# blairstar/NaturalDiffusion

Hardware: AMD Instinct MI355X
Metric: images/sec at 15-step Natural Inference (CIFAR10 32x32, NCSN++), 3-stream throughput (higher is better)
Workload: dtype bf16; 1 GPU; CIFAR10 NI 15-step step_15_weight_173.npz B=512/GPU NCSN++ 61.8M bf16, ni_step fp64 history; nfe=15, batch_per_gpu=512, streams=3

## Files before the change

### include/natinf_ncsnpp.h

```cpp
#ifndef NATINF_NCSNPP_H
#define NATINF_NCSNPP_H

#include <stdint.h>
#include "natinf.h"

#ifdef __cplusplus
extern "C" {
#endif

typedef struct natinf_ncsnpp* natinf_ncsnpp_t;

#define NATINF_NCSNPP_KEEP_ACTIVATIONS 1
#define NATINF_NCSNPP_DDPM 2

int64_t natinf_ncsnpp_param_count(void);
int64_t natinf_ncsnpp_packed_bytes(void);
int64_t natinf_ncsnpp_handle_param_count(natinf_ncsnpp_t h);
int64_t natinf_ncsnpp_handle_packed_bytes(natinf_ncsnpp_t h);
int64_t natinf_ncsnpp_workspace_bytes(natinf_ncsnpp_t h, int max_batch);

int natinf_ncsnpp_create(natinf_ncsnpp_t* out, int flags);
int natinf_ncsnpp_destroy(natinf_ncsnpp_t h);

int natinf_ncsnpp_describe(natinf_ncsnpp_t h, char* buf, int cap);

int natinf_ncsnpp_load(natinf_ncsnpp_t h, const float* params_f32, int64_t n_params,
                       void* packed, int64_t packed_bytes, natinf_stream_t stream);

int natinf_ncsnpp_share(natinf_ncsnpp_t h, natinf_ncsnpp_t loaded);

int natinf_ncsnpp_forward(natinf_ncsnpp_t h, const float* x, const float* labels, float* out, int B,
                          void* workspace, int64_t workspace_bytes, natinf_stream_t stream);

int natinf_ncsnpp_describe_gemms(natinf_ncsnpp_t h, int B, char* buf, int cap);

int natinf_debug_gemm(int variant, int M, int N, int K0, int K1, int taps, int logW, int batch,
                      const void* a0, const void* a1, const void* b, const float* bias_n, void* c, int c_f32, float scale,
                      int iters, natinf_stream_t stream);
int natinf_debug_quant_fp8_rows(const float* w, void* q, float* row_scale, int rows, int cols, natinf_stream_t stream);
int natinf_debug_gemm_fused(int variant, int M, int N, int K, const void* a, const void* b, const float* bias_n, const float* bias_m,
                            const float* rowvec, const float* gate, int log_rows_per_sample, const void* resid_bf16, const float* resid_f32,
                            float scale, int act, void* c, int c_f32, float* gn_part, int* bm_out, int fp32_slab, natinf_stream_t stream);
int natinf_debug_gemm_fp8(int M, int N, int K, const void* a8, const float* a_scale, const void* a_mx, const void* b8, const float* b_scale,
                          const float* bias_n, void* c, void* c_mx, int c_mode, int iters, natinf_stream_t stream);
int natinf_debug_conv_gn_up(int flags);
int natinf_debug_conv_gn(int res, int B, int N, int cin, int c1, const void* x, const float* scale, const float* shift, const void* w_packed, void* w_frag,
                         const void* a1, const float* bias_n, const void* resid, float out_scale, void* out, float* gn_part, int iters,
                         natinf_stream_t stream);
int natinf_set_gemm_variant(int variant);
int natinf_set_gemm_epilogue(int fp32_slab);
int natinf_set_gemm_pref512(int on);
int natinf_set_gemm_half_issue(int on);
int natinf_set_gemm_round_model(int on);
int natinf_set_gemm_w128(int on);
int natinf_set_gemm_raster(int rows);
int natinf_set_fuse_gn(int on);
int natinf_set_conv_gn_wide(int mask);
int natinf_set_conv_gn_w128(int mask);
int natinf_set_conv_gn_w128_min_k(int shape, int k);
int natinf_set_conv_gn_regw(int on);
int natinf_set_fuse_up(int on);
int natinf_set_fuse_head(int on);
int natinf_set_fuse_gn8(int on);
int natinf_set_fuse_gn4(int on);
int natinf_set_fuse_fin(int on);
int natinf_set_conv_gn_warm(int mask);
int natinf_set_attn256(int on);
int natinf_set_attn_proj(int on);
int natinf_set_attn_waves8(int on);
int natinf_set_attn_block(int on);
int natinf_set_attn_qkv(int on);
int natinf_set_conv_gn8_tile(int one_image);
int natinf_set_gemm_splitk(int on);
int natinf_debug_set_splitk_workspace(float* ws, int max_slices);
int natinf_debug_timestamps(void* dev_buf16);

int natinf_ncsnpp_profile(natinf_ncsnpp_t h, int enable);
int natinf_ncsnpp_profile_read(natinf_ncsnpp_t h, double* ms_by_class , int64_t* launches_by_class );

int natinf_gemm_profile(int enable);
int natinf_gemm_profile_read(char* buf, int cap);

int natinf_ncsnpp_debug_tap(natinf_ncsnpp_t h, int module_idx, float* out, int64_t capacity_elems,
                            natinf_stream_t stream);

#ifdef __cplusplus
}
#endif
#endif
```

### naturaldiffusion_amd/_lib.py

```python
from __future__ import annotations

import ctypes as C
import os
from pathlib import Path

os.environ.setdefault("GPU_MAX_HW_QUEUES", "8")

_HERE = Path(__file__).resolve().parent
LIB_PATH = Path(os.environ.get("NATINF_LIB", _HERE / "libnatinf.so"))

if not LIB_PATH.exists():
    raise ImportError(
        f"{LIB_PATH} not found: build it with `make -C {_HERE / 'csrc'}` "
        "(or `python -c 'import __graft_entry__ as g; g.build()'`). "
        "naturaldiffusion_amd has no CPU or eager-PyTorch fallback.")

lib = C.CDLL(str(LIB_PATH))

_p, _i32, _i64, _f32, _f64 = C.c_void_p, C.c_int, C.c_int64, C.c_float, C.c_double

SIGNATURES = {
    "natinf_abi_version": (C.c_int, []),
    "natinf_strerror": (C.c_char_p, [_i32]),
    "natinf_probe": (C.c_int, []),
    "natinf_step_f64hist": (C.c_int, [_p, _p, _p, _p, _p, _p, _p, _i32, _f64, _i32, _f64, _f64, _f32, _f32, _i64, _p]),
    "natinf_step_f32hist": (C.c_int, [_p, _p, _p, _p, _p, _p, _p, _i32, _f32, _i32, _f32, _f32, _f32, _f32, _i64, _p]),
    "natinf_weighted_sum_f64": (C.c_int, [_p, _p, _p, _p, _i32, _i64, _p]),
    "natinf_randn_philox_f32": (C.c_int, [_p, _i64, _i64, _p, _i64, _i64, C.c_uint64, _p]),
    "natinf_to_pixel_u8": (C.c_int, [_p, _p, _i32, _i32, _i32, _i32, _i32, _p]),
    "natinf_step_f32prod": (C.c_int, [_p, _p, _p, _f32, _i64, _i64, _p, _p, _p, _p, _p, _i32, _f32, _p, _p, _i32,
                                      _i32, _f32, _f32, _i64, _p]),
    "natinf_weighted_sum_f32prod": (C.c_int, [_p, _p, _p, _p, _i32, _i64, _p]),
    "natinf_step_f16chain": (C.c_int, [_p, _p, _p, _p, _p, _p, _p, _p, _p, _i32, _f32, _f32, _i32, _f32, _f32, _f32,
                                       _f32, _i32, _i64, _p]),
    "natinf_weighted_mean_f16": (C.c_int, [_p, _p, _p, _p, _i32, _f32, _i64, _p]),
    "natinf_flow_input_f16": (C.c_int, [_p, _p, _p, _f32, _f32, _i64, _p]),
    "natinf_ncsnpp_param_count": (C.c_int64, []),
    "natinf_ncsnpp_workspace_bytes": (C.c_int64, [_p, _i32]),
    "natinf_ncsnpp_packed_bytes": (C.c_int64, []),
    "natinf_ncsnpp_handle_param_count": (_i64, [_p]),
    "natinf_ncsnpp_handle_packed_bytes": (_i64, [_p]),
    "natinf_ncsnpp_create": (C.c_int, [C.POINTER(_p), _i32]),
    "natinf_ncsnpp_describe": (C.c_int, [_p, C.c_char_p, _i32]),
    "natinf_ncsnpp_destroy": (C.c_int, [_p]),
    "natinf_ncsnpp_load": (C.c_int, [_p, _p, _i64, _p, _i64, _p]),
    "natinf_ncsnpp_share": (C.c_int, [_p, _p]),
    "natinf_ncsnpp_forward": (C.c_int, [_p, _p, _p, _p, _i32, _p, _i64, _p]),
    "natinf_ncsnpp_debug_tap": (C.c_int, [_p, _i32, _p, _i64, _p]),
    "natinf_ncsnpp_describe_gemms": (C.c_int, [_p, _i32, C.c_char_p, _i32]),
    "natinf_debug_gemm": (C.c_int, [_i32, _i32, _i32, _i32, _i32, _i32, _i32, _i32, _p, _p, _p, _p, _p, _i32, _f32, _i32, _p]),
    "natinf_set_gemm_variant": (C.c_int, [_i32]),
    "natinf_debug_timestamps": (C.c_int, [_p]),
    "natinf_set_gemm_epilogue": (C.c_int, [_i32]),
    "natinf_debug_gemm_fused": (C.c_int, [_i32, _i32, _i32, _i32, _p, _p, _p, _p, _p, _p, _i32, _p, _p, _f32, _i32, _p, _i32, _p, _p, _i32, _p]),
    "natinf_set_gemm_pref512": (C.c_int, [_i32]),
    "natinf_set_gemm_half_issue": (C.c_int, [_i32]),
    "natinf_set_gemm_raster": (C.c_int, [_i32]),
    "natinf_set_gemm_round_model": (C.c_int, [_i32]),
    "natinf_set_gemm_w128": (C.c_int, [_i32]),
    "natinf_set_fuse_gn": (C.c_int, [_i32]),
    "natinf_set_conv_gn_wide": (C.c_int, [_i32]),
    "natinf_set_attn_block": (C.c_int, [_i32]),
    "natinf_set_conv_gn_w128": (C.c_int, [_i32]),
    "natinf_set_conv_gn_w128_min_k": (C.c_int, [_i32, _i32]),
    "natinf_set_conv_gn_regw": (C.c_int, [_i32]),
    "natinf_set_fuse_up": (C.c_int, [_i32]),
    "natinf_set_fuse_head": (C.c_int, [_i32]),
    "natinf_set_fuse_gn8": (C.c_int, [_i32]),
    "natinf_set_fuse_gn4": (C.c_int, [_i32]),
    "natinf_set_fuse_fin": (C.c_int, [_i32]),
    "natinf_set_attn_proj": (C.c_int, [_i32]),
    "natinf_set_attn_waves8": (C.c_int, [_i32]),
    "natinf_set_attn_qkv": (C.c_int, [_i32]),
    "natinf_set_conv_gn_warm": (C.c_int, [_i32]),
    "natinf_set_attn256": (C.c_int, [_i32]),
    "natinf_set_conv_gn8_tile": (C.c_int, [_i32]),
    "natinf_set_gemm_splitk": (C.c_int, [_i32]),
    "natinf_debug_set_splitk_workspace": (C.c_int, [_p, _i32]),
    "natinf_debug_conv_gn": (C.c_int, [_i32, _i32, _i32, _i32, _i32, _p, _p, _p, _p, _p, _p, _p, _p, _f32, _p, _p, _i32, _p]),
    "natinf_debug_conv_gn_up": (C.c_int, [_i32]),
    "natinf_ncsnpp_profile": (C.c_int, [_p, _i32]),
    "natinf_ncsnpp_profile_read": (C.c_int, [_p, C.POINTER(C.c_double), C.POINTER(C.c_int64)]),
    "natinf_debug_quant_fp8_rows": (C.c_int, [_p, _p, _p, _i32, _i32, _p]),
    "natinf_debug_gemm_fp8": (C.c_int, [_i32, _i32, _i32, _p, _p, _p, _p, _p, _p, _p, _p, _i32, _i32, _p]),
    "natinf_dit_create": (C.c_int, [C.POINTER(_p), _i32, _i32, _i32, _i32]),
    "natinf_dit_destroy": (C.c_int, [_p]),
    "natinf_dit_param_count": (C.c_int64, [_p]),
    "natinf_dit_packed_bytes": (C.c_int64, [_p]),
    "natinf_dit_workspace_bytes": (C.c_int64, [_p, _i32]),
    "natinf_dit_load": (C.c_int, [_p, _p, _i64, _p, _i64, _p]),
    "natinf_dit_forward": (C.c_int, [_p, _p, _p, _p, _p, _i32, _p, _i64, _p]),
    "natinf_mmdit_create": (C.c_int, [C.POINTER(_p), _i32, _i32, _i32, _i32, _i32, _i32, _i32, _i32]),
    "natinf_mmdit_destroy": (C.c_int, [_p]),
    "natinf_mmdit_param_count": (C.c_int64, [_p]),
    "natinf_mmdit_packed_bytes": (C.c_int64, [_p]),
    "natinf_mmdit_workspace_bytes": (C.c_int64, [_p, _i32]),
    "natinf_mmdit_load": (C.c_int, [_p, _p, _i64, _p, _i64, _p]),
    "natinf_mmdit_forward": (C.c_int, [_p, _p, _p, _p, _p, _p, _i32, _p, _i64, _p]),
    "natinf_attention_hd64_bf16": (C.c_int, [_p, _p, _i32, _i64, _p, _p, _i32, _i64, _i32, _i32, _i32, _i32, C.c_float, _p]),
    "natinf_inception_create": (C.c_int, [_p, _i32, _i32]),
    "natinf_inception_destroy": (C.c_int, [_p]),
    "natinf_set_inception_conv": (C.c_int, [_i32]),
    "natinf_debug_conv_ring": (C.c_int, [_i32] * 14 + [_p, _p, _p, _p, _p, _p, _i32, _p]),
    "natinf_inception_param_count": (_i64, [_p]),
    "natinf_inception_packed_bytes": (_i64, [_p]),
    "natinf_inception_workspace_bytes": (_i64, [_p, _i32]),
    "natinf_inception_load": (C.c_int, [_p, _p, _i64, _p, _i64, _p]),
    "natinf_inception_forward": (C.c_int, [_p, _p, _i32, _p, _i32, _p, _i64, _p]),
    "natinf_gemm_profile": (C.c_int, [_i32]),
    "natinf_gemm_profile_read": (C.c_int, [_p, _i32]),
    "natinf_set_mmdit_stream16": (C.c_int, [_i32]),
    "natinf_set_dit_stream16": (C.c_int, [_i32]),
    "natinf_set_mmdit_text_flat": (C.c_int, [_i32]),
    "natinf_attention_profile": (C.c_int, [_i32]),
    "natinf_set_mmdit_text_stream": (C.c_int, [_i32]),
    "natinf_set_flash_mode": (C.c_int, [_i32]),
    "natinf_attention_profile_read": (C.c_int, [_p, _p]),
    "natinf_vae_create": (C.c_int, [C.POINTER(_p), _i32, _i32]),
    "natinf_vae_destroy": (C.c_int, [_p]),
    "natinf_vae_param_count": (C.c_int64, [_p]),
    "natinf_vae_packed_bytes": (C.c_int64, [_p]),
    "natinf_vae_workspace_bytes": (C.c_int64, [_p, _i32]),
    "natinf_vae_load": (C.c_int, [_p, _p, _i64, _p, _i64, _p]),
    "natinf_vae_decode": (C.c_int, [_p, _p, _p, _i32, _p, _i64, _p]),
}

for _name, (_res, _args) in SIGNATURES.items():
    try:
        _fn = getattr(lib, _name)
    except AttributeError as e:
        raise ImportError(f"{LIB_PATH} does not export {_name}; rebuild it") from e
    _fn.restype, _fn.argtypes = _res, _args

SD3_CFG_ON_VELOCITY = 1


def check(rc: int, what: str) -> None:
    if rc != 0:
        raise RuntimeError(f"{what} failed: {lib.natinf_strerror(rc).decode()} ({rc})")


def stream_ptr(stream=None) -> int:
    import torch
    s = stream if stream is not None else torch.cuda.current_stream()
    return int(s.cuda_stream)


def ptr(t) -> int:
    return 0 if t is None else int(t.data_ptr())


def require_gpu() -> None:
    import torch
    if not torch.cuda.is_available():
        raise RuntimeError("naturaldiffusion_amd needs an MI355X (gfx950) GPU: torch.cuda.is_available() is False "
                           "and there is no CPU fallback")
    check(lib.natinf_probe(), "natinf_probe")
```

### naturaldiffusion_amd/csrc/conv_gn3.h

```cpp
#pragma once
#include "gemm_dma.h"

namespace ncsn {

template <int RES, int WM_, int WN_>
struct ConvGn3Cfg {
    static_assert(WM_ * WN_ == 4 && (RES == 32 || RES == 16), "four waves; 32x32 / 16x16 images");
    static constexpr int W = RES, WS = RES + 2, HW = RES * RES, NW = 4, THREADS = 256, KT = 32;
    static constexpr int WM = WM_, WN = WN_, TM = 8, TN = 8;
    static constexpr int BM_ = WM_ * 128, BN_ = WN_ * 128;
    static_assert(HW % BM_ == 0 && BM_ % W == 0, "a tile is whole image rows of one image");
    static constexpr int PR = BM_ / W + 2, PLAST = PR * WS;
    static constexpr int NPIECE = (PLAST + 15) / 16, NROUND = (NPIECE + NW - 1) / NW;
    static constexpr int PATCH_BYTES = NROUND * NW * 1024;
    static constexpr int TAB_BYTES = 256;
    static constexpr int PSW = BM_ / 16 / NW, SC_BYTES = BM_ * 64;
    static constexpr int OFF_TAB = 2 * PATCH_BYTES, OFF_SC = OFF_TAB + 2 * TAB_BYTES, LOOP_BYTES = OFF_SC + 2 * SC_BYTES;
    using Epi = EpiCfg<WM_, WN_, 8, 8, 163840>;
    static constexpr int LDS_BYTES = LOOP_BYTES > Epi::PACK_BYTES ? LOOP_BYTES : Epi::PACK_BYTES;
    static_assert(Epi::PACK_OK && LDS_BYTES <= 163840, "one block per CU");
    static constexpr int swz_key(int xx) { return (xx >> 1) & 2; }
    static constexpr int aoff(int i) { return (RES == 32 ? (i >> 1) * WS + (i & 1) * 16 : i * WS) * 64; }
    static constexpr int BAR = 40;
    static constexpr int rd_a(int i) { return 10 + 2 * i; }
    static constexpr int rd_a_late(int i) { return BAR + 2 + 2 * i; }
    static constexpr int dma_sc(int n) { return BAR + 1 + 2 * n; }
    static_assert(rd_a_late(7) < 64 && dma_sc(PSW - 1) < 64, "inside the step");
    static constexpr int RLEN = 34;
    static constexpr int G_END = 6 * 64 + BAR - 2;
    static constexpr int STRIDE = (G_END - 1 - RLEN - 2 - 12) / (NROUND - 1) > RLEN + 1 ? (G_END - 1 - RLEN - 2 - 12) / (NROUND - 1) : RLEN + 1;
    static constexpr int gp(int r) { return 12 + r * STRIDE; }
    static constexpr int gl(int r) { return r == 0 ? 2 : gp(r - 1) + 5; }
    static_assert(gp(NROUND - 1) + RLEN + 2 < G_END, "the rounds end in front of the barrier of tap 8");
    static constexpr int td(int r) { return gl(r) / 64; }
    static constexpr int nd(int t) { int n = t == 0 ? 2 : 0; for (int r = 0; r < NROUND; ++r) n += td(r) == t; return n; }
    static constexpr int DMA_TAB = 9;
    static constexpr int dma_piece(int r) { int k = td(r) == 0 ? 1 : 0; for (int q = 0; q < r; ++q) k += td(q) == td(r); return 9 + 2 * k; }
    static_assert(td(NROUND - 1) < 8 && dma_piece(NROUND - 1) < 40, "requests behind the weight loads, in front of the barrier");
};

__device__ __forceinline__ void cg3_mfma(f32x4& acc, const u32x4& b, const u32x4& a) {
    asm volatile("v_mfma_f32_16x16x32_bf16 %0, %1, %2, %0" : "+a"(acc) : "v"(b), "v"(a));
}
__device__ __forceinline__ u32x4 cg3_gload16(unsigned voff, const void* sbase) {
    u32x4 v;
    asm volatile("global_load_dwordx4 %0, %1, %2" : "=v"(v) : "v"(voff), "s"(sbase) : "memory");
    return v;
}
__device__ __forceinline__ void cg3_glds16(unsigned voff, const void* sbase, unsigned lds_dst) {
    NATINF_M0_ASM_BEGIN
    asm volatile("s_mov_b32 m0, %2\n\ts_nop 0\n\tglobal_load_lds_dwordx4 %0, %1" :: "v"(voff), "s"(sbase), "s"(lds_dst) : "memory", "m0");
    NATINF_M0_ASM_END
}
__device__ __forceinline__ void cg3_gtab(unsigned toff, const float* sc, const float* sh, unsigned lds_dst) {
    unsigned long long save;
    NATINF_M0_ASM_BEGIN
    asm volatile("s_mov_b32 m0, %4\n\t"
                 "s_mov_b64 %0, exec\n\t"
                 "s_mov_b32 exec_lo, -1\n\t"
                 "s_mov_b32 exec_hi, 0\n\t"
                 "global_load_lds_dword %1, %2\n\t"
                 "s_not_b64 exec, exec\n\t"
                 "global_load_lds_dword %1, %3\n\t"
                 "s_mov_b64 exec, %0"
                 : "=&s"(save) : "v"(toff), "s"(sc), "s"(sh), "s"(lds_dst) : "memory", "m0", "scc");
    NATINF_M0_ASM_END
}
template <int OFF> __device__ __forceinline__ void cg3_lds_write16(unsigned addr, const u32x4& v) {
    asm volatile("ds_write_b128 %0, %1 offset:%2" :: "v"(addr), "v"(v), "n"(OFF) : "memory");
}
template <int VM, int LGKM> __device__ __forceinline__ void cg3_wait() {
    if constexpr (LGKM >= 0) asm volatile("s_waitcnt vmcnt(%0) lgkmcnt(%1)" :: "n"(VM), "n"(LGKM) : "memory");
    else asm volatile("s_waitcnt vmcnt(%0)" :: "n"(VM) : "memory");
}
__device__ __forceinline__ void cg3_wait_lgkm0() { asm volatile("s_waitcnt lgkmcnt(0)" ::: "memory"); }
__device__ __forceinline__ void cg3_barrier() { asm volatile("s_barrier" ::: "memory"); }

#ifdef NATINF_CG3_TIMELINE
#define NATINF_CG3_STAMP(i) do { if (g.dbg_ts && (blockIdx.x == 0 || blockIdx.x == 300) && threadIdx.x == 0) { unsigned long long t_; \
    asm volatile("s_memtime %0\n\ts_waitcnt lgkmcnt(0)" : "=s"(t_) :: "memory"); g.dbg_ts[(blockIdx.x ? 64 : 0) + (i)] = t_; } } while (0)
#else
#define NATINF_CG3_STAMP(i) do { } while (0)
#endif

template <class Cfg>
struct CG3Ctx {
    u32x4 fa[2][8], fb[2][8];
    unsigned boff[8];
    unsigned vo[Cfg::NROUND];
    unsigned scv[Cfg::PSW];
    unsigned a_dx[3];
    unsigned a_sc;
    unsigned nadr[Cfg::NROUND];
    unsigned ninf[Cfg::NROUND];
    unsigned n_tab;
    unsigned tvo;
    u32x4 nv, ns0, ns1, nh0, nh1, npk;
    unsigned nx[8], ne[8];
    const unsigned char* wnext;
    const bf16* pnext;
    const float* tsc; const float* tsh;
    const bf16* scnext;
    unsigned lds_patch, lds_tab, lds_sc, wave;
};

template <int GG, int R, class Cfg>
__device__ __forceinline__ void cg3_norm_gap(CG3Ctx<Cfg>& c) {
    if constexpr (GG < 4) {
        asm volatile("v_lshlrev_b32 %0, 16, %1" : "=v"(c.nx[2 * GG]) : "v"(c.nv[GG]));
        asm volatile("v_and_b32 %0, 0xffff0000, %1" : "=v"(c.nx[2 * GG + 1]) : "v"(c.nv[GG]));
    } else if constexpr (GG < 8) {
        constexpr int P = GG - 4;
        if constexpr (P < 2) {
            asm volatile("v_fma_f32 %0, %0, %1, %2" : "+v"(c.nx[2 * P]) : "v"(c.ns0[2 * P]), "v"(c.nh0[2 * P]));
            asm volatile("v_fma_f32 %0, %0, %1, %2" : "+v"(c.nx[2 * P + 1]) : "v"(c.ns0[2 * P + 1]), "v"(c.nh0[2 * P + 1]));
        } else {
            asm volatile("v_fma_f32 %0, %0, %1, %2" : "+v"(c.nx[2 * P]) : "v"(c.ns1[2 * P - 4]), "v"(c.nh1[2 * P - 4]));
            asm volatile("v_fma_f32 %0, %0, %1, %2" : "+v"(c.nx[2 * P + 1]) : "v"(c.ns1[2 * P - 3]), "v"(c.nh1[2 * P - 3]));
        }
    } else if constexpr (GG < 16) asm volatile("v_exp_f32 %0, %1" : "=v"(c.ne[GG - 8]) : "v"(c.nx[GG - 8]));
    else if constexpr (GG < 20) {
        asm volatile("v_add_f32 %0, %1, %0" : "+v"(c.ne[2 * (GG - 16)]) : "v"(c.ninf[R]));
        asm volatile("v_add_f32 %0, %1, %0" : "+v"(c.ne[2 * (GG - 16) + 1]) : "v"(c.ninf[R]));
    } else if constexpr (GG < 28) asm volatile("v_rcp_f32 %0, %0" : "+v"(c.ne[GG - 20]));
    else if constexpr (GG < 32) {
        asm volatile("v_mul_f32 %0, %0, %1" : "+v"(c.nx[2 * (GG - 28)]) : "v"(c.ne[2 * (GG - 28)]));
        asm volatile("v_mul_f32 %0, %0, %1" : "+v"(c.nx[2 * (GG - 28) + 1]) : "v"(c.ne[2 * (GG - 28) + 1]));
    } else {
        constexpr int P = 2 * (GG - 32);
        asm volatile("v_cvt_pk_bf16_f32 %0, %1, %2" : "=v"(c.npk[P]) : "v"(c.nx[2 * P]), "v"(c.nx[2 * P + 1]));
        asm volatile("v_cvt_pk_bf16_f32 %0, %1, %2" : "=v"(c.npk[P + 1]) : "v"(c.nx[2 * P + 2]), "v"(c.nx[2 * P + 3]));
    }
}

template <class Cfg, int NB, int G, int R = 0>
__device__ __forceinline__ void cg3_norm_slot(CG3Ctx<Cfg>& c) {
    if constexpr (R == 0) {
        if constexpr (G == 0) { c.ns0 = lds_read16<NB * Cfg::TAB_BYTES>(c.n_tab); c.ns1 = lds_read16<NB * Cfg::TAB_BYTES + 16>(c.n_tab); }
        if constexpr (G == 1) { c.nh0 = lds_read16<NB * Cfg::TAB_BYTES + 128>(c.n_tab); c.nh1 = lds_read16<NB * Cfg::TAB_BYTES + 144>(c.n_tab); }
    }
    if constexpr (R < Cfg::NROUND) {
        constexpr int GP = Cfg::gp(R);
        if constexpr (G == Cfg::gl(R)) c.nv = lds_read16<NB * Cfg::PATCH_BYTES>(c.nadr[R]);
        if constexpr (G == GP) cg3_wait_lgkm0();
        if constexpr (G >= GP && G < GP + Cfg::RLEN) cg3_norm_gap<G - GP, R>(c);
        if constexpr (G == GP + Cfg::RLEN) cg3_lds_write16<NB * Cfg::PATCH_BYTES>(c.nadr[R], c.npk);
        cg3_norm_slot<Cfg, NB, G, R + 1>(c);
    }
}

template <class Cfg, int T, int HP, bool NEXT, int S>
struct CG3Tap {
    template <int I>
    static __device__ __forceinline__ void reads(CG3Ctx<Cfg>& c) {
        if constexpr (I < 8) {
            constexpr int P = (T + HP) & 1;
            if constexpr (T < 8) {
                if constexpr (S == Cfg::rd_a(I))
                    c.fa[P ^ 1][I] = lds_read16<HP * Cfg::PATCH_BYTES + Cfg::aoff(I) + ((T + 1) / 3) * Cfg::WS * 64>(c.a_dx[(T + 1) % 3]);
            } else if constexpr (S == Cfg::rd_a_late(I)) {
                if constexpr (NEXT) c.fa[P ^ 1][I] = lds_read16<(HP ^ 1) * Cfg::PATCH_BYTES + Cfg::aoff(I)>(c.a_dx[0]);
                else c.fa[P ^ 1][I] = lds_read16<I * 1024>(c.a_sc);
            }
            reads<I + 1>(c);
        }
    }
    template <int R>
    static __device__ __forceinline__ void requests(CG3Ctx<Cfg>& c) {
        if constexpr (R < Cfg::NROUND) {
            if constexpr (T == Cfg::td(R) && S == Cfg::dma_piece(R))
                cg3_glds16(c.vo[R], c.pnext, c.lds_patch + (HP ^ 1) * Cfg::PATCH_BYTES + (R * Cfg::NW) * 1024 + c.wave * 1024);
            requests<R + 1>(c);
        }
    }
    static __device__ __forceinline__ void run(f32x4 (&acc)[8][8], CG3Ctx<Cfg>& c) {
        constexpr int P = (T + HP) & 1;
        if constexpr (S == 0) {
            if constexpr (T >= 1 && NEXT) cg3_wait<Cfg::nd(T - 1), 0>(); else cg3_wait<0, 0>();
        }
        if constexpr (S >= 1 && S <= 8) c.fb[P ^ 1][S - 1] = cg3_gload16(c.boff[S - 1], c.wnext);
        reads<0>(c);
        if constexpr (NEXT) {
            if constexpr (T == 0 && S == Cfg::DMA_TAB) cg3_gtab(c.tvo, c.tsc, c.tsh, c.lds_tab + (HP ^ 1) * Cfg::TAB_BYTES);
            requests<0>(c);
        } else if constexpr (T == 8 && S > Cfg::BAR && (S - Cfg::BAR - 1) % 2 == 0 && (S - Cfg::BAR - 1) / 2 < Cfg::PSW) {
            constexpr int n = (S - Cfg::BAR - 1) / 2;
            cg3_glds16(c.scv[n], c.scnext, c.lds_sc + Cfg::SC_BYTES + n * 1024 + c.wave * (Cfg::PSW * 1024));
        }
        if constexpr (T >= 2 && NEXT) cg3_norm_slot<Cfg, HP ^ 1, (T - 2) * 64 + S>(c);
        if constexpr (T == 8) {
            if constexpr (S == Cfg::BAR - 1) cg3_wait_lgkm0();
            if constexpr (S == Cfg::BAR) cg3_barrier();
        }
        constexpr int i = S >> 3, j = S & 7;
        cg3_mfma(acc[i][j], c.fb[P][j], c.fa[P][i]);
        if constexpr (S + 1 < 64) CG3Tap<Cfg, T, HP, NEXT, S + 1>::run(acc, c);
    }
};

template <class Cfg, int P, int S>
struct CG3Sc {
    static __device__ __forceinline__ void run(f32x4 (&acc)[8][8], CG3Ctx<Cfg>& c) {
        if constexpr (S == 0) cg3_wait<Cfg::PSW, 0>();
        if constexpr (S == 1) cg3_barrier();
        if constexpr (S >= 1 && S <= 8) c.fb[P ^ 1][S - 1] = cg3_gload16(c.boff[S - 1], c.wnext);
        if constexpr (S >= 9 && (S - 9) % 2 == 0 && (S - 9) / 2 < Cfg::PSW) {
            constexpr int n = (S - 9) / 2;
            cg3_glds16(c.scv[n], c.scnext, c.lds_sc + P * Cfg::SC_BYTES + n * 1024 + c.wave * (Cfg::PSW * 1024));
        }
        if constexpr (S == Cfg::BAR - 1) cg3_wait<8 + Cfg::PSW, -1>();
        if constexpr (S == Cfg::BAR) cg3_barrier();
        if constexpr (S > Cfg::BAR + 1 && (S - Cfg::BAR - 2) % 2 == 0 && (S - Cfg::BAR - 2) / 2 < 8) {
            constexpr int i = (S - Cfg::BAR - 2) / 2;
            c.fa[P ^ 1][i] = lds_read16<(P ^ 1) * Cfg::SC_BYTES + i * 1024>(c.a_sc);
        }
        constexpr int i = S >> 3, j = S & 7;
        cg3_mfma(acc[i][j], c.fb[P][j], c.fa[P][i]);
        if constexpr (S + 1 < 64) CG3Sc<Cfg, P, S + 1>::run(acc, c);
    }
};

template <int RES, int WM, int WN, int EPI>
__global__ __launch_bounds__(256) __attribute__((amdgpu_waves_per_eu(1, 1))) void k_conv_gn3(const GemmArgs g)
{
    using Cfg = ConvGn3Cfg<RES, WM, WN>;
    constexpr int W = Cfg::W, WS = Cfg::WS, HW = Cfg::HW, BM_ = Cfg::BM_, BN_ = Cfg::BN_, NROUND = Cfg::NROUND, PSW = Cfg::PSW, KT = Cfg::KT;
    extern __shared__ __attribute__((aligned(16))) unsigned char smem[];
    lds_poison();
    const int tid = threadIdx.x, lane = tid & 63;
    const int wave = __builtin_amdgcn_readfirstlane(tid >> 6);
    NATINF_CG3_STAMP(0);
    const int wm = wave / WN, wn = wave % WN;
    const int nN = g.N / BN_, nM = g.M / BM_;
    const int tile = xcd_remap(blockIdx.x, nM * nN);
    const int mt = tile / nN, nt = tile - mt * nN;
    const int m0 = mt * BM_, n0 = nt * BN_;
    const int b = m0 / HW, y0 = (m0 % HW) / W;
    const int ush = g.a0_up;
    const bf16* const img = g.a0 + (int64_t)b * (HW >> (2 * ush)) * g.a0_ld;
    const float* const gsc = g.gn_scale + (int64_t)b * g.gn_ld;
    const float* const gsh = g.gn_shift + (int64_t)b * g.gn_ld;
    const int n_half = g.a0_C / KT, n_sc = g.a1 ? g.a1_C / KT : 0;
    const int nk = 9 * n_half, NT = nk + n_sc;
    const unsigned char* const wfrag = reinterpret_cast<const unsigned char*>(g.b_frag);
    const int sup = g.a1_up;
    const bf16* const a1base = g.a1 ? g.a1 + (int64_t)(sup ? b * (HW >> 2) : m0) * g.a1_ld : nullptr;

    typedef __attribute__((address_space(3))) unsigned char lds_u8;
    CG3Ctx<Cfg> c;
    c.wave = (unsigned)wave;
    c.lds_patch = (unsigned)(uintptr_t)((lds_u8*)smem);
    c.lds_tab = c.lds_patch + Cfg::OFF_TAB;
    c.lds_sc = c.lds_patch + Cfg::OFF_SC;
    const int prow = lane >> 2, pslot = lane & 3;
#pragma unroll
    for (int j = 0; j < 8; ++j) c.boff[j] = (unsigned)(((n0 >> 4) + wn * 8 + j) * NT) * 1024u + (unsigned)lane * 16u;
#pragma unroll
    for (int r = 0; r < NROUND; ++r) {
        const int pp = (r * 4 + wave) * 16 + prow;
        const int yy = pp / WS, xx = pp - yy * WS;
        const int y = min(max(y0 - 1 + yy, 0), RES - 1), x = min(max(xx - 1, 0), RES - 1);
        c.vo[r] = (unsigned)(((y >> ush) * (W >> ush) + (x >> ush)) * g.a0_ld + ((pslot ^ Cfg::swz_key(xx)) << 3)) * 2u;
        const bool inside = (unsigned)(y0 - 1 + yy) < (unsigned)RES && (unsigned)(xx - 1) < (unsigned)RES;
        c.ninf[r] = inside ? 0x3f800000u : 0x7f800000u;
        c.nadr[r] = c.lds_patch + (unsigned)((r * 4 + wave) * 1024 + prow * 64 + ((pslot ^ Cfg::swz_key(xx)) << 4));
    }
#pragma unroll
    for (int n = 0; n < PSW; ++n) {
        const int pp = (wave * PSW + n) * 16 + prow;
        const int src = sup ? ((y0 + pp / W) >> 1) * (W >> 1) + ((pp % W) >> 1) : pp;
        c.scv[n] = (unsigned)(src * g.a1_ld + ((pslot ^ ((pp >> 1) & 2)) << 3)) * 2u;
    }
    c.tvo = (unsigned)(lane & 31) * 4u;
    c.n_tab = c.lds_tab + ((unsigned)pslot << 5);
    {
        const int frow = lane & 15, fq = lane >> 4;
        const int ml = wm * 128 + frow;
        const int pc = ((ml / W) + 1) * WS + (ml % W) + 1, xc = ml % W;
#pragma unroll
        for (int d = 0; d < 3; ++d) c.a_dx[d] = c.lds_patch + (unsigned)((pc - WS + d - 1) * 64 + ((fq ^ Cfg::swz_key(xc + d)) << 4));
        c.a_sc = c.lds_sc + (unsigned)(ml * 64 + ((fq ^ ((ml >> 1) & 2)) << 4));
    }

    if (n_sc > 0) {
#pragma unroll
        for (int n = 0; n < PSW; ++n) cg3_glds16(c.scv[n], a1base, c.lds_sc + n * 1024 + c.wave * (PSW * 1024));
    }
    cg3_gtab(c.tvo, gsc, gsh, c.lds_tab);
#pragma unroll
    for (int r = 0; r < NROUND; ++r) cg3_glds16(c.vo[r], img, c.lds_patch + (r * 4) * 1024 + c.wave * 1024);
#pragma unroll
    for (int j = 0; j < 8; ++j) c.fb[0][j] = cg3_gload16(c.boff[j], wfrag);
    c.scnext = n_sc > 0 ? a1base + KT : reinterpret_cast<const bf16*>(wfrag);
    f32x4 acc[8][8];
#pragma unroll
    for (int i = 0; i < 8; ++i)
#pragma unroll
        for (int j = 0; j < 8; ++j) acc[i][j] = f32x4{0.f, 0.f, 0.f, 0.f};
    NATINF_CG3_STAMP(1);
    auto norm0 = [&](auto r_tag, const f32x4& s0, const f32x4& s1, const f32x4& h0, const f32x4& h1) __attribute__((always_inline)) {
        constexpr int R = decltype(r_tag)::value;
        cg3_wait<NROUND - 1 - R + 8, -1>();
        unsigned char* const pa = smem + (c.nadr[R] - c.lds_patch);
        const u32x4 nv = *reinterpret_cast<const u32x4*>(pa);
        const float ni = __uint_as_float(c.ninf[R]);
        u32x4 ou;
#pragma unroll
        for (int p = 0; p < 4; ++p) {
            const unsigned w_ = nv[p];
            const float x0 = __uint_as_float(w_ << 16), x1 = __uint_as_float(w_ & 0xffff0000u);
            const float sa = p < 2 ? s0[2 * p] : s1[2 * p - 4], sb = p < 2 ? s0[2 * p + 1] : s1[2 * p - 3];
            const float ha = p < 2 ? h0[2 * p] : h1[2 * p - 4], hb = p < 2 ? h0[2 * p + 1] : h1[2 * p - 3];
            const float t0 = __builtin_fmaf(x0, sa, ha), t1 = __builtin_fmaf(x1, sb, hb);
            const float y0_ = t0 * __builtin_amdgcn_rcpf(ni + __builtin_amdgcn_exp2f(t0)), y1_ = t1 * __builtin_amdgcn_rcpf(ni + __builtin_amdgcn_exp2f(t1));
            typedef __bf16 bf16x2_t __attribute__((ext_vector_type(2)));
            const bf16x2_t pr_ = {(bf16)y0_, (bf16)y1_};
            ou[p] = __builtin_bit_cast(unsigned, pr_);
        }
        *reinterpret_cast<u32x4*>(pa) = ou;
    };
    {
        cg3_wait<NROUND + 8, -1>();
        NATINF_CG3_STAMP(2);
        const unsigned char* const tp = smem + (c.n_tab - c.lds_patch);
        const f32x4 s0 = *reinterpret_cast<const f32x4*>(tp), s1 = *reinterpret_cast<const f32x4*>(tp + 16);
        const f32x4 h0 = *reinterpret_cast<const f32x4*>(tp + 128), h1 = *reinterpret_cast<const f32x4*>(tp + 144);
        using std::integral_constant;
        norm0(integral_constant<int, 0>{}, s0, s1, h0, h1); norm0(integral_constant<int, 1>{}, s0, s1, h0, h1); norm0(integral_constant<int, 2>{}, s0, s1, h0, h1);
        norm0(integral_constant<int, 3>{}, s0, s1, h0, h1); norm0(integral_constant<int, 4>{}, s0, s1, h0, h1); norm0(integral_constant<int, 5>{}, s0, s1, h0, h1);
        if constexpr (NROUND > 6) { norm0(integral_constant<int, 6>{}, s0, s1, h0, h1); norm0(integral_constant<int, 7>{}, s0, s1, h0, h1); }
        if constexpr (NROUND > 8) { norm0(integral_constant<int, 8>{}, s0, s1, h0, h1); norm0(integral_constant<int, 9>{}, s0, s1, h0, h1); }
        static_assert(NROUND == 6 || NROUND == 8 || NROUND == 10, "rounds of the prologue");
    }
    cg3_wait<0, -1>();
    __syncthreads();
#pragma unroll
    for (int i = 0; i < 8; ++i) c.fa[0][i] = *reinterpret_cast<const u32x4*>(smem + (c.a_dx[0] - c.lds_patch) + Cfg::aoff(i));
    asm volatile("s_waitcnt lgkmcnt(0)" ::: "memory");
    __builtin_amdgcn_sched_barrier(0);

    NATINF_CG3_STAMP(3);
    using std::integral_constant;
    auto half_chunk = [&](auto hp_tag, auto next_tag, int h) __attribute__((always_inline)) {
        constexpr int HP = decltype(hp_tag)::value;
        constexpr bool NEXT = decltype(next_tag)::value;
        c.pnext = img + (h + 1) * KT; c.tsc = gsc + (h + 1) * KT; c.tsh = gsh + (h + 1) * KT;
        const int kt = h * 9;
        NATINF_CG3_STAMP(4 + (h < 36 ? h : 35));
#define NATINF_CG3_TAP(T)                                                                                             \
        c.wnext = wfrag + (int64_t)((T < 8 || NEXT) ? kt + T + 1 : min(nk, NT - 1)) * 1024;                              \
        CG3Tap<Cfg, T, HP, NEXT, 0>::run(acc, c);
        NATINF_CG3_TAP(0) NATINF_CG3_TAP(1) NATINF_CG3_TAP(2) NATINF_CG3_TAP(3) NATINF_CG3_TAP(4)
        NATINF_CG3_TAP(5) NATINF_CG3_TAP(6) NATINF_CG3_TAP(7) NATINF_CG3_TAP(8)
#undef NATINF_CG3_TAP
    };
    for (int h = 0; h + 2 < n_half; h += 2) {
        half_chunk(integral_constant<int, 0>{}, std::true_type{}, h);
        half_chunk(integral_constant<int, 1>{}, std::true_type{}, h + 1);
    }
    half_chunk(integral_constant<int, 0>{}, std::true_type{}, n_half - 2);
    half_chunk(integral_constant<int, 1>{}, std::false_type{}, n_half - 1);
    NATINF_CG3_STAMP(40);
    for (int s = 0; s < n_sc; s += 2) {
        c.wnext = wfrag + (int64_t)min(nk + s + 1, NT - 1) * 1024; c.scnext = a1base + min(s + 2, n_sc - 1) * KT;
        CG3Sc<Cfg, 0, 0>::run(acc, c);
        c.wnext = wfrag + (int64_t)min(nk + s + 2, NT - 1) * 1024; c.scnext = a1base + min(s + 3, n_sc - 1) * KT;
        CG3Sc<Cfg, 1, 0>::run(acc, c);
    }
    cg3_wait<0, 0>();
#define NATINF_CG3_PIN8(a) asm volatile("" :: "v"(a[0]), "v"(a[1]), "v"(a[2]), "v"(a[3]), "v"(a[4]), "v"(a[5]), "v"(a[6]), "v"(a[7]));
    NATINF_CG3_PIN8(c.fb[0]) NATINF_CG3_PIN8(c.fb[1]) NATINF_CG3_PIN8(c.fa[0]) NATINF_CG3_PIN8(c.fa[1])
#undef NATINF_CG3_PIN8
    NATINF_CG3_STAMP(41);
#if defined(__HIP_DEVICE_COMPILE__)
    typedef const unsigned __attribute__((address_space(4))) *kernarg_u32_t;
    kernarg_u32_t gp = (kernarg_u32_t)__builtin_amdgcn_kernarg_segment_ptr();
    asm volatile("" : "+s"(gp));
    GemmArgs ge;
    {
        unsigned* d = reinterpret_cast<unsigned*>(&ge);
#pragma unroll
        for (unsigned i = 0; i < sizeof(GemmArgs) / 4; ++i) d[i] = gp[i];
    }
    asm volatile("" :: "s"(ge.c), "s"(ge.bias_n), "s"(ge.rowvec), "s"(ge.resid), "s"(ge.gn_part), "s"(ge.c_ld), "s"(ge.rowvec_ld), "s"(ge.resid_ld), "s"(ge.gn_quads),
                 "s"(ge.log_rows_per_sample), "s"(ge.scale), "s"(ge.M), "s"(ge.N));
#else
    const GemmArgs ge = g;
#endif
    asm volatile("s_waitcnt vmcnt(0) lgkmcnt(0)\n\ts_nop 15\n\ts_nop 15\n\ts_barrier" ::: "memory");
    __builtin_amdgcn_sched_barrier(0);
    int lane_e;
    asm volatile("v_mbcnt_lo_u32_b32 %0, -1, 0\n\tv_mbcnt_hi_u32_b32 %0, -1, %0" : "=v"(lane_e));
    const int tid_e = wave * 64 + lane_e;
    NATINF_CG3_STAMP(42);
    static_assert(EPI == 1 || EPI == 2 || EPI == 5 || EPI == 6, "packed epilogues: plain / + GroupNorm partials / + bf16 residual / both");
    constexpr bool FIN16 = RES == 16 && WM == 2 && WN == 2 && (EPI == 2 || EPI == 6);
    packed_tile_epilogue<WM, WN, 8, 8, typename Cfg::Epi, ACT_NONE, EPI == 2 || EPI == 6, EPI == 5 || EPI == 6, false, false, 1, FIN16, true, true>(ge, smem, acc, m0, n0, 0, tid_e, lane_e, wm, wn);
    NATINF_CG3_STAMP(43);
}

}
```

### naturaldiffusion_amd/csrc/ncsnpp.hip

```cpp
#include <hip/hip_runtime.h>
#include <stdint.h>
#include <stdio.h>
#include <string.h>
#include <stdlib.h>
#include <functional>
#include <map>
#include <memory>
#include <string>
#include <vector>

#include "natinf_ncsnpp.h"
#include "ncsnpp_kernels.h"
#include "gemm_dma.h"
#include "gemm_w128.h"
#include "conv_ring.h"
#include "conv_gn.h"
#include "conv_gn2.h"
#include "head_conv.h"
#ifdef NATINF_DEV
#include "conv_patch.h"
#include "gemm_8phase.h"
#endif
#include "gemm_fp8.h"
#include "attn_fused.h"
#include "attn256.h"
#include "attn_qkv.h"
#include "attn_blk256.h"
#include "flash_attn.h"

using namespace ncsn;

namespace {

constexpr int NF = 128, IMG = 32, TEMB = 512, NLEVEL = 4;
constexpr int CH_MULT[NLEVEL] = {1, 2, 2, 2};
constexpr float GN_EPS = 1e-6f;
constexpr float INV_SQRT2 = 0.70710678118654752440f;
inline bool attn_at(int res) { return res == 16; }
inline int ilog2(int v) { int l = 0; while ((1 << l) < v) ++l; return l; }
inline int64_t align_up(int64_t v, int64_t a) { return (v + a - 1) / a * a; }

enum Kind { K_LIN, K_CONV, K_RES, K_ATTN, K_GN, K_DOWN, K_UP };
const char* kind_name(int k) { static const char* n[] = {"lin", "conv", "res", "attn", "gn", "down", "up"}; return n[k]; }

struct Mod { int idx, kind, cin, cout, up, down, res; int64_t poff; };

struct TRef { int64_t off = -1; int C = 0, ld = 0, res = 0, coff = 0, pad = 0; };

struct Ctx {
    int B; unsigned char* ws; const unsigned char* wp; hipStream_t stream;
    const float* x; const float* labels; float* out;
    int* part_bm;
    hipStream_t stream2 = nullptr; hipEvent_t* ev = nullptr;
    unsigned char* fin_done = nullptr;
    bf16* act(const TRef& t) const { return reinterpret_cast<bf16*>(ws + t.off * B) + t.coff; }
    template <class T> T* at(int64_t off) const { return reinterpret_cast<T*>(ws + off * B); }
    template <class T> const T* w(int64_t off) const { return reinterpret_cast<const T*>(wp + off); }
};
using OpFn = std::function<void(const Ctx&)>;
enum { CLS_GEMM = 0, CLS_OTHER = 1, CLS_CONV_GN = 2, CLS_CONV_GN8 = 3, N_CLS = 4 };

struct PackCtx { const float* params; unsigned char* packed; hipStream_t stream; };
using PackFn = std::function<void(const PackCtx&)>;

struct Arena {
    bool keep = false; int64_t top = 0, peak = 0;
    std::map<int64_t, int64_t> free_;
    std::map<int64_t, int64_t> live_;
    int64_t alloc(int64_t bytes) {
        bytes = align_up(bytes, 256);
        if (!keep)
            for (auto it = free_.begin(); it != free_.end(); ++it)
                if (it->second >= bytes) {
                    const int64_t off = it->first, rest = it->second - bytes;
                    free_.erase(it);
                    if (rest) free_[off + bytes] = rest;
                    live_[off] = bytes;
                    return off;
                }
        const int64_t off = top; top += bytes; if (top > peak) peak = top;
        live_[off] = bytes;
        return off;
    }
    void release(int64_t off) {
        if (keep || off < 0) return;
        auto it = live_.find(off);
        if (it == live_.end()) return;
        int64_t o = off, s = it->second;
        live_.erase(it);
        auto nx = free_.lower_bound(o);
        if (nx != free_.end() && o + s == nx->first) { s += nx->second; nx = free_.erase(nx); }
        if (nx != free_.begin()) { auto pv = std::prev(nx); if (pv->first + pv->second == o) { o = pv->first; s += pv->second; free_.erase(pv); } }
        if (o + s == top) top = o; else free_[o] = s;
    }
};

}

struct natinf_ncsnpp {
    int flags = 0;
    std::vector<Mod> mods;
    int64_t n_params = 0;
    std::vector<OpFn> ops;
    std::vector<int> op_cls;
    std::vector<PackFn> packs;
    bool prof = false;
    struct Rec { hipEvent_t a, b; int cls; };
    std::vector<Rec> recs;
    std::vector<hipEvent_t> pool;
    std::map<int, TRef> taps;
    int64_t ws_per_image = 0, packed_bytes = 0;
    uint64_t plan_sig = 0;
    const unsigned char* packed = nullptr;
    bool attr_set = false;
    int last_B = 0; unsigned char* last_ws = nullptr;
    std::vector<int> part_bm;
    std::vector<unsigned char> fin_done;
};

bool configure_conv_ring();
namespace { bool configure_dit_attention(); }
namespace ncsn_cg3 { bool configure(); int tile_rows(int shape); int tile_cols(int shape); void launch(const void* gemm_args, int shape, int epi, void* stream); }

namespace {

int g_epi_fp32_slab = 0;
GemmArgs gemm_defaults() {
    GemmArgs g;
    memset(&g, 0, sizeof(g));
    g.epi_fp32_slab = g_epi_fp32_slab;
    g.taps = 1; g.batch = 1; g.scale = 1.0f; g.act = ACT_NONE; g.c_mode = OUT_BF16;
    return g;
}
constexpr int NUM_CU = 256;
enum GemmVariant {
    V_AUTO = 0, V_GENERIC = 1,
    V_DMA_256x256 = 2, V_DMA_256x128 = 3, V_DMA_128x128 = 4,
    V_RING_256x256 = 5, V_RING_256x128 = 6, V_RING_128x128 = 7, V_RING_64x128 = 8,
    V_RING_256x128_W4 = 9, V_DMA_256x128_W4 = 10,
    V_DMA_256x256_S = 11, V_DMA_128x128_S = 12,
    V_DMA_512x128 = 13,
    V_PATCH_256x256 = 14, V_PATCH_256x128 = 15,
    V_DMA_256x256_P = 16, V_DMA_128x128_P = 17, V_DMA_256x128W4_P = 18,
    V_8PH_256x256 = 19, V_8PH_NOPRIO = 20, V_8PH_READFIRST = 21, V_8PH_BOTH = 22,
    V_FP8_256x256 = 23,
    V_ABL_NODMA = 24, V_ABL_NOMFMA = 25,
    V_DMA_256x256_H = 26, V_DMA_512x128_H = 27,
    V_CONV_GN = 28,
    V_W128 = 29,
    V_W128_A = 30, V_W128_D = 31, V_W128_X = 32,
    V_COUNT
};
const char* variant_name(int v) {
    static const char* n[] = {"auto", "generic128", "dma256x256", "dma256x128", "dma128x128", "ring256x256", "ring256x128",
                              "ring128x128", "ring64x128", "ring256x128w4", "dma256x128w4", "dma256x256s", "dma128x128s", "dma512x128", "patch256x256", "patch256x128", "dma256x256p", "dma128x128p", "dma256x128w4p", "gemm8ph", "gemm8ph_np", "gemm8ph_rf", "gemm8ph_nprf", "fp8_256x256", "abl_nodma", "abl_nomfma", "dma256x256h", "dma512x128h", "conv_gn", "w128_256x256", "w128_a", "w128_d", "w128_x"};
    return v >= 0 && v < V_COUNT ? n[v] : "?";
}
inline bool variant_shipped(int v) {
#ifdef NATINF_DEV
    return v >= 0 && v < V_COUNT;
#else
    switch (v) {
        case V_AUTO: case V_GENERIC: case V_RING_64x128: case V_RING_256x128_W4: case V_DMA_128x128_P: case V_FP8_256x256:
        case V_DMA_256x256_H: case V_DMA_512x128_H: case V_CONV_GN: case V_W128: return true;
        default: return false;
    }
#endif
}
unsigned long long* g_dbg_ts = nullptr;
int g_force_variant = V_AUTO;
int g_half_issue = 1;
int g_round_model = 1;
int g_round_model_w128 = 13;
int g_pref_512 = 1;
std::string* g_record = nullptr;

int g_raster_g = 8;
template <class Cfg, class K>
inline void launch_tiles(K kernel, const GemmArgs& g0, hipStream_t s) {
    const int nM = (g0.M + Cfg::BM_ - 1) / Cfg::BM_, nN = (g0.N + Cfg::BN_ - 1) / Cfg::BN_;
    GemmArgs g = g0;
    g.raster_g = (g_raster_g > 1 && nN >= 8 && nM >= g_raster_g) ? g_raster_g : 0;
    int lds = Cfg::LDS_BYTES;
#ifdef NATINF_DEV
    static const int one_per_cu = getenv("NATINF_ONE_BLOCK_PER_CU") ? 1 : 0;
    if (one_per_cu && lds < 84000) {
        lds = 84000;
        (void)hipFuncSetAttribute(reinterpret_cast<const void*>(kernel), hipFuncAttributeMaxDynamicSharedMemorySize, lds);
    }
#endif
    hipLaunchKernelGGL(kernel, dim3(nM * nN, 1, g.batch), dim3(Cfg::THREADS), lds, s, g);
}
template <class Cfg, class K>
inline bool set_lds(K kernel) {
    return hipFuncSetAttribute(reinterpret_cast<const void*>(kernel), hipFuncAttributeMaxDynamicSharedMemorySize, Cfg::LDS_BYTES) == hipSuccess;
}
using CfgD256x256 = DmaCfg<2, 4, 8, 4>;  using CfgD256x128 = DmaCfg<4, 2, 4, 4>;  using CfgD128x128 = DmaCfg<2, 2, 4, 4>;
using CfgR256x256 = RingCfg<2, 4, 8, 4, 4>; using CfgR256x128 = RingCfg<4, 2, 4, 4, 6>;
using CfgR128x128 = RingCfg<2, 2, 4, 4, 4>; using CfgR64x128 = RingCfg<2, 2, 2, 4, 4>;
using CfgR256x128W4 = RingCfg<2, 2, 8, 4, 3>; using CfgD256x128W4 = DmaCfg<2, 2, 8, 4>;
using CfgD512x128 = DmaCfg<4, 2, 8, 4>;
using CfgH32 = ConvGn2Cfg<32>; using CfgH16 = ConvGn2Cfg<16>; using CfgH16W = ConvGn2Cfg<16, true>; using CfgH32W = ConvGn2Cfg<32, true>; using CfgH8T = ConvGn2Cfg<8, true, 4>; using CfgH4T = ConvGn2Cfg<4, true, 4, 2, 2>;
#ifdef NATINF_DEV
using CfgH8W = ConvGn2Cfg<8, true>;
using CfgP256x256 = PatchCfg<2, 4, 8, 4, 344>; using CfgP256x128 = PatchCfg<4, 2, 4, 4, 400>;
using CfgG32 = ConvGnCfg<32>; using CfgG16 = ConvGnCfg<16>; using CfgG16W = ConvGnCfg<16, true>;
#endif
int g_fuse_head = 1;
int g_cg8_tm4 = 1;
constexpr int ATTN_BLK_DEFAULT = 2;
int g_attn_blk = ATTN_BLK_DEFAULT;
int g_attn_qkv = 1;
int g_attn_w8 = 1;
int g_attn_proj = 1;
int g_attn256 = 1;
int g_fuse_gn8 = 1;
int g_cg_warm = 15;
int g_fuse_fin = 3;
int g_fuse_gn4 = 1;
int g_fuse_gn = 1;

constexpr unsigned EPI_ALL = 0x1FF;
constexpr unsigned EPI_R64 = EPI_ALL, EPI_D128 = EPI_ALL, EPI_RW4 = EPI_ALL & ~(1u << 3), EPI_D256H = EPI_ALL & ~(1u << 3),
                   EPI_D512H = EPI_ALL & ~((1u << 3) | (1u << 4) | (1u << 7) | (1u << 8)),
                   EPI_W128 = EPI_ALL & ~((1u << 2) | (1u << 3) | (1u << 6));
template <unsigned MASK, int E, class F> inline void epi_case(F&& f) { if constexpr ((MASK >> E) & 1u) f(std::integral_constant<int, E>{}); }
template <unsigned MASK, class F> inline bool for_each_epi(F&& f) {
    bool ok = true;
    auto one = [&](auto tag) { ok = ok && f(tag); };
    epi_case<MASK, 0>(one); epi_case<MASK, 1>(one); epi_case<MASK, 2>(one); epi_case<MASK, 3>(one); epi_case<MASK, 4>(one);
    epi_case<MASK, 5>(one); epi_case<MASK, 6>(one); epi_case<MASK, 7>(one); epi_case<MASK, 8>(one);
    return ok;
}
#define NATINF_EPI_OF(tag) decltype(tag)::value
bool set_lds_epi_all() {
    return for_each_epi<EPI_D128>([](auto t) { return set_lds<CfgD128x128>(&k_gemm_dma<2, 2, 4, 4, 2, NATINF_EPI_OF(t)>); }) &&
           for_each_epi<EPI_RW4>([](auto t) { return set_lds<CfgR256x128W4>(&k_gemm_ring<2, 2, 8, 4, 3, NATINF_EPI_OF(t)>); }) &&
           for_each_epi<EPI_R64>([](auto t) { return set_lds<CfgR64x128>(&k_gemm_ring<2, 2, 2, 4, 4, NATINF_EPI_OF(t)>); }) &&
           for_each_epi<EPI_D256H>([](auto t) { return set_lds<CfgD256x256>(&k_gemm_dma<2, 4, 8, 4, 6, NATINF_EPI_OF(t)>); }) &&
           for_each_epi<EPI_D512H>([](auto t) { return set_lds<CfgD512x128>(&k_gemm_dma<4, 2, 8, 4, 6, NATINF_EPI_OF(t)>); }) &&
           for_each_epi<EPI_W128>([](auto t) { return set_lds<W128Cfg>(&k_gemm_w128<NATINF_EPI_OF(t)>); }) && set_lds<W128Cfg>(&k_gemm_w128<9>)
#ifdef NATINF_DEV
           && set_lds<W128Cfg>(&k_gemm_w128<1, W128SchA>) && set_lds<W128Cfg>(&k_gemm_w128<1, W128SchP>) && set_lds<W128Cfg>(&k_gemm_w128<1, W128SchX>)
           && for_each_epi<EPI_ALL>([](auto t) { return set_lds<CfgD256x256>(&k_gemm_dma<2, 4, 8, 4, 2, NATINF_EPI_OF(t)>); })
           && for_each_epi<EPI_ALL>([](auto t) { return set_lds<CfgD512x128>(&k_gemm_dma<4, 2, 8, 4, 2, NATINF_EPI_OF(t)>); })
#endif
        ;
}
template <int EPI>
bool set_lds_conv_gn() {
    return set_lds<CfgH32>(&k_conv_gn2<32, false, EPI>) && set_lds<CfgH32W>(&k_conv_gn2<32, true, EPI>) && set_lds<CfgH16>(&k_conv_gn2<16, false, EPI>) && set_lds<CfgH16W>(&k_conv_gn2<16, true, EPI>) &&
           set_lds<CfgH8T>(&k_conv_gn2<8, true, EPI, 4>) && set_lds<CfgH4T>(&k_conv_gn2<4, true, EPI, 4, 2, 2>)
#ifdef NATINF_DEV
           && set_lds<CfgH8W>(&k_conv_gn2<8, true, EPI>)
           && set_lds<CfgG32>(&k_conv_gn<32, false, EPI>) && set_lds<CfgG16>(&k_conv_gn<16, false, EPI>) && set_lds<CfgG16W>(&k_conv_gn<16, true, EPI>)
#endif
        ;
}

bool configure_gemm_kernels() {
    bool ok = hipFuncSetAttribute(reinterpret_cast<const void*>(&k_gemm_bf16), hipFuncAttributeMaxDynamicSharedMemorySize,
                                  GEMM_LDS_BYTES) == hipSuccess;
    ok = ok && hipFuncSetAttribute(reinterpret_cast<const void*>(&k_head_conv), hipFuncAttributeMaxDynamicSharedMemorySize, HeadConvCfg::LDS_BYTES) == hipSuccess &&
         set_lds<CfgR128x128>(&k_gemm_ring<2, 2, 4, 4, 4, 9>) &&
         set_lds_epi_all() && ncsn_cg3::configure() && ::configure_conv_ring() && configure_dit_attention() && set_lds_conv_gn<1>() && set_lds_conv_gn<2>() && set_lds_conv_gn<5>() && set_lds_conv_gn<6>() &&
#ifdef NATINF_DEV
         set_lds<CfgD256x256>(&k_gemm_dma<2, 4, 8, 4>) && set_lds<CfgD256x128>(&k_gemm_dma<4, 2, 4, 4>) &&
         set_lds<CfgD128x128>(&k_gemm_dma<2, 2, 4, 4>) && set_lds<CfgR256x256>(&k_gemm_ring<2, 4, 8, 4, 4>) &&
         set_lds<CfgR256x128>(&k_gemm_ring<4, 2, 4, 4, 6>) && set_lds<CfgR128x128>(&k_gemm_ring<2, 2, 4, 4, 4>) &&
         set_lds<CfgD256x128W4>(&k_gemm_dma<2, 2, 8, 4>) && set_lds<CfgD256x256>(&k_gemm_dma<2, 4, 8, 4, 1>) &&
         set_lds<CfgD128x128>(&k_gemm_dma<2, 2, 4, 4, 1>) && set_lds<CfgD512x128>(&k_gemm_dma<4, 2, 8, 4>) &&
         set_lds<CfgP256x256>(&k_conv_patch<2, 4, 8, 4, 344>) && set_lds<CfgP256x128>(&k_conv_patch<4, 2, 4, 4, 400>) &&
         set_lds<CfgD256x128W4>(&k_gemm_dma<2, 2, 8, 4, 2>) &&
         set_lds<CfgD256x256>(&k_gemm_dma<2, 4, 8, 4, 3, 1>) && set_lds<CfgD256x256>(&k_gemm_dma<2, 4, 8, 4, 4, 1>) &&
         set_lds<Cfg8ph>(&k_gemm_8ph<0>) && set_lds<Cfg8ph>(&k_gemm_8ph<1>) && set_lds<Cfg8ph>(&k_gemm_8ph<2>) && set_lds<Cfg8ph>(&k_gemm_8ph<3>) &&
#endif
         set_lds<CfgD256x256>(&k_gemm_fp8<false, 0>) && set_lds<CfgD256x256>(&k_gemm_fp8<true, 0>) &&
         set_lds<CfgD256x256>(&k_gemm_fp8<false, 1>) && set_lds<CfgD256x256>(&k_gemm_fp8<true, 1>) &&
         set_lds<CfgD256x256>(&k_gemm_fp8<false, 2>) && set_lds<CfgD256x256>(&k_gemm_fp8<true, 2>) &&
         set_lds<CfgD256x256>(&k_gemm_fp8<false, 3>) && set_lds<CfgD256x256>(&k_gemm_fp8<true, 3>) &&
         set_lds<W128F8Cfg>(&k_gemm_w128_fp8<false, 0>) && set_lds<W128F8Cfg>(&k_gemm_w128_fp8<true, 0>) && set_lds<W128F8Cfg>(&k_gemm_w128_fp8<false, 1>) && set_lds<W128F8Cfg>(&k_gemm_w128_fp8<true, 1>) &&
         set_lds<W128F8Cfg>(&k_gemm_w128_fp8<false, 2>) && set_lds<W128F8Cfg>(&k_gemm_w128_fp8<true, 2>) && set_lds<W128F8Cfg>(&k_gemm_w128_fp8<false, 3>) && set_lds<W128F8Cfg>(&k_gemm_w128_fp8<true, 3>) &&
#ifdef NATINF_DEV
         set_lds<AttnCfg<8, 16, true>>(&k_attn_fused<8, 16, true>) &&
#endif
         hipFuncSetAttribute(reinterpret_cast<const void*>(&k_qkv256), hipFuncAttributeMaxDynamicSharedMemorySize, QKV_LDS_BYTES) == hipSuccess &&
         hipFuncSetAttribute(reinterpret_cast<const void*>(&k_attn256<false>), hipFuncAttributeMaxDynamicSharedMemorySize, A256_LDS_BYTES) == hipSuccess &&
         hipFuncSetAttribute(reinterpret_cast<const void*>(&k_attn256<true>), hipFuncAttributeMaxDynamicSharedMemorySize, A256_LDS_BYTES) == hipSuccess &&
         hipFuncSetAttribute(reinterpret_cast<const void*>(&k_attn256<true, 8>), hipFuncAttributeMaxDynamicSharedMemorySize, A256_LDS_BYTES) == hipSuccess &&
         hipFuncSetAttribute(reinterpret_cast<const void*>(&k_attn_blk256), hipFuncAttributeMaxDynamicSharedMemorySize, ABLK_LDS_BYTES) == hipSuccess &&
         hipFuncSetAttribute(reinterpret_cast<const void*>(&k_attn_blk256_v2), hipFuncAttributeMaxDynamicSharedMemorySize, ABLK2_LDS_BYTES) == hipSuccess &&
         hipFuncSetAttribute(reinterpret_cast<const void*>(&k_flash_attn64), hipFuncAttributeMaxDynamicSharedMemorySize, FA_LDS_BYTES) == hipSuccess &&
#ifdef NATINF_DEV
         hipFuncSetAttribute(reinterpret_cast<const void*>(&k_flash_attn64_v2<0>), hipFuncAttributeMaxDynamicSharedMemorySize, FA_LDS_BYTES) == hipSuccess &&
         hipFuncSetAttribute(reinterpret_cast<const void*>(&k_flash_attn64_v2<1>), hipFuncAttributeMaxDynamicSharedMemorySize, FA_LDS_BYTES) == hipSuccess &&
#endif
         hipFuncSetAttribute(reinterpret_cast<const void*>(&k_flash_attn64_v2<1, 64>), hipFuncAttributeMaxDynamicSharedMemorySize, FA_LDS_BYTES / 2) == hipSuccess;
    if (!ok) (void)hipGetLastError();
    return ok;
}

#ifdef NATINF_DEV
inline bool eligible_8ph(const GemmArgs& g) { return g.M % 256 == 0 && g.N % 256 == 0; }
#endif

int variant_bm(int v);
int packed_epi(const GemmArgs& g, int bm);
int g_cg3 = 7;
int g_cg_wide = 3;
int g_fuse_up = 1;
int g_cg_regw = 1;
int g_cg3_min_k[3] = {2304, 0, 2304};
inline int conv_gn3_shape(const GemmArgs& g) {
    const int res = 1 << g.logW;
    if (!g_cg3 || !g_cg_regw || !g.b_frag || g.N % 128) return -1;
    int sh = -1;
    if (res == 32) sh = g.N % 256 ? ((g_cg3 & 1) ? 0 : -1) : ((g_cg3 & 2) ? 1 : -1);
    else if (res == 16) sh = (g.N % 256 == 0 && (g_cg3 & 4)) ? 2 : -1;
    if (sh >= 0 && 9 * g.a0_C + (g.a1 ? g.a1_C : 0) < g_cg3_min_k[sh]) sh = -1;
    return sh;
}
inline int conv_gn_bm(const GemmArgs& g) {
    const int res = 1 << g.logW;
    if (const int sh3 = conv_gn3_shape(g); sh3 >= 0) return ncsn_cg3::tile_rows(sh3);
    if (res == 8) return g_cg8_tm4 ? 64 : 128;
    if (res == 4) return 64;
    if (res == 32) return ((g_cg_wide & 2) && g.N % 256 == 0 && g_cg_regw && g.b_frag) ? 128 : 256;
    return ((g_cg_wide & 1) && res == 16 && g.N % 256 == 0) ? 128 : 256;
}
inline int conv_gn_part_rows(const GemmArgs& g) { const int res = 1 << g.logW; return res <= 8 ? res * res : conv_gn_bm(g); }
inline bool conv_gn_regw(const GemmArgs& g) { return g_cg_regw && g.b_frag && (conv_gn3_shape(g) >= 0 || g.N % ((conv_gn_bm(g) <= 128 && (1 << g.logW) != 4) ? 256 : 128) == 0); }
#ifdef NATINF_DEV
constexpr bool HAVE_CONV_GN_V1 = true;
#else
constexpr bool HAVE_CONV_GN_V1 = false;
#endif
inline int conv_gn_epi(const GemmArgs& g) { GemmArgs t = g; t.epi_fp32_slab = 0; return packed_epi(t, conv_gn_part_rows(g)); }
inline bool conv_gn_ok(const GemmArgs& g) {
    if (!g.gn_scale || !g.gn_shift || !g.gn_folded || g.taps != 9 || g.batch != 1 || g.a0_C % BK || (g.a1 && g.a1_C % BK)) return false;
    const int res = 1 << g.logW;
    if (g.logHW != 2 * g.logW || (res != 32 && res != 16 && res != 8 && res != 4) || g.N % 8) return false;
    if (res == 4 && (g.a0_C % (64 * CfgH4T::NG) || (g.a1 && g.a1_C % (64 * CfgH4T::NG)))) return false;
    if (res <= 8 ? (g.M % (res * res) || g.N % (res == 4 ? 128 : 256) || g.a0_up || g.a1_up || !conv_gn_regw(g) || (g.resid && g.rowvec)) : g.M % std::max(256, conv_gn_bm(g)) != 0) return false;
    if ((g.a0_up || g.a1_up || !HAVE_CONV_GN_V1) && !conv_gn_regw(g)) return false;
    const int e = conv_gn_epi(g);
    return e == 1 || e == 2 || e == 5 || e == 6;
}
int g_w128 = 1;
bool w128_ok(const GemmArgs& g) {
    if (g.taps != 1 || g.a1 || g.gn_scale || g.deq_m || g.deq_n || g.splitk > 1) return false;
    if (g.a0_C % BK || g.a0_C < 2 * BK || g.N % 8 || g.M % 8) return false;
    return (int64_t)g.M * g.a0_ld * 2 < (int64_t)1 << 32 && (int64_t)g.N * g.b_ld * 2 < (int64_t)1 << 32;
}
int choose_variant(const GemmArgs& g) {
    if (g.gn_scale) return V_CONV_GN;
    const int K0 = g.taps * g.a0_C, K1 = g.a1 ? g.a1_C : 0;
    const bool dma = K0 % BK == 0 && K1 % BK == 0 && (g.taps == 1 || (g.a0_padded && g.a0_C % BK == 0));
    if (!dma) return V_GENERIC;
    if (!variant_shipped(g_force_variant)) {  }
#ifdef NATINF_DEV
    else if (g_force_variant == V_PATCH_256x256 || g_force_variant == V_PATCH_256x128) {
        const bool patch_ok = g.taps == 9 && g.batch == 1 && g.logW >= 3;
        if (patch_ok && (g_force_variant == V_PATCH_256x128 || g.logW >= 4)) return g_force_variant;
    } else if (g_force_variant >= V_8PH_256x256 && g_force_variant <= V_8PH_BOTH) {
        if (eligible_8ph(g)) return g_force_variant;
    }
#endif
    else if (g_force_variant == V_W128) {
        if (w128_ok(g) && (!g.gn_part || (1 << g.logHW) % 256 == 0)) return V_W128;
    }
#ifdef NATINF_DEV
    else if (g_force_variant >= V_W128_A && g_force_variant <= V_W128_X) {
        if (w128_ok(g) && packed_epi(g, 256) == 1) return g_force_variant;
    }
#endif
    else if (g_force_variant > V_GENERIC && g_force_variant != V_CONV_GN && g_force_variant != V_FP8_256x256) {
        if (!g.gn_part || (g.taps == 9 && (1 << g.logHW) % variant_bm(g_force_variant) == 0)) return g_force_variant;
    }
    const int64_t mt256 = (g.M + 255) / 256, mt128 = (g.M + 127) / 128;
    const int64_t nt128 = (g.N + 127) / 128;
#ifdef NATINF_DEV
    const bool half = g_half_issue != 0;
#else
    constexpr bool half = true;
#endif
    const bool w128 = g_w128 && w128_ok(g) && (!g.gn_part || (1 << g.logHW) % 256 == 0);
    const int64_t nt256 = (g.N + 255) / 256;
    const bool n_ok256 = g.N % 256 == 0 || (w128 && g.N % 128 == 0);
    if (g_round_model && g.taps == 1 && !g.gn_part && g.batch == 1 && n_ok256 && K0 + K1 >= 1024 && mt256 * nt256 < 2 * NUM_CU) {
        const int64_t r256 = (mt256 * nt256 + NUM_CU - 1) / NUM_CU, r128 = (mt128 * nt128 + 2 * NUM_CU - 1) / (2 * NUM_CU);
        const int64_t c256 = w128 ? g_round_model_w128 : 15;
        if (mt128 * nt128 >= NUM_CU / 2) return c256 * r256 < 10 * r128 ? (w128 ? V_W128 : half ? V_DMA_256x256_H : V_DMA_256x256_P) : V_DMA_128x128_P;
    }
    if (n_ok256 && K0 + K1 >= 1024 && mt256 * nt256 * g.batch >= NUM_CU) return w128 ? V_W128 : half ? V_DMA_256x256_H : V_DMA_256x256_P;
    if (g_pref_512 && g.N <= 128 && K0 + K1 >= 1024 && ((g.M + 511) / 512) * g.batch >= 2 * NUM_CU &&
        (!g.gn_part || (g.taps == 9 && (1 << g.logHW) % 512 == 0)))
        return half ? V_DMA_512x128_H : V_DMA_512x128;
    if (mt256 * nt128 * g.batch >= 2 * NUM_CU) return V_RING_256x128_W4;
    if (mt128 * nt128 * g.batch >= NUM_CU) return V_DMA_128x128_P;
    return V_RING_64x128;
}

int variant_bm(int v) {
    switch (v) {
        case V_CONV_GN: case V_DMA_256x256: case V_DMA_256x128: case V_RING_256x256: case V_RING_256x128: case V_RING_256x128_W4: case V_DMA_256x128_W4:
        case V_ABL_NODMA: case V_ABL_NOMFMA: case V_DMA_256x256_H: case V_DMA_256x256_S: case V_PATCH_256x256: case V_PATCH_256x128: case V_DMA_256x256_P: case V_DMA_256x128W4_P: case V_8PH_256x256: case V_8PH_NOPRIO: case V_8PH_READFIRST: case V_8PH_BOTH: case V_FP8_256x256: case V_W128: case V_W128_A: case V_W128_D: case V_W128_X: return 256;
        case V_DMA_512x128: case V_DMA_512x128_H: return 512;
        case V_RING_64x128: return 64;
        default: return 128;
    }
}

int fp8_epi(const GemmArgs& g) {
    if (g.epi_fp32_slab || g.resid || g.gn_part) return 0;
    if ((g.rowvec || g.gate) && g.log_rows_per_sample < 30 && ((1 << g.log_rows_per_sample) % 256 != 0)) return 0;
    if (g.c_mode == OUT_F32 && g.resid_f32 && !g.bias_m && g.act == ACT_NONE && g.resid_f32_ld % 4 == 0 && g.c_ld % 4 == 0) return 3;
    if (g.resid_f32 || g.gate) return 0;
    if (g.c_mode == OUT_BF16 && g.act == ACT_NONE) return 1;
    if (g.c_mode == OUT_FP8_MX && g.act == ACT_GELU_TANH && g.c_mx && g.N % 32 == 0 && !g.bias_m && g.scale == 1.0f) return 2;
    return 0;
}
extern int g_w128;
bool w128_fp8_ok(const GemmArgs& g) {
    return g.taps == 1 && !g.a1 && g.a0_C % 256 == 0 && g.N % 8 == 0 && g.M % 8 == 0 && (!g.a_mx || g.M % 256 == 0) &&
           (int64_t)g.M * g.a0_ld < (int64_t)1 << 32 && (int64_t)g.N * g.b_ld < (int64_t)1 << 32;
}
bool fp8_on_w128(const GemmArgs& g) { return g_w128 && w128_fp8_ok(g) && (fp8_epi(g) != 2 || g_w128 != 2); }
template <bool MXA>
void launch_gemm_fp8_t(const GemmArgs& g, hipStream_t s) {
    if (fp8_on_w128(g)) {
        switch (fp8_epi(g)) {
            case 1: launch_tiles<W128F8Cfg>(&k_gemm_w128_fp8<MXA, 1>, g, s); break;
            case 2: launch_tiles<W128F8Cfg>(&k_gemm_w128_fp8<MXA, 2>, g, s); break;
            case 3: launch_tiles<W128F8Cfg>(&k_gemm_w128_fp8<MXA, 3>, g, s); break;
            default: launch_tiles<W128F8Cfg>(&k_gemm_w128_fp8<MXA, 0>, g, s); break;
        }
        return;
    }
    switch (fp8_epi(g)) {
        case 1: launch_tiles<CfgD256x256>(&k_gemm_fp8<MXA, 1>, g, s); break;
        case 2: launch_tiles<CfgD256x256>(&k_gemm_fp8<MXA, 2>, g, s); break;
        case 3: launch_tiles<CfgD256x256>(&k_gemm_fp8<MXA, 3>, g, s); break;
        default: launch_tiles<CfgD256x256>(&k_gemm_fp8<MXA, 0>, g, s); break;
    }
}
struct GemmProf {
    struct Rec { hipEvent_t a, b; std::string tag; };
    bool on = false; std::vector<Rec> ev; std::vector<std::pair<hipEvent_t, hipEvent_t>> pool;
    bool begin(Rec& r, hipStream_t s) {
        r.a = r.b = nullptr;
        if (!pool.empty()) { r.a = pool.back().first; r.b = pool.back().second; pool.pop_back(); }
        else if (hipEventCreate(&r.a) != hipSuccess || hipEventCreate(&r.b) != hipSuccess) { r.a = r.b = nullptr; (void)hipGetLastError(); return false; }
        (void)hipEventRecord(r.a, s);
        return true;
    }
    void end(Rec& r, hipStream_t s) { (void)hipEventRecord(r.b, s); ev.push_back(std::move(r)); }
} g_gemm_prof;
void launch_gemm_fp8(const GemmArgs& g, hipStream_t s) {
    GemmProf::Rec r;
    const bool prof = g_gemm_prof.on && !g_record && g_gemm_prof.begin(r, s);
    if (prof) {
        char line[160];
        snprintf(line, sizeof(line), "%d %d %d %d %d %d %s%s/e%d", g.M, g.N, g.taps * g.a0_C, 0, g.taps, g.batch, fp8_on_w128(g) ? "w128_fp8" : "fp8_256x256", g.a_mx ? "_mxa" : "", fp8_epi(g));
        r.tag = line;
    }
    if (g.a_mx) launch_gemm_fp8_t<true>(g, s); else launch_gemm_fp8_t<false>(g, s);
    if (prof) g_gemm_prof.end(r, s);
}

int packed_epi(const GemmArgs& g, int bm) {
    if (g.epi_fp32_slab || g.deq_m || g.deq_n || g.act == ACT_RELU) return 0;
    if (g.bias_m) return (g.c_mode == OUT_BF16 && !g.resid && !g.resid_f32 && !g.gate && !g.rowvec && !g.gn_part && g.act == ACT_NONE) ? 8 : 0;
    if ((g.rowvec || g.gate) && g.log_rows_per_sample < 30 && ((1 << g.log_rows_per_sample) % bm != 0)) return 0;
    if (g.c_mode == OUT_F32 && g.resid_f32 && !g.resid && !g.gn_part && g.act == ACT_NONE && g.resid_f32_ld % 4 == 0 && g.c_ld % 4 == 0) return 7;
    if (g.c_mode != OUT_BF16 || g.resid_f32 || g.gate) return 0;
    if (g.resid && (g.act != ACT_NONE || g.resid_ld % 4 != 0)) return 0;
    if (g.gn_part) return (g.act == ACT_NONE && g.M % bm == 0) ? (g.resid ? 6 : 2) : 0;
    if (g.resid) return 5;
    return g.act == ACT_NONE ? 1 : (g.act == ACT_SILU ? 3 : 4);
}
inline unsigned epi_mask(int v) {
    switch (v) {
        case V_RING_64x128: return EPI_R64;  case V_DMA_128x128_P: return EPI_D128;  case V_RING_256x128_W4: return EPI_RW4;
        case V_DMA_256x256_H: return EPI_D256H;  case V_DMA_512x128_H: return EPI_D512H;
        case V_DMA_256x256_P: case V_DMA_512x128: return EPI_ALL;
        case V_W128: return EPI_W128;
        default: return 1u;
    }
}
inline int effective_epi(int v, const GemmArgs& g) { const int e = packed_epi(g, variant_bm(v)); return ((epi_mask(v) >> e) & 1u) ? e : 0; }
#define NATINF_LAUNCH_EPI(MASK, CFG, KERN, ...)                                                                      \
    {                                                                                                                \
        auto run_ = [&](auto t_) { launch_tiles<CFG>(&KERN<__VA_ARGS__, NATINF_EPI_OF(t_)>, g, s); };                \
        switch (effective_epi(v, g)) {                                                                               \
            case 1: epi_case<MASK, 1>(run_); break;  case 2: epi_case<MASK, 2>(run_); break;                         \
            case 3: epi_case<MASK, 3>(run_); break;  case 4: epi_case<MASK, 4>(run_); break;                         \
            case 5: epi_case<MASK, 5>(run_); break;  case 6: epi_case<MASK, 6>(run_); break;                         \
            case 7: epi_case<MASK, 7>(run_); break;  case 8: epi_case<MASK, 8>(run_); break;                         \
            default: run_(std::integral_constant<int, 0>{}); break;                                                  \
        }                                                                                                            \
    }

thread_local int g_launch_error = 0;
thread_local bool g_fin_written = false;
int g_splitk = 1;
float* g_dbg_splitk_ws = nullptr; int g_dbg_splitk_max = 0;
int splitk_slices(const GemmArgs& g) {
    if (!g_splitk || !g.splitk_ws || g.splitk_max < 2 || g.batch != 1 || g.gn_scale || g.c_mode != OUT_BF16 || g.N % 8 || 256 % (g.N / 8)) return 1;
    if (g.gn_part && (g.M % SPLITK_ROWS || g.act != ACT_NONE || (g.taps == 9 && (1 << g.logHW) % SPLITK_ROWS))) return 1;
    if (g.bias_m || g.gate || g.resid_f32 || g.deq_m || g.deq_n) return 1;
    const int K0 = g.taps * g.a0_C, K1 = g.a1 ? g.a1_C : 0;
    if (K0 % 64 || K1 % 64 || (g.taps == 9 && !g.a0_padded) || K0 + K1 < 2048) return 1;
    const int64_t tiles = ((g.M + 127) / 128) * ((g.N + 127) / 128);
    if (tiles >= 2 * NUM_CU) return 1;
    int S = (int)((2 * NUM_CU + tiles - 1) / tiles);
    if (S > g.splitk_max) S = g.splitk_max;
    while (S > 1 && (K0 + K1) / 32 / S < 16) --S;
    return S;
}
int w128_splitk_slices(const GemmArgs& g) {
    if (!g_splitk || !g_w128 || !g.splitk_ws || g.splitk_max < 2 || g.batch != 1 || !w128_ok(g) || g.a0_C < 3072) return 1;
    if (g.c_mode != OUT_F32 || !g.resid_f32 || g.resid || g.rowvec || g.bias_m || g.gn_part || g.act != ACT_NONE || g.epi_fp32_slab || g.N % 4 || g.c_ld % 4 || g.resid_f32_ld % 4) return 1;
    const int64_t tiles = (int64_t)((g.M + 255) / 256) * ((g.N + 255) / 256) * g.batch;
    if (tiles * 2 > NUM_CU) return 1;
    int S = (int)(NUM_CU / tiles);
    if (S > g.splitk_max) S = g.splitk_max;
    while (S > 1 && g.a0_C / BK / S < 16) --S;
    return S;
}
int launch_gemm_run(const GemmArgs& g0, hipStream_t s);
int launch_gemm(const GemmArgs& g0, hipStream_t s) {
    if (!g_gemm_prof.on || g_record) return launch_gemm_run(g0, s);
    GemmProf::Rec r;
    std::string tag;
    g_record = &tag; (void)launch_gemm_run(g0, s); g_record = nullptr;
    while (!tag.empty() && tag.back() == '\n') tag.pop_back();
    if (!g_gemm_prof.begin(r, s)) return launch_gemm_run(g0, s);
    r.tag = std::move(tag);
    const int bm = launch_gemm_run(g0, s);
    g_gemm_prof.end(r, s);
    return bm;
}
int launch_gemm_run(const GemmArgs& g0, hipStream_t s) {
    if (g_force_variant == V_AUTO) {
        const int S8 = w128_splitk_slices(g0);
        if (S8 > 1) {
            if (g_record) {
                char line[160];
                snprintf(line, sizeof(line), "%d %d %d %d %d %d splitk%d_w128_256x256/e7\n", g0.M, g0.N, g0.taps * g0.a0_C, 0, g0.taps, g0.batch, S8);
                *g_record += line;
                return 256;
            }
            GemmArgs p = g0;
            p.splitk = S8; p.c = g0.splitk_ws; p.c_mode = OUT_F32;
            const int nM = (p.M + 255) / 256, nN = (p.N + 255) / 256;
            p.raster_g = 0;
            hipLaunchKernelGGL((k_gemm_w128<9>), dim3(nM * nN, S8, p.batch), dim3(256), W128Cfg::LDS_BYTES, s, p);
            const int64_t per = (int64_t)g0.M * (g0.N / 4);
            hipLaunchKernelGGL(k_splitk_reduce_f32, dim3((unsigned)((per + 255) / 256), (unsigned)g0.batch), dim3(256), 0, s, g0.splitk_ws, S8, (int64_t)g0.batch * g0.M * g0.N, g0.M, g0.N,
                               g0.bias_n, g0.gate, g0.gate_ld, g0.log_rows_per_sample, g0.z_samples, g0.resid_f32, g0.resid_f32_ld, g0.c_bs, g0.scale,
                               reinterpret_cast<float*>(g0.c), g0.c_ld, g0.stream_f16);
            return 256;
        }
    }
    const int S = g_force_variant == V_AUTO ? splitk_slices(g0) : 1;
    if (S > 1) {
        if (g_record) {
            char line[160];
            snprintf(line, sizeof(line), "%d %d %d %d %d %d splitk%d_ring128x128/e9\n", g0.M, g0.N, g0.taps * g0.a0_C, g0.a1 ? g0.a1_C : 0, g0.taps, g0.batch, S);
            *g_record += line;
            return SPLITK_ROWS;
        }
        GemmArgs p = g0;
        p.splitk = S; p.c = g0.splitk_ws; p.c_mode = OUT_F32; p.batch = S;
        p.bias_n = nullptr; p.rowvec = nullptr; p.resid = nullptr; p.scale = 1.0f; p.act = ACT_NONE; p.gn_part = nullptr;
        launch_tiles<CfgR128x128>(&k_gemm_ring<2, 2, 4, 4, 4, 9>, p, s);
        hipLaunchKernelGGL(k_splitk_reduce, dim3((unsigned)((g0.M + SPLITK_ROWS - 1) / SPLITK_ROWS)), dim3(256), 0, s, g0.splitk_ws, S, g0.M, g0.N,
                           g0.bias_n, g0.rowvec, g0.rowvec_ld, g0.log_rows_per_sample, reinterpret_cast<const bf16*>(g0.resid), g0.resid_ld, g0.scale,
                           g0.act, reinterpret_cast<bf16*>(g0.c), g0.c_ld, reinterpret_cast<float2*>(g0.gn_part), g0.gn_quads);
        return SPLITK_ROWS;
    }
    const GemmArgs& g = g0;
    const int v = choose_variant(g);
    if (v == V_CONV_GN && !conv_gn_ok(g)) {
        if (g_record) {
            char line[160];
            snprintf(line, sizeof(line), "%d %d %d %d %d %d invalid_conv_gn/e0\n", g.M, g.N, g.taps * g.a0_C, g.a1 ? g.a1_C : 0, g.taps, g.batch);
            *g_record += line;
        } else g_launch_error = 1;
        return 256;
    }
    if (g_record) {
        char line[160];
        snprintf(line, sizeof(line), "%d %d %d %d %d %d %s/e%d\n", g.M, g.N, g.taps * g.a0_C, g.a1 ? g.a1_C : 0, g.taps, g.batch,
                 v == V_CONV_GN && conv_gn3_shape(g) >= 0 ? "conv_gn3" : variant_name(v), v == V_CONV_GN ? conv_gn_epi(g) : effective_epi(v, g));
        *g_record += line;
        return v == V_CONV_GN ? conv_gn_part_rows(g) : variant_bm(v);
    }
    switch (v) {
        case V_GENERIC: {
            const int nM = (g.M + BM - 1) / BM, nN = (g.N + BN - 1) / BN;
            hipLaunchKernelGGL(k_gemm_bf16, dim3(nM * nN, 1, g.batch), dim3(256), GEMM_LDS_BYTES, s, g);
            break;
        }
        case V_RING_64x128: NATINF_LAUNCH_EPI(EPI_R64, CfgR64x128, k_gemm_ring, 2, 2, 2, 4, 4) break;
        case V_RING_256x128_W4: NATINF_LAUNCH_EPI(EPI_RW4, CfgR256x128W4, k_gemm_ring, 2, 2, 8, 4, 3) break;
        case V_DMA_128x128_P: NATINF_LAUNCH_EPI(EPI_D128, CfgD128x128, k_gemm_dma, 2, 2, 4, 4, 2) break;
        case V_FP8_256x256: launch_tiles<CfgD256x256>(&k_gemm_fp8<false, 0>, g, s); break;
        case V_DMA_256x256_H: NATINF_LAUNCH_EPI(EPI_D256H, CfgD256x256, k_gemm_dma, 2, 4, 8, 4, 6) break;
        case V_DMA_512x128_H: NATINF_LAUNCH_EPI(EPI_D512H, CfgD512x128, k_gemm_dma, 4, 2, 8, 4, 6) break;
#ifdef NATINF_DEV
        case V_W128_A: launch_tiles<W128Cfg>(&k_gemm_w128<1, W128SchA>, g, s); break;
        case V_W128_D: launch_tiles<W128Cfg>(&k_gemm_w128<1, W128SchP>, g, s); break;
        case V_W128_X: launch_tiles<W128Cfg>(&k_gemm_w128<1, W128SchX>, g, s); break;
#endif
        case V_W128: {
            auto run_ = [&](auto t_) { launch_tiles<W128Cfg>(&k_gemm_w128<NATINF_EPI_OF(t_)>, g, s); };
            switch (effective_epi(v, g)) {
                case 1: epi_case<EPI_W128, 1>(run_); break;  case 4: epi_case<EPI_W128, 4>(run_); break;
                case 5: epi_case<EPI_W128, 5>(run_); break;  case 7: epi_case<EPI_W128, 7>(run_); break;
                case 8: epi_case<EPI_W128, 8>(run_); break;
                default: run_(std::integral_constant<int, 0>{}); break;
            }
            break;
        }
#ifdef NATINF_DEV
        case V_DMA_256x256: launch_tiles<CfgD256x256>(&k_gemm_dma<2, 4, 8, 4>, g, s); break;
        case V_DMA_256x128: launch_tiles<CfgD256x128>(&k_gemm_dma<4, 2, 4, 4>, g, s); break;
        case V_DMA_128x128: launch_tiles<CfgD128x128>(&k_gemm_dma<2, 2, 4, 4>, g, s); break;
        case V_RING_256x256: launch_tiles<CfgR256x256>(&k_gemm_ring<2, 4, 8, 4, 4>, g, s); break;
        case V_RING_256x128: launch_tiles<CfgR256x128>(&k_gemm_ring<4, 2, 4, 4, 6>, g, s); break;
        case V_RING_128x128: launch_tiles<CfgR128x128>(&k_gemm_ring<2, 2, 4, 4, 4>, g, s); break;
        case V_DMA_256x128_W4: launch_tiles<CfgD256x128W4>(&k_gemm_dma<2, 2, 8, 4>, g, s); break;
        case V_DMA_256x256_S: launch_tiles<CfgD256x256>(&k_gemm_dma<2, 4, 8, 4, 1>, g, s); break;
        case V_DMA_128x128_S: launch_tiles<CfgD128x128>(&k_gemm_dma<2, 2, 4, 4, 1>, g, s); break;
        case V_DMA_512x128: NATINF_LAUNCH_EPI(EPI_ALL, CfgD512x128, k_gemm_dma, 4, 2, 8, 4, 2) break;
        case V_PATCH_256x256: launch_tiles<CfgP256x256>(&k_conv_patch<2, 4, 8, 4, 344>, g, s); break;
        case V_PATCH_256x128: launch_tiles<CfgP256x128>(&k_conv_patch<4, 2, 4, 4, 400>, g, s); break;
        case V_DMA_256x256_P: NATINF_LAUNCH_EPI(EPI_ALL, CfgD256x256, k_gemm_dma, 2, 4, 8, 4, 2) break;
        case V_DMA_256x128W4_P: launch_tiles<CfgD256x128W4>(&k_gemm_dma<2, 2, 8, 4, 2>, g, s); break;
        case V_8PH_256x256: launch_tiles<Cfg8ph>(&k_gemm_8ph<0>, g, s); break;
        case V_8PH_NOPRIO: launch_tiles<Cfg8ph>(&k_gemm_8ph<1>, g, s); break;
        case V_8PH_READFIRST: launch_tiles<Cfg8ph>(&k_gemm_8ph<2>, g, s); break;
        case V_8PH_BOTH: launch_tiles<Cfg8ph>(&k_gemm_8ph<3>, g, s); break;
        case V_ABL_NODMA: launch_tiles<CfgD256x256>(&k_gemm_dma<2, 4, 8, 4, 3, 1>, g, s); break;
        case V_ABL_NOMFMA: launch_tiles<CfgD256x256>(&k_gemm_dma<2, 4, 8, 4, 4, 1>, g, s); break;
#endif
        case V_CONV_GN: {
            GemmArgs gw = g0;
            gw.w_warm = (g_cg_warm >> (g0.logW - 2)) & 1;
            const GemmArgs& g = gw;
            const int e = conv_gn_epi(g);
            const int e4 = e == 1 ? 0 : (e == 2 ? 1 : (e == 5 ? 2 : 3));
#define NATINF_CG2_LAUNCH(CFG, RES, WIDE)                                                                   \
            switch (e4) {                                                                                       \
                case 0: launch_tiles<CFG>(&k_conv_gn2<RES, WIDE, 1>, g, s); break;                              \
                case 1: launch_tiles<CFG>(&k_conv_gn2<RES, WIDE, 2>, g, s); break;                              \
                case 2: launch_tiles<CFG>(&k_conv_gn2<RES, WIDE, 5>, g, s); break;                              \
                default: launch_tiles<CFG>(&k_conv_gn2<RES, WIDE, 6>, g, s); break;                             \
            }
            if (const int sh3 = conv_gn3_shape(g); sh3 >= 0) {
                ncsn_cg3::launch(&g, sh3, e, (void*)s);
                g_fin_written = sh3 == 2 && g.fin_scale && (e == 2 || e == 6) && g.N == 256;
                return conv_gn_part_rows(g);
            }
            if (conv_gn_regw(g)) {
                if ((1 << g.logW) == 8 && g_cg8_tm4) {
                    switch (e4) {
                        case 0: launch_tiles<CfgH8T>(&k_conv_gn2<8, true, 1, 4>, g, s); break;
                        case 1: launch_tiles<CfgH8T>(&k_conv_gn2<8, true, 2, 4>, g, s); break;
                        case 2: launch_tiles<CfgH8T>(&k_conv_gn2<8, true, 5, 4>, g, s); break;
                        default: launch_tiles<CfgH8T>(&k_conv_gn2<8, true, 6, 4>, g, s); break;
                    }
                }
#ifdef NATINF_DEV
                else if ((1 << g.logW) == 8) { NATINF_CG2_LAUNCH(CfgH8W, 8, true) }
#endif
                else if ((1 << g.logW) == 4) {
                    switch (e4) {
                        case 0: launch_tiles<CfgH4T>(&k_conv_gn2<4, true, 1, 4, 2, 2>, g, s); break;
                        case 1: launch_tiles<CfgH4T>(&k_conv_gn2<4, true, 2, 4, 2, 2>, g, s); break;
                        case 2: launch_tiles<CfgH4T>(&k_conv_gn2<4, true, 5, 4, 2, 2>, g, s); break;
                        default: launch_tiles<CfgH4T>(&k_conv_gn2<4, true, 6, 4, 2, 2>, g, s); break;
                    }
                }
                else if ((1 << g.logW) == 32 && conv_gn_bm(g) == 128) { NATINF_CG2_LAUNCH(CfgH32W, 32, true) }
                else if ((1 << g.logW) == 32) { NATINF_CG2_LAUNCH(CfgH32, 32, false) }
                else if (conv_gn_bm(g) == 128) { NATINF_CG2_LAUNCH(CfgH16W, 16, true) }
                else { NATINF_CG2_LAUNCH(CfgH16, 16, false) }
            }
#undef NATINF_CG2_LAUNCH
#ifdef NATINF_DEV
#define NATINF_CG_LAUNCH(CFG, RES, WIDE)                                                                    \
            switch (e4) {                                                                                       \
                case 0: launch_tiles<CFG>(&k_conv_gn<RES, WIDE, 1>, g, s); break;                               \
                case 1: launch_tiles<CFG>(&k_conv_gn<RES, WIDE, 2>, g, s); break;                               \
                case 2: launch_tiles<CFG>(&k_conv_gn<RES, WIDE, 5>, g, s); break;                               \
                default: launch_tiles<CFG>(&k_conv_gn<RES, WIDE, 6>, g, s); break;                              \
            }
            else if ((1 << g.logW) == 32) { NATINF_CG_LAUNCH(CfgG32, 32, false) }
            else if (conv_gn_bm(g) == 128) { NATINF_CG_LAUNCH(CfgG16W, 16, true) }
            else { NATINF_CG_LAUNCH(CfgG16, 16, false) }
#undef NATINF_CG_LAUNCH
#endif
            return conv_gn_part_rows(g);
        }
        default: break;
    }
    return variant_bm(v);
}
inline int grid1d(int64_t n, int block = 256, int cap = 4096) {
    int64_t g = (n + block - 1) / block; return (int)(g < 1 ? 1 : (g > cap ? cap : g));
}

struct Builder {
    natinf_ncsnpp& E;
    Arena arena;
    int64_t wtop = 0;
    int64_t poff = 0;
    int dense_total = 0; int64_t dense_w = 0, dense_b = 0, dense_out = 0;

    const bool ddpm;
    const int NUM_RES;
    const float res_scale;
    explicit Builder(natinf_ncsnpp& e) : E(e), ddpm((e.flags & NATINF_NCSNPP_DDPM) != 0), NUM_RES(ddpm ? 2 : 4), res_scale(ddpm ? 1.0f : INV_SQRT2) {
        arena.keep = (e.flags & NATINF_NCSNPP_KEEP_ACTIVATIONS) != 0;
    }

    void op(int cls, OpFn f) { E.ops.push_back(std::move(f)); E.op_cls.push_back(cls); }
    int64_t wres(int64_t bytes) { const int64_t o = wtop; wtop += align_up(bytes, 256); return o; }
    int64_t take(int64_t n) { const int64_t o = poff; poff += n; return o; }

    void pack_conv(int64_t src, int64_t dst, int N, int Cin, int taps, int dst_ld, int koff, int tapstride, float wmul = 1.0f) {
        const int chunked = taps == 9 && Cin % BK == 0;
        E.packs.push_back([=](const PackCtx& p) {
            const int64_t n = (int64_t)N * Cin * taps;
            hipLaunchKernelGGL(k_pack_conv, dim3(grid1d(n, 256, 1 << 30)), dim3(256), 0, p.stream, p.params + src,
                               reinterpret_cast<bf16*>(p.packed + dst), N, Cin, taps, dst_ld, koff, tapstride, chunked, wmul);
        });
    }
    void pack_frag(int64_t src_packed, int64_t dst, int N, int ld, int cin, int c1) {
        E.packs.push_back([=](const PackCtx& p) {
            const int64_t n = (int64_t)(N / 16) * (9 * (cin / 32) + c1 / 32) * 64;
            hipLaunchKernelGGL(k_pack_frag, dim3(grid1d(n, 256, 1 << 30)), dim3(256), 0, p.stream, reinterpret_cast<const bf16*>(p.packed + src_packed),
                               reinterpret_cast<bf16*>(p.packed + dst), N, ld, cin, c1);
        });
    }
    void pack_transpose(int64_t src, int64_t dst, int K, int N, int dst_ld) {
        E.packs.push_back([=](const PackCtx& p) {
            hipLaunchKernelGGL(k_pack_transpose, dim3(grid1d((int64_t)K * N, 256, 1 << 30)), dim3(256), 0, p.stream,
                               p.params + src, reinterpret_cast<bf16*>(p.packed + dst), K, N, dst_ld);
        });
    }
    void pack_transpose_at(int64_t src, int64_t dst_bytes, int K, int N, int dst_ld) { pack_transpose(src, dst_bytes, K, N, dst_ld); }
    void pack_zero(int64_t dst, int64_t n) {
        E.packs.push_back([=](const PackCtx& p) {
            hipLaunchKernelGGL(k_fill_bf16_zero, dim3(grid1d(n, 256, 1 << 30)), dim3(256), 0, p.stream,
                               reinterpret_cast<bf16*>(p.packed + dst), n);
        });
    }
    int64_t pack_f32(int64_t src, int n, int64_t src2 = -1) {
        const int64_t dst = wres((int64_t)n * 4);
        pack_f32_at(src, n, dst, src2);
        return dst;
    }
    void pack_f32_at(int64_t src, int n, int64_t dst, int64_t src2 = -1) {
        E.packs.push_back([=](const PackCtx& p) {
            hipLaunchKernelGGL(k_copy_add_f32, dim3(grid1d(n)), dim3(256), 0, p.stream, p.params + src,
                               src2 >= 0 ? p.params + src2 : nullptr, reinterpret_cast<float*>(p.packed + dst), n);
        });
    }

    struct GN { int64_t gamma, beta; };
    GN take_gn(int C) { GN g; g.gamma = pack_f32(take(C), C); g.beta = pack_f32(take(C), C); return g; }

    void emit_gn_stats(const TRef& x, GN gn, int64_t& sc, int64_t& sh, float out_mul = 1.0f) {
        if (emit_gn_from_parts(x, gn, sc, sh, out_mul)) return;
        const int HW = x.res * x.res;
        op(CLS_OTHER, [=](const Ctx& c) {
            hipLaunchKernelGGL(k_gn_stats, dim3(c.B), dim3(256), 0, c.stream, c.act(x), x.ld, x.C, HW,
                               c.w<float>(gn.gamma), c.w<float>(gn.beta), c.at<float>(sc), c.at<float>(sh), GN_EPS, out_mul);
        });
    }
    void emit_gn_apply(const TRef& x, int64_t sc, int64_t sh, const TRef& y, const TRef* xr, int act, int mode) {
        const int logW = ilog2(x.res), logHW = 2 * logW;
        const int rd = mode == RS_UP ? 2 * x.res : (mode == RS_DOWN ? x.res / 2 : x.res);
        const int rows_per_img = rd + 2 * y.pad;
        const TRef xrr = xr ? *xr : TRef();
        op(CLS_OTHER, [=](const Ctx& c) {
            hipLaunchKernelGGL(k_gn_apply, dim3((unsigned)((rows_per_img + GN_ROWS - 1) / GN_ROWS), (unsigned)c.B), dim3(256), 0, c.stream, c.act(x), x.ld, x.C,
                               logW, logHW, c.at<float>(sc), c.at<float>(sh), c.act(y),
                               xrr.off >= 0 ? c.act(xrr) : (bf16*)nullptr, act, mode, y.pad);
        });
    }
    TRef new_act(int res, int C, int pad = 0) {
        TRef t; t.off = arena.alloc((int64_t)(res + 2 * pad) * (res + 2 * pad) * C * 2); t.C = C; t.ld = C; t.res = res; t.pad = pad;
        return t;
    }

    void emit_res(const Mod& m, const TRef& x, const TRef& out) {
        const int cin = m.cin, cout = m.cout;
        const int ro = m.up ? m.res * 2 : (m.down ? m.res / 2 : m.res);
        const bool shortcut = cin != cout || m.up || m.down;
        const GN gn0 = take_gn(cin);
        const int64_t p_c0w = take((int64_t)cout * cin * 9), p_c0b = take(cout);
        const int64_t p_dw = take((int64_t)cout * TEMB), p_db = take(cout);
        const GN gn1 = take_gn(cout);
        const int64_t p_c1w = take((int64_t)cout * cout * 9), p_c1b = take(cout);
        const int64_t p_c2w = shortcut ? take((int64_t)cout * cin) : -1, p_c2b = shortcut ? take(cout) : -1;

        const int K0a = 9 * cin, K1tot = 9 * cout + (shortcut ? cin : 0);
        const bool fusable_res = g_fuse_gn && (ro == 32 || ro == 16 || (ro == 8 && g_fuse_gn8 && cout % 256 == 0) || (ro == 4 && g_fuse_gn4 && cout % 256 == 0));
        const bool fuse1 = fusable_res && cout % BK == 0;
        const bool fuse_up = fuse1 && ro > 8 && g_fuse_up && m.up && cin % BK == 0 && cout % 128 == 0;
        const bool fuse = (fusable_res && !m.up && !m.down && cin % BK == 0) || fuse_up;
        const float LOG2E = 1.4426950408889634f, LN2 = 0.6931471805599453f;
        const float gn_mul = fuse ? -LOG2E : 1.0f, w_mul = fuse ? -LN2 : 1.0f, gn_mul1 = fuse1 ? -LOG2E : 1.0f, w_mul1 = fuse1 ? -LN2 : 1.0f;
        const int64_t w0 = wres((int64_t)cout * K0a * 2), w1 = wres((int64_t)cout * K1tot * 2);
        pack_conv(p_c0w, w0, cout, cin, 9, K0a, 0, cin, w_mul);
        pack_conv(p_c1w, w1, cout, cout, 9, K1tot, 0, cout, w_mul1);
        if (shortcut && !ddpm) pack_conv(p_c2w, w1, cout, cin, 1, K1tot, 9 * cout, cin);
        if (shortcut && ddpm) pack_transpose_at(p_c2w, w1 + (int64_t)9 * cout * 2, cin, cout, K1tot);
        const int64_t w0f = (fuse && cout % 16 == 0) ? wres((int64_t)cout * K0a * 2) : -1, w1f = (fuse1 && cout % 16 == 0) ? wres((int64_t)cout * K1tot * 2) : -1;
        if (w0f >= 0) pack_frag(w0, w0f, cout, K0a, cin, 0);
        if (w1f >= 0) pack_frag(w1, w1f, cout, K1tot, cout, shortcut ? cin : 0);
        const int64_t b0 = pack_f32(p_c0b, cout), b1 = pack_f32(p_c1b, cout, shortcut ? p_c2b : -1);
        const int drow = dense_rows_next;
        pack_conv(p_dw, dense_w + (int64_t)drow * TEMB * 2, cout, TEMB, 1, TEMB, 0, TEMB);
        pack_f32_at(p_db, cout, dense_b + (int64_t)drow * 4);
        dense_rows_next += cout;

        const int64_t own_sc = arena.alloc((int64_t)std::max(cin, cout) * 4), own_sh = arena.alloc((int64_t)std::max(cin, cout) * 4);
        int64_t sc = own_sc, sh = own_sh;
        emit_gn_stats(x, gn0, sc, sh, gn_mul);
        TRef h, xr;
        if (!fuse) {
            h = new_act(ro, cin, 1);
            if (m.up || m.down) xr = new_act(ro, cin);
            emit_gn_apply(x, sc, sh, h, (m.up || m.down) ? &xr : nullptr, ACT_SILU, m.up ? RS_UP : (m.down ? RS_DOWN : RS_NONE));
        }

        const int SK_MAX = 4;
        const int64_t skws = (ro <= 8) ? arena.alloc((int64_t)SK_MAX * ro * ro * cout * 4) : -1;
        TRef t = new_act(ro, cout);
        const Part pt = register_output(t, fuse);
        const int logW = ilog2(ro), logHW = 2 * logW, HWo = ro * ro;
        const int dtotal = dense_total; const int64_t dout = dense_out;
        op(fuse ? (ro <= 8 ? CLS_CONV_GN8 : CLS_CONV_GN) : CLS_GEMM, [=](const Ctx& c) {
            GemmArgs g = gemm_defaults();
            if (fuse) { g.a0 = c.act(x); g.a0_ld = x.ld; g.gn_scale = c.at<float>(sc); g.gn_shift = c.at<float>(sh); g.gn_ld = cin; g.gn_folded = 1; g.a0_up = fuse_up; }
            else { g.a0 = c.act(h); g.a0_ld = h.ld; g.a0_padded = 1; }
            g.a0_C = cin; g.taps = 9; g.logW = logW; g.logHW = logHW;
            g.M = c.B * HWo; g.N = cout; g.b = c.w<bf16>(w0); g.b_ld = K0a;
            if (w0f >= 0) g.b_frag = c.w<bf16>(w0f);
            g.bias_n = c.w<float>(b0);
            g.rowvec = c.at<float>(dout) + drow; g.rowvec_ld = dtotal; g.log_rows_per_sample = logHW;
            if (skws >= 0) { g.splitk_ws = c.at<float>(skws); g.splitk_max = SK_MAX; }
            g.c = c.act(t); g.c_ld = t.ld;
            if (pt.valid) { g.gn_part = c.at<float>(pt.off); g.gn_quads = pt.quads; set_fin(g, pt, c); }
            g_fin_written = false;
            const int bm = launch_gemm(g, c.stream);
            if (pt.valid) c.part_bm[pt.id] = bm;
            if (pt.fin && pt.fin->check) c.fin_done[pt.id] = g_fin_written;
        });
        if (!fuse) arena.release(h.off);
        int64_t sc1 = own_sc, sh1 = own_sh;
        emit_gn_stats(t, gn1, sc1, sh1, gn_mul1);
        TRef u;
        if (!fuse1) {
            u = new_act(ro, cout, 1);
            emit_gn_apply(t, sc1, sh1, u, nullptr, ACT_SILU, RS_NONE);
            arena.release(t.off);
        }
        if (pt.valid) arena.release(pt.off);
        const TRef xs = ((m.up || m.down) && !fuse_up) ? xr : x;
        const float rs = res_scale;
        const Part po = register_output(out, fuse1);
        op(fuse1 ? (ro <= 8 ? CLS_CONV_GN8 : CLS_CONV_GN) : CLS_GEMM, [=](const Ctx& c) {
            GemmArgs g = gemm_defaults();
            if (fuse1) { g.a0 = c.act(t); g.a0_ld = t.ld; g.gn_scale = c.at<float>(sc1); g.gn_shift = c.at<float>(sh1); g.gn_ld = cout; g.gn_folded = 1; }
            else { g.a0 = c.act(u); g.a0_ld = u.ld; g.a0_padded = 1; }
            g.a0_C = cout; g.taps = 9; g.logW = logW; g.logHW = logHW;
            if (shortcut) { g.a1 = c.act(xs); g.a1_ld = xs.ld; g.a1_C = cin; g.a1_up = fuse_up; }
            else { g.resid = c.act(xs); g.resid_ld = xs.ld; }
            g.M = c.B * HWo; g.N = cout; g.b = c.w<bf16>(w1); g.b_ld = K1tot;
            if (w1f >= 0) g.b_frag = c.w<bf16>(w1f);
            g.bias_n = c.w<float>(b1); g.scale = rs;
            if (skws >= 0) { g.splitk_ws = c.at<float>(skws); g.splitk_max = SK_MAX; }
            g.c = c.act(out); g.c_ld = out.ld;
            if (po.valid) { g.gn_part = c.at<float>(po.off); g.gn_quads = po.quads; set_fin(g, po, c); }
            g_fin_written = false;
            const int bm = launch_gemm(g, c.stream);
            if (po.valid) c.part_bm[po.id] = bm;
            if (po.fin && po.fin->check) c.fin_done[po.id] = g_fin_written;
        });
        if (skws >= 0) arena.release(skws);
        if (fuse1) arena.release(t.off); else arena.release(u.off);
        if ((m.up || m.down) && !fuse_up) arena.release(xr.off);
        arena.release(own_sc); arena.release(own_sh);
        if (sc != own_sc) { arena.release(sc); arena.release(sh); }
        if (sc1 != own_sc) { arena.release(sc1); arena.release(sh1); }
        E.taps[m.idx] = out;
    }

    void emit_attn(const Mod& m, const TRef& x, const TRef& out) {
        const int C = m.cin, T = m.res * m.res;
        const GN gn = take_gn(C);
        int64_t pw[4], pb[4];
        for (int i = 0; i < 4; ++i) { pw[i] = take((int64_t)C * C); pb[i] = take(C); }
        const int64_t wqk = wres((int64_t)2 * C * C * 2), wv = wres((int64_t)C * C * 2), w3 = wres((int64_t)C * C * 2);
        pack_transpose(pw[0], wqk, C, C, C);
        pack_transpose(pw[1], wqk + (int64_t)C * C * 2, C, C, C);
        pack_transpose(pw[2], wv, C, C, C);
        pack_transpose(pw[3], w3, C, C, C);
        const int64_t bqk = wres((int64_t)2 * C * 4);
        pack_f32_at(pb[0], C, bqk); pack_f32_at(pb[1], C, bqk + (int64_t)C * 4);
        const int64_t bv = pack_f32(pb[2], C), b3 = pack_f32(pb[3], C);

        const int64_t own_sc = arena.alloc((int64_t)C * 4), own_sh = arena.alloc((int64_t)C * 4);
        int64_t sc = own_sc, sh = own_sh;
        emit_gn_stats(x, gn, sc, sh);
        const bool fuse_qkv = T == 256 && C == 256 && g_attn_qkv;
        TRef h = new_act(m.res, C);
        if (!fuse_qkv) emit_gn_apply(x, sc, sh, h, nullptr, ACT_NONE, RS_NONE);
        const int64_t qk = arena.alloc((int64_t)T * 2 * C * 2), vT = arena.alloc((int64_t)C * T * 2);
        const bool blk = fuse_qkv && g_attn256 && g_attn_proj && g_attn_w8 && g_attn_blk;
        int64_t wqkvf = -1;
        const int64_t sc_q = sc, sh_q = sh;
        if (fuse_qkv) {
            wqkvf = wres((int64_t)3 * C * C * 2);
            const int64_t s0 = pw[0], s1 = pw[1], s2 = pw[2];
            E.packs.push_back([=](const PackCtx& p) {
                hipLaunchKernelGGL(k_pack_qkv_w, dim3(3 * 256), dim3(256), 0, p.stream, p.params + s0, p.params + s1, p.params + s2, reinterpret_cast<bf16*>(p.packed + wqkvf));
            });
            const int64_t sc_ = sc, sh_ = sh;
            if (!blk)
            op(CLS_GEMM, [=](const Ctx& c) {
                if (g_record) return;
                hipLaunchKernelGGL(k_qkv256, dim3((unsigned)c.B), dim3(512), QKV_LDS_BYTES, c.stream, (const bf16*)c.act(x), x.ld, c.at<float>(sc_), c.at<float>(sh_),
                                   c.w<bf16>(wqkvf), c.w<float>(bqk), c.w<float>(bv), c.at<bf16>(qk), c.at<bf16>(vT));
            });
        }
        if (!fuse_qkv)
        op(CLS_GEMM, [=](const Ctx& c) {
            GemmArgs g = gemm_defaults();
            g.a0 = c.act(h); g.a0_ld = C; g.a0_C = C; g.M = c.B * T; g.N = 2 * C;
            g.b = c.w<bf16>(wqk); g.b_ld = C; g.bias_n = c.w<float>(bqk);
            g.c = c.at<bf16>(qk); g.c_ld = 2 * C;
            launch_gemm(g, c.stream);
        });
        if (!fuse_qkv)
        op(CLS_GEMM, [=](const Ctx& c) {
            GemmArgs g = gemm_defaults();
            g.a0 = c.w<bf16>(wv); g.a0_ld = C; g.a0_C = C; g.a_bs = 0; g.M = C; g.N = T;
            g.b = c.act(h); g.b_ld = C; g.b_bs = (int64_t)T * C; g.bias_m = c.w<float>(bv);
            g.c = c.at<bf16>(vT); g.c_ld = T; g.c_bs = (int64_t)C * T; g.batch = c.B;
            launch_gemm(g, c.stream);
        });
        arena.release(h.off);
        const bool proj = T == 256 && C == 256 && g_attn256 && g_attn_proj;
        int64_t w3f = -1;
        if (proj) {
            w3f = wres((int64_t)C * C * 2);
            const int64_t src = pw[3];
            E.packs.push_back([=](const PackCtx& p) {
                hipLaunchKernelGGL(k_pack_attn_w3, dim3(256), dim3(256), 0, p.stream, p.params + src, reinterpret_cast<bf16*>(p.packed + w3f));
            });
        }
        const bool blk2 = blk && g_attn_blk == 2;
        int64_t wqf2 = -1, wvof2 = -1, cq2 = -1, bo2 = -1;
        if (blk2) {
            const int64_t fq = wres((int64_t)C * C * 4), fv = wres((int64_t)C * C * 4);
            cq2 = wres((int64_t)C * 4); bo2 = wres((int64_t)C * 4);
            wqf2 = wres((int64_t)C * C * 2); wvof2 = wres((int64_t)C * C * 2);
            const int64_t w0_ = pw[0], w1_ = pw[1], w2_ = pw[2], w3_ = pw[3], b0_ = pb[0], b2_ = pb[2], b3_ = pb[3], cq_ = cq2, bo_ = bo2, wq_ = wqf2, wv_ = wvof2;
            E.packs.push_back([=](const PackCtx& p) {
                float* fqp = reinterpret_cast<float*>(p.packed + fq); float* fvp = reinterpret_cast<float*>(p.packed + fv);
                hipLaunchKernelGGL(k_attn_fold_w, dim3(257), dim3(256), 0, p.stream, p.params + w0_, p.params + w1_, p.params + w2_, p.params + w3_, p.params + b0_, p.params + b2_,
                                   p.params + b3_, fqp, reinterpret_cast<float*>(p.packed + cq_), fvp, reinterpret_cast<float*>(p.packed + bo_));
                hipLaunchKernelGGL(k_pack_qkv_w, dim3(256), dim3(256), 0, p.stream, (const float*)fqp, (const float*)fqp, (const float*)fqp, reinterpret_cast<bf16*>(p.packed + wq_), 1);
                hipLaunchKernelGGL(k_pack_attn_w3, dim3(256), dim3(256), 0, p.stream, (const float*)fvp, reinterpret_cast<bf16*>(p.packed + wv_));
            });
        }
        const Part po_attn = proj ? register_output(out) : Part();
        const float rs_attn = res_scale;
        TRef O = new_act(m.res, C);
        if (T == 256 && C == 256) {
            op(CLS_GEMM, [=](const Ctx& c) {
                if (g_record) return;
                if (blk2) {
                    hipLaunchKernelGGL(k_attn_blk256_v2, dim3((unsigned)c.B), dim3(512), ABLK2_LDS_BYTES, c.stream, (const bf16*)c.act(x), x.ld, c.at<float>(sc_q), c.at<float>(sh_q),
                                       c.w<bf16>(wqf2), c.w<float>(cq2), 1.0f / sqrtf((float)C), c.w<bf16>(wvof2), c.w<float>(bo2),
                                       c.act(out), out.ld, rs_attn, po_attn.valid ? c.at<float2>(po_attn.off) : (float2*)nullptr, po_attn.quads);
                    if (po_attn.valid) c.part_bm[po_attn.id] = 256;
                } else if (blk) {
                    hipLaunchKernelGGL(k_attn_blk256, dim3((unsigned)c.B), dim3(512), ABLK_LDS_BYTES, c.stream, (const bf16*)c.act(x), x.ld, c.at<float>(sc_q), c.at<float>(sh_q),
                                       c.w<bf16>(wqkvf), c.w<float>(bqk), c.w<float>(bv), c.at<bf16>(qk), c.at<bf16>(vT), 1.0f / sqrtf((float)C), c.w<bf16>(w3f), c.w<float>(b3),
                                       c.act(out), out.ld, rs_attn, po_attn.valid ? c.at<float2>(po_attn.off) : (float2*)nullptr, po_attn.quads);
                    if (po_attn.valid) c.part_bm[po_attn.id] = 256;
                } else if (proj) {
                    if (g_attn_w8) {
                        hipLaunchKernelGGL((k_attn256<true, 8>), dim3((unsigned)c.B), dim3(512), A256_LDS_BYTES, c.stream, c.at<bf16>(qk), 2 * C, C, c.at<bf16>(vT), c.act(out), out.ld,
                                           1.0f / sqrtf((float)C), c.w<bf16>(w3f), c.w<float>(b3), (const bf16*)c.act(x), x.ld, rs_attn,
                                           po_attn.valid ? c.at<float2>(po_attn.off) : (float2*)nullptr, po_attn.quads);
                        if (po_attn.valid) c.part_bm[po_attn.id] = 256;
                    } else {
                    hipLaunchKernelGGL(k_attn256<true>, dim3((unsigned)(2 * c.B)), dim3(256), A256_LDS_BYTES, c.stream, c.at<bf16>(qk), 2 * C, C, c.at<bf16>(vT), c.act(out), out.ld,
                                       1.0f / sqrtf((float)C), c.w<bf16>(w3f), c.w<float>(b3), (const bf16*)c.act(x), x.ld, rs_attn,
                                       po_attn.valid ? c.at<float2>(po_attn.off) : (float2*)nullptr, po_attn.quads);
                    if (po_attn.valid) c.part_bm[po_attn.id] = 128;
                    }
                }
                else if (g_attn256)
                    hipLaunchKernelGGL(k_attn256<false>, dim3((unsigned)(2 * c.B)), dim3(256), A256_LDS_BYTES, c.stream, c.at<bf16>(qk), 2 * C, C, c.at<bf16>(vT), c.act(O), C,
                                       1.0f / sqrtf((float)C), (const bf16*)nullptr, (const float*)nullptr, (const bf16*)nullptr, 0, 1.0f, (float2*)nullptr, 0);
#ifdef NATINF_DEV
                else {
                    using Cfg = AttnCfg<8, 16, true>;
                    hipLaunchKernelGGL((&k_attn_fused<8, 16, true>), dim3((unsigned)c.B), dim3(Cfg::THREADS), Cfg::LDS_BYTES, c.stream, c.at<bf16>(qk), 2 * C, C,
                                       c.at<bf16>(vT), c.act(O), C, 1, C, 1.0f / sqrtf((float)C));
                }
#endif
            });
            arena.release(vT); arena.release(qk);
        } else {
        const int64_t S = arena.alloc((int64_t)T * T * 4);
            op(CLS_GEMM, [=](const Ctx& c) {
                GemmArgs g = gemm_defaults();
                g.a0 = c.at<bf16>(qk); g.a0_ld = 2 * C; g.a0_C = C; g.a_bs = (int64_t)T * 2 * C; g.M = T; g.N = T;
                g.b = c.at<bf16>(qk) + C; g.b_ld = 2 * C; g.b_bs = (int64_t)T * 2 * C;
                g.scale = 1.0f / sqrtf((float)C);
                g.c = c.at<float>(S); g.c_ld = T; g.c_bs = (int64_t)T * T; g.c_mode = OUT_F32; g.batch = c.B;
                launch_gemm(g, c.stream);
            });
            const int64_t P = arena.alloc((int64_t)T * T * 2);
            op(CLS_OTHER, [=](const Ctx& c) {
                const int64_t rows = (int64_t)c.B * T;
                hipLaunchKernelGGL(k_softmax_rows, dim3((unsigned)((rows + 3) / 4)), dim3(256), 0, c.stream,
                                   c.at<float>(S), c.at<bf16>(P), T, rows);
            });
            arena.release(S);
            op(CLS_GEMM, [=](const Ctx& c) {
                GemmArgs g = gemm_defaults();
                g.a0 = c.at<bf16>(P); g.a0_ld = T; g.a0_C = T; g.a_bs = (int64_t)T * T; g.M = T; g.N = C;
                g.b = c.at<bf16>(vT); g.b_ld = T; g.b_bs = (int64_t)C * T;
                g.c = c.act(O); g.c_ld = C; g.c_bs = (int64_t)T * C; g.batch = c.B;
                launch_gemm(g, c.stream);
            });
            arena.release(P); arena.release(vT); arena.release(qk);
        }
        if (proj) {
            arena.release(O.off); arena.release(own_sc); arena.release(own_sh);
            if (sc != own_sc) { arena.release(sc); arena.release(sh); }
            E.taps[m.idx] = out;
            return;
        }
        const Part po = register_output(out);
        const float rs = res_scale;
        op(CLS_GEMM, [=](const Ctx& c) {
            GemmArgs g = gemm_defaults();
            g.a0 = c.act(O); g.a0_ld = C; g.a0_C = C; g.M = c.B * T; g.N = C;
            g.b = c.w<bf16>(w3); g.b_ld = C; g.bias_n = c.w<float>(b3);
            g.resid = c.act(x); g.resid_ld = x.ld; g.scale = rs;
            g.c = c.act(out); g.c_ld = out.ld;
            if (po.valid) { g.gn_part = c.at<float>(po.off); g.gn_quads = po.quads; }
            const int bm = launch_gemm(g, c.stream);
            if (po.valid) c.part_bm[po.id] = bm;
        });
        arena.release(O.off); arena.release(own_sc); arena.release(own_sh);
        if (sc != own_sc) { arena.release(sc); arena.release(sh); }
        E.taps[m.idx] = out;
    }

    void emit_downconv(const Mod& m, const TRef& x, const TRef& out) {
        const int C = m.cin, ro = m.res / 2, Kd = 9 * C;
        const int64_t pw = take((int64_t)C * C * 9), pb = take(C);
        const int64_t w = wres((int64_t)C * Kd * 2);
        E.packs.push_back([=](const PackCtx& p) {
            const int64_t n = (int64_t)C * C * 9;
            hipLaunchKernelGGL(k_pack_conv, dim3(grid1d(n, 256, 1 << 30)), dim3(256), 0, p.stream, p.params + pw, reinterpret_cast<bf16*>(p.packed + w), C, C, 9, Kd, 0, C, 0, 1.0f);
        });
        const int64_t b = pack_f32(pb, C);
        const int64_t col = arena.alloc((int64_t)ro * ro * Kd * 2);
        const Part po = register_output(out);
        const int rin = m.res;
        op(CLS_GEMM, [=](const Ctx& c) {
            const int64_t M = (int64_t)c.B * ro * ro;
            if (!g_record) {
                const int64_t total = M * (Kd / 8);
                hipLaunchKernelGGL(k_inc_im2col, dim3(grid1d(total, 256, 1 << 30)), dim3(256), 0, c.stream, c.act(x), rin, rin, x.ld, C, 3, 3, 2, 0, 0, ro, ro, Kd,
                                   c.at<bf16>(col), total);
            }
            GemmArgs g = gemm_defaults();
            g.a0 = c.at<bf16>(col); g.a0_ld = Kd; g.a0_C = Kd; g.M = (int)M; g.N = C; g.b = c.w<bf16>(w); g.b_ld = Kd; g.bias_n = c.w<float>(b);
            g.log_rows_per_sample = 2 * ilog2(ro); g.logHW = 2 * ilog2(ro); g.logW = ilog2(ro);
            g.c = c.act(out); g.c_ld = out.ld;
            if (po.valid) { g.gn_part = c.at<float>(po.off); g.gn_quads = po.quads; }
            const int bm = launch_gemm(g, c.stream);
            if (po.valid) c.part_bm[po.id] = bm;
        });
        arena.release(col);
        E.taps[m.idx] = out;
    }
    int64_t ident_sc = -1, ident_sh = -1;
    void emit_upconv(const Mod& m, const TRef& x, const TRef& out) {
        const int C = m.cin, ro = m.res * 2, Ku = 9 * C;
        const int64_t pw = take((int64_t)C * C * 9), pb = take(C);
        const int64_t w = wres((int64_t)C * Ku * 2);
        pack_conv(pw, w, C, C, 9, Ku, 0, C);
        const int64_t b = pack_f32(pb, C);
        if (ident_sc < 0) {
            ident_sc = arena.alloc((int64_t)2 * NF * 4); ident_sh = arena.alloc((int64_t)2 * NF * 4);
            const int64_t isc = ident_sc, ish = ident_sh;
            op(CLS_OTHER, [=](const Ctx& c) {
                const int64_t n = (int64_t)c.B * 2 * NF;
                hipLaunchKernelGGL(k_fill_f32, dim3(grid1d(n, 256, 1 << 30)), dim3(256), 0, c.stream, c.at<float>(isc), 1.0f, n);
                hipLaunchKernelGGL(k_fill_f32, dim3(grid1d(n, 256, 1 << 30)), dim3(256), 0, c.stream, c.at<float>(ish), 0.0f, n);
            });
        }
        TRef u = new_act(ro, C, 1);
        emit_gn_apply(x, ident_sc, ident_sh, u, nullptr, ACT_NONE, RS_UP);
        const Part po = register_output(out);
        const int logW = ilog2(ro);
        op(CLS_GEMM, [=](const Ctx& c) {
            GemmArgs g = gemm_defaults();
            g.a0 = c.act(u); g.a0_ld = u.ld; g.a0_C = C; g.taps = 9; g.logW = logW; g.logHW = 2 * logW; g.a0_padded = 1;
            g.M = c.B * ro * ro; g.N = C; g.b = c.w<bf16>(w); g.b_ld = Ku; g.bias_n = c.w<float>(b); g.log_rows_per_sample = 2 * logW;
            g.c = c.act(out); g.c_ld = out.ld;
            if (po.valid) { g.gn_part = c.at<float>(po.off); g.gn_quads = po.quads; }
            const int bm = launch_gemm(g, c.stream);
            if (po.valid) c.part_bm[po.id] = bm;
        });
        arena.release(u.off);
        E.taps[m.idx] = out;
    }

    int dense_rows_next = 0;

    struct Fin { int64_t sc = -1, sh = -1, gamma = -1, beta = -1; int C = 0; float out_mul = 1.0f; bool claimed = false, check = false; };
    struct Part { int64_t off = -1; int quads = 0, id = -1, res = 0; bool valid = false; std::shared_ptr<Fin> fin; };
    static void set_fin(GemmArgs& g, const Part& p, const Ctx& c) {
        if (!p.fin || !p.fin->claimed) return;
        const Fin& f = *p.fin;
        g.fin_scale = c.at<float>(f.sc); g.fin_shift = c.at<float>(f.sh); g.fin_gamma = c.w<float>(f.gamma); g.fin_beta = c.w<float>(f.beta);
        g.fin_ld = f.C; g.fin_cg = f.C / 32; g.fin_mul = f.out_mul; g.fin_eps = GN_EPS;
    }
    std::map<std::pair<int64_t, int>, Part> parts;
    int n_parts = 0;
    static bool fusable(int res) { return res >= 16; }
    Part new_part(int res, int C) {
        Part p; p.quads = C / 4; p.res = res; p.id = n_parts++; p.valid = true;
        p.off = arena.alloc((int64_t)std::max(res * res / 64, 1) * p.quads * 8);
        return p;
    }
    Part register_output(const TRef& out, bool fused8 = false) {
        Part p;
        if (fusable(out.res) || (out.res <= 8 && fused8)) p = new_part(out.res, out.C);
        if (p.valid && out.res <= 8 && fused8 && (g_fuse_fin & 1) && out.C == 256) {
            p.fin = std::make_shared<Fin>();
            p.fin->sc = arena.alloc((int64_t)out.C * 4); p.fin->sh = arena.alloc((int64_t)out.C * 4); p.fin->C = out.C;
        }
        if (p.valid && out.res == 16 && fused8 && (g_fuse_fin & 2) && out.C == 256 && !ddpm) {
            p.fin = std::make_shared<Fin>();
            p.fin->sc = arena.alloc((int64_t)out.C * 4); p.fin->sh = arena.alloc((int64_t)out.C * 4); p.fin->C = out.C; p.fin->check = true;
        }
        parts[{out.off, out.coff}] = p;
        return p;
    }
    bool emit_gn_from_parts(const TRef& x, GN gn, int64_t& sc, int64_t& sh, float out_mul) {
        std::vector<Part> src;
        int ch = 0;
        while (ch < x.C) {
            auto it = parts.find({x.off, x.coff + ch});
            if (it == parts.end() || !it->second.valid || it->second.res != x.res) return false;
            src.push_back(it->second);
            ch += it->second.quads * 4;
        }
        if (ch != x.C || src.empty() || src.size() > 2) return false;
        const Part p0 = src[0], p1 = src.size() > 1 ? src[1] : Part();
        const int HW = x.res * x.res, C = x.C;
        if (src.size() == 1 && p0.fin && !p0.fin->claimed && p0.fin->C == C) {
            Fin& f = *p0.fin;
            f.gamma = gn.gamma; f.beta = gn.beta; f.out_mul = out_mul; f.claimed = true;
            sc = f.sc; sh = f.sh;
            if (f.check) {
                const std::shared_ptr<Fin> fp = p0.fin;
                const int64_t fsc = f.sc, fsh = f.sh;
                op(CLS_OTHER, [=](const Ctx& c) {
                    if (c.fin_done[p0.id]) return;
                    hipLaunchKernelGGL(k_gn_finalize, dim3(c.B), dim3(256), 0, c.stream, c.at<float2>(p0.off), HW / c.part_bm[p0.id], p0.quads, (const float2*)nullptr, 0, 0, C, HW,
                                       c.w<float>(gn.gamma), c.w<float>(gn.beta), c.at<float>(fsc), c.at<float>(fsh), GN_EPS, out_mul);
                });
            }
            return true;
        }
        const int64_t sc_ = sc, sh_ = sh;
        op(CLS_OTHER, [=](const Ctx& c) {
            const int tps0 = HW / c.part_bm[p0.id], tps1 = p1.valid ? HW / c.part_bm[p1.id] : 0;
            hipLaunchKernelGGL(k_gn_finalize, dim3(c.B), dim3(256), 0, c.stream, c.at<float2>(p0.off), tps0, p0.quads,
                               p1.valid ? c.at<float2>(p1.off) : (const float2*)nullptr, tps1, p1.valid ? p1.quads : 0, C, HW,
                               c.w<float>(gn.gamma), c.w<float>(gn.beta), c.at<float>(sc_), c.at<float>(sh_), GN_EPS, out_mul);
        });
        return true;
    }

    void list_modules() {
        auto add = [&](int kind, int cin, int cout, int up, int down, int res) {
            Mod m; m.idx = (int)E.mods.size(); m.kind = kind; m.cin = cin; m.cout = cout; m.up = up; m.down = down; m.res = res; m.poff = 0;
            E.mods.push_back(m);
        };
        add(K_LIN, NF, TEMB, 0, 0, 0); add(K_LIN, TEMB, TEMB, 0, 0, 0); add(K_CONV, 3, NF, 0, 0, IMG);
        std::vector<int> skip = {NF};
        int ch = NF, res = IMG;
        for (int l = 0; l < NLEVEL; ++l) {
            for (int b = 0; b < NUM_RES; ++b) {
                add(K_RES, ch, NF * CH_MULT[l], 0, 0, res); ch = NF * CH_MULT[l];
                if (attn_at(res)) add(K_ATTN, ch, ch, 0, 0, res);
                skip.push_back(ch);
            }
            if (l != NLEVEL - 1) { if (ddpm) add(K_DOWN, ch, ch, 0, 0, res); else add(K_RES, ch, ch, 0, 1, res); res /= 2; skip.push_back(ch); }
        }
        add(K_RES, ch, ch, 0, 0, res); add(K_ATTN, ch, ch, 0, 0, res); add(K_RES, ch, ch, 0, 0, res);
        for (int l = NLEVEL - 1; l >= 0; --l) {
            for (int b = 0; b < NUM_RES + 1; ++b) { add(K_RES, ch + skip.back(), NF * CH_MULT[l], 0, 0, res); skip.pop_back(); ch = NF * CH_MULT[l]; }
            if (attn_at(res)) add(K_ATTN, ch, ch, 0, 0, res);
            if (l != 0) { if (ddpm) add(K_UP, ch, ch, 0, 0, res); else add(K_RES, ch, ch, 1, 0, res); res *= 2; }
        }
        add(K_GN, ch, ch, 0, 0, res); add(K_CONV, ch, 3, 0, 0, res);
    }

    void build() {
        list_modules();
        auto& M = E.mods;
        struct Cat { TRef buf; int ch_h, ch_s; };
        std::vector<Cat> cats;
        std::vector<int> skip_ch, skip_res;
        {
            int ch = NF, res = IMG; skip_ch.push_back(NF); skip_res.push_back(IMG);
            for (int l = 0; l < NLEVEL; ++l) {
                for (int b = 0; b < NUM_RES; ++b) { ch = NF * CH_MULT[l]; skip_ch.push_back(ch); skip_res.push_back(res); }
                if (l != NLEVEL - 1) { res /= 2; skip_ch.push_back(ch); skip_res.push_back(res); }
            }
            int sp = (int)skip_ch.size();
            for (int l = NLEVEL - 1; l >= 0; --l) {
                for (int b = 0; b < NUM_RES + 1; ++b) {
                    --sp;
                    Cat c; c.ch_h = ch; c.ch_s = skip_ch[sp];
                    c.buf = new_act(res, c.ch_h + c.ch_s);
                    cats.push_back(c);
                    ch = NF * CH_MULT[l];
                }
                if (l != 0) res *= 2;
            }
        }
        const int P = (int)skip_ch.size();
        auto skip_slot = [&](int i) { const Cat& c = cats[P - 1 - i]; TRef t = c.buf; t.C = c.ch_s; t.coff = c.ch_h; return t; };
        auto h_slot = [&](int j) { const Cat& c = cats[j]; TRef t = c.buf; t.C = c.ch_h; t.coff = 0; return t; };

        for (auto& m : M) if (m.kind == K_RES) dense_total += m.cout;
        dense_w = wres((int64_t)dense_total * TEMB * 2); dense_b = wres((int64_t)dense_total * 4);
        dense_out = arena.alloc((int64_t)dense_total * 4);
        const int64_t emb = arena.alloc(128 * 2), t1 = arena.alloc(TEMB * 2), t2 = arena.alloc(TEMB * 2);

        size_t mi = 0;
        {
            const Mod& m0 = M[mi++]; const Mod& m1 = M[mi++]; (void)m0; (void)m1;
            const int64_t pw0 = take((int64_t)TEMB * NF), pb0 = take(TEMB), pw1 = take((int64_t)TEMB * TEMB), pb1 = take(TEMB);
            const int64_t w0 = wres((int64_t)TEMB * NF * 2), w1 = wres((int64_t)TEMB * TEMB * 2);
            pack_conv(pw0, w0, TEMB, NF, 1, NF, 0, NF); pack_conv(pw1, w1, TEMB, TEMB, 1, TEMB, 0, TEMB);
            const int64_t b0 = pack_f32(pb0, TEMB), b1 = pack_f32(pb1, TEMB);
            const int64_t dw = dense_w, db = dense_b, dout = dense_out; const int dtot = dense_total;
            op(CLS_OTHER, [=](const Ctx& c) {
                hipLaunchKernelGGL(k_time_embed, dim3(grid1d((int64_t)c.B * 128)), dim3(256), 0, c.stream, c.labels, c.at<bf16>(emb), c.B);
            });
            op(CLS_GEMM, [=](const Ctx& c) {
                GemmArgs g = gemm_defaults();
                g.a0 = c.at<bf16>(emb); g.a0_ld = NF; g.a0_C = NF; g.M = c.B; g.N = TEMB;
                g.b = c.w<bf16>(w0); g.b_ld = NF; g.bias_n = c.w<float>(b0); g.act = ACT_SILU;
                g.c = c.at<bf16>(t1); g.c_ld = TEMB;
                launch_gemm(g, c.stream);
                g = gemm_defaults();
                g.a0 = c.at<bf16>(t1); g.a0_ld = TEMB; g.a0_C = TEMB; g.M = c.B; g.N = TEMB;
                g.b = c.w<bf16>(w1); g.b_ld = TEMB; g.bias_n = c.w<float>(b1); g.act = ACT_SILU;
                g.c = c.at<bf16>(t2); g.c_ld = TEMB;
                launch_gemm(g, c.stream);
                g = gemm_defaults();
                g.a0 = c.at<bf16>(t2); g.a0_ld = TEMB; g.a0_C = TEMB; g.M = c.B; g.N = dtot;
                g.b = c.w<bf16>(dw); g.b_ld = TEMB; g.bias_n = c.w<float>(db);
                g.c = c.at<float>(dout); g.c_ld = dtot; g.c_mode = OUT_F32;
                launch_gemm(g, c.stream);
            });
        }
        int si = 0;
        TRef cur = skip_slot(si++);
        {
            const Mod& m = M[mi++];
            const int64_t pw = take((int64_t)NF * 27), pb = take(NF);
            const int64_t w = wres((int64_t)NF * 64 * 2);
            pack_zero(w, (int64_t)NF * 64);
            pack_conv(pw, w, NF, 3, 9, 64, 0, 3);
            const int64_t b = pack_f32(pb, NF);
            const int64_t a0 = arena.alloc((int64_t)IMG * IMG * 64 * 2);
            const TRef dst = cur;
            const Part po = register_output(dst);
            op(CLS_OTHER, [=](const Ctx& c) {
                const int64_t rows = (int64_t)c.B * IMG * IMG;
                hipLaunchKernelGGL(k_stem_im2col, dim3((unsigned)((rows * 8 + 255) / 256)), dim3(256), 0, c.stream, c.x, c.at<bf16>(a0), rows);
            });
            op(CLS_GEMM, [=](const Ctx& c) {
                const int64_t rows = (int64_t)c.B * IMG * IMG;
                GemmArgs g = gemm_defaults();
                g.a0 = c.at<bf16>(a0); g.a0_ld = 64; g.a0_C = 64; g.M = (int)rows; g.N = NF;
                g.b = c.w<bf16>(w); g.b_ld = 64; g.bias_n = c.w<float>(b);
                g.c = c.act(dst); g.c_ld = dst.ld;
                if (po.valid) { g.gn_part = c.at<float>(po.off); g.gn_quads = po.quads; }
                const int bm = launch_gemm(g, c.stream);
                if (po.valid) c.part_bm[po.id] = bm;
            });
            arena.release(a0);
            E.taps[m.idx] = dst;
        }
        int res = IMG;
        for (int l = 0; l < NLEVEL; ++l) {
            for (int b = 0; b < NUM_RES; ++b) {
                const Mod& m = M[mi++];
                const TRef dst = skip_slot(si++);
                if (attn_at(res)) {
                    TRef tmp = new_act(res, m.cout);
                    emit_res(m, cur, tmp);
                    emit_attn(M[mi++], tmp, dst);
                    arena.release(tmp.off);
                } else {
                    emit_res(m, cur, dst);
                }
                cur = dst;
            }
            if (l != NLEVEL - 1) {
                const Mod& m = M[mi++];
                const TRef dst = skip_slot(si++);
                if (ddpm) emit_downconv(m, cur, dst); else emit_res(m, cur, dst);
                cur = dst; res /= 2;
            }
        }
        {
            TRef a = new_act(res, cur.C), b = new_act(res, cur.C);
            emit_res(M[mi++], cur, a);
            emit_attn(M[mi++], a, b);
            arena.release(a.off);
            emit_res(M[mi++], b, h_slot(0));
            arena.release(b.off);
        }
        int j = 0;
        TRef last;
        for (int l = NLEVEL - 1; l >= 0; --l) {
            for (int b = 0; b < NUM_RES + 1; ++b) {
                const Mod& m = M[mi++];
                const bool level_end = b == NUM_RES;
                TRef in = cats[j].buf;
                TRef dst = level_end ? new_act(res, m.cout) : h_slot(j + 1);
                emit_res(m, in, dst);
                arena.release(cats[j].buf.off);
                last = dst; ++j;
            }
            if (attn_at(res)) {
                TRef dst = new_act(res, last.C);
                emit_attn(M[mi++], last, dst);
                arena.release(last.off);
                last = dst;
            }
            if (l != 0) {
                const Mod& m = M[mi++];
                if (ddpm) emit_upconv(m, last, h_slot(j)); else emit_res(m, last, h_slot(j));
                arena.release(last.off);
                res *= 2;
            }
        }
        {
            const Mod& mg = M[mi++]; const Mod& mc = M[mi++];
            const GN gn = take_gn(mg.cin);
            const int64_t pw = take((int64_t)3 * mc.cin * 9), pb = take(3);
            const int Kf = 9 * mc.cin;
            const int64_t w = wres((int64_t)3 * Kf * 2);
            pack_conv(pw, w, 3, mc.cin, 9, Kf, 0, mc.cin);
            const int64_t b = pack_f32(pb, 3);
            int64_t sc = arena.alloc((int64_t)mg.cin * 4), sh = arena.alloc((int64_t)mg.cin * 4);
            const int logW = ilog2(res), cinf = mc.cin;
            if (g_fuse_head && res == HeadConvCfg::RES && mc.cin == HeadConvCfg::C) {
                const int64_t w16 = wres((int64_t)16 * Kf * 2);
                pack_zero(w16, (int64_t)16 * Kf);
                pack_conv(pw, w16, 3, mc.cin, 9, Kf, 0, mc.cin, -0.6931471805599453f);
                emit_gn_stats(last, gn, sc, sh, -1.4426950408889634f);
                const TRef src = last;
                op(CLS_GEMM, [=](const Ctx& c) {
                    if (g_record) {
                        char line[160];
                        snprintf(line, sizeof(line), "%d %d %d %d %d %d head_conv/e0\n", c.B * res * res, 3, Kf, 0, 9, 1);
                        *g_record += line;
                        return;
                    }
                    hipLaunchKernelGGL(k_head_conv, dim3((unsigned)(c.B * (HeadConvCfg::RES / HeadConvCfg::ROWS))), dim3(256), HeadConvCfg::LDS_BYTES, c.stream,
                                       c.act(src), src.ld, c.at<float>(sc), c.at<float>(sh), c.w<bf16>(w16), c.w<float>(b), c.out);
                });
            } else {
            emit_gn_stats(last, gn, sc, sh);
            TRef u = new_act(res, mg.cin, 1);
            emit_gn_apply(last, sc, sh, u, nullptr, ACT_SILU, RS_NONE);
            op(CLS_GEMM, [=](const Ctx& c) {
                GemmArgs g = gemm_defaults();
                g.a0 = c.act(u); g.a0_ld = u.ld; g.a0_C = cinf; g.taps = 9; g.logW = logW; g.logHW = 2 * logW; g.a0_padded = 1;
                g.M = c.B * res * res; g.N = 3; g.b = c.w<bf16>(w); g.b_ld = Kf; g.bias_n = c.w<float>(b);
                g.c = c.out; g.c_mode = OUT_F32_NCHW;
                launch_gemm(g, c.stream);
            });
            }
            E.taps[mg.idx] = last;
        }
        E.n_params = poff;
        E.part_bm.assign(n_parts > 0 ? n_parts : 1, 128);
        E.fin_done.assign(n_parts > 0 ? n_parts : 1, 0);
        E.ws_per_image = arena.peak;
        E.packed_bytes = wtop;
    }
};

int64_t module_param_count(const Mod& m) {
    switch (m.kind) {
        case K_LIN: return (int64_t)m.cout * m.cin + m.cout;
        case K_CONV: return (int64_t)m.cout * m.cin * 9 + m.cout;
        case K_GN: return 2 * (int64_t)m.cin;
        case K_DOWN: case K_UP: return (int64_t)m.cout * m.cin * 9 + m.cout;
        case K_ATTN: return 2 * (int64_t)m.cin + 4 * ((int64_t)m.cin * m.cin + m.cin);
        case K_RES: {
            int64_t n = 2 * (int64_t)m.cin + (int64_t)m.cout * m.cin * 9 + m.cout + (int64_t)m.cout * TEMB + m.cout +
                        2 * (int64_t)m.cout + (int64_t)m.cout * m.cout * 9 + m.cout;
            if (m.cin != m.cout || m.up || m.down) n += (int64_t)m.cout * m.cin + m.cout;
            return n;
        }
    }
    return 0;
}

natinf_ncsnpp* make_engine(int flags) {
    natinf_ncsnpp* e = new natinf_ncsnpp();
    e->flags = flags;
    Builder b(*e);
    b.build();
    int64_t off = 0;
    for (auto& m : e->mods) { m.poff = off; off += module_param_count(m); }
    if (off != e->n_params) { delete e; return nullptr; }
    return e;
}

const natinf_ncsnpp& reference_engine() {
    static natinf_ncsnpp* e = [] {
        int* knobs[] = {&g_fuse_gn, &g_fuse_up, &g_fuse_head, &g_fuse_gn8, &g_fuse_gn4, &g_fuse_fin, &g_attn_qkv, &g_attn_proj, &g_attn256};
        int saved[sizeof(knobs) / sizeof(knobs[0])];
        for (size_t i = 0; i < sizeof(knobs) / sizeof(knobs[0]); ++i) { saved[i] = *knobs[i]; *knobs[i] = 1; }
        g_fuse_fin = 3;
        natinf_ncsnpp* r = make_engine(0);
        for (size_t i = 0; i < sizeof(knobs) / sizeof(knobs[0]); ++i) *knobs[i] = saved[i];
        return r;
    }();
    return *e;
}

}

extern "C" {

int64_t natinf_ncsnpp_param_count(void) { return reference_engine().n_params; }
int64_t natinf_ncsnpp_packed_bytes(void) { return reference_engine().packed_bytes; }

int64_t natinf_ncsnpp_handle_param_count(natinf_ncsnpp_t h) { return h ? h->n_params : NATINF_EINVAL; }
int64_t natinf_ncsnpp_handle_packed_bytes(natinf_ncsnpp_t h) { return h ? h->packed_bytes : NATINF_EINVAL; }

int64_t natinf_ncsnpp_workspace_bytes(natinf_ncsnpp_t h, int max_batch) {
    if (!h || max_batch <= 0) return NATINF_EINVAL;
    return h->ws_per_image * (int64_t)max_batch;
}

static uint64_t plan_signature() {
    const int k[] = {g_fuse_head, g_cg8_tm4, g_attn_qkv, g_attn_w8, g_attn_proj, g_attn256, g_fuse_gn8, g_fuse_fin, g_fuse_gn4, g_fuse_gn, g_cg_wide, g_fuse_up, g_cg_regw,
                     g_attn_blk , g_cg3 };
    uint64_t h = 1469598103934665603ull;
    for (int v : k) h = (h ^ (uint64_t)(v & 0xff)) * 1099511628211ull;
    return h;
}

int natinf_ncsnpp_create(natinf_ncsnpp_t* out, int flags) {
    if (!out || (flags & ~(NATINF_NCSNPP_KEEP_ACTIVATIONS | NATINF_NCSNPP_DDPM))) return NATINF_EINVAL;
    natinf_ncsnpp* e = make_engine(flags);
    if (!e) return NATINF_ESTATE;
    e->plan_sig = plan_signature();
    *out = e;
    return NATINF_OK;
}

int natinf_ncsnpp_destroy(natinf_ncsnpp_t h) {
    if (!h) return NATINF_EINVAL;
    for (auto& r : h->recs) { (void)hipEventDestroy(r.a); (void)hipEventDestroy(r.b); }
    for (auto e : h->pool) (void)hipEventDestroy(e);
    delete h;
    return NATINF_OK;
}

int natinf_ncsnpp_describe(natinf_ncsnpp_t h, char* buf, int cap) {
    if (!h || !buf || cap <= 0) return NATINF_EINVAL;
    std::string s;
    char line[160];
    for (const auto& m : h->mods) {
        snprintf(line, sizeof(line), "%d %s %d %d %d %d %d %lld\n", m.idx, kind_name(m.kind), m.cin, m.cout, m.up, m.down, m.res,
                 (long long)m.poff);
        s += line;
    }
    if ((int)s.size() + 1 > cap) return NATINF_EINVAL;
    memcpy(buf, s.c_str(), s.size() + 1);
    return (int)s.size();
}

int natinf_ncsnpp_load(natinf_ncsnpp_t h, const float* params_f32, int64_t n_params, void* packed, int64_t packed_bytes,
                       natinf_stream_t stream) {
    if (!h || !params_f32 || !packed || n_params != h->n_params || packed_bytes < h->packed_bytes) return NATINF_EINVAL;
    PackCtx p{params_f32, reinterpret_cast<unsigned char*>(packed), (hipStream_t)stream};
    for (const auto& f : h->packs) f(p);
    h->packed = reinterpret_cast<const unsigned char*>(packed);
    return hipGetLastError() == hipSuccess ? NATINF_OK : NATINF_ELAUNCH;
}

int natinf_ncsnpp_share(natinf_ncsnpp_t h, natinf_ncsnpp_t loaded) {
    if (!h || !loaded || h == loaded) return NATINF_EINVAL;
    if (!loaded->packed) return NATINF_ESTATE;
    if ((h->flags & NATINF_NCSNPP_DDPM) != (loaded->flags & NATINF_NCSNPP_DDPM) || h->n_params != loaded->n_params || h->packed_bytes != loaded->packed_bytes ||
        h->packs.size() != loaded->packs.size() || h->plan_sig != loaded->plan_sig)
        return NATINF_EINVAL;
    h->packed = loaded->packed;
    return NATINF_OK;
}

int natinf_ncsnpp_forward(natinf_ncsnpp_t h, const float* x, const float* labels, float* out, int B, void* workspace,
                          int64_t workspace_bytes, natinf_stream_t stream) {
    if (!h || !x || !labels || !out || !workspace || B <= 0) return NATINF_EINVAL;
    if (!h->packed) return NATINF_ESTATE;
    if (workspace_bytes < h->ws_per_image * (int64_t)B || (int64_t)B * IMG * IMG >= (1LL << 31)) return NATINF_EINVAL;
    if (!h->attr_set) {
        if (!configure_gemm_kernels()) return NATINF_ENODEV;
        h->attr_set = true;
    }
    Ctx c{B, reinterpret_cast<unsigned char*>(workspace), h->packed, (hipStream_t)stream, x, labels, out, h->part_bm.data()};
    c.fin_done = h->fin_done.data();
    g_launch_error = 0;
    if (!h->prof) {
        for (const auto& f : h->ops) f(c);
    } else {
        for (size_t i = 0; i < h->ops.size(); ++i) {
            natinf_ncsnpp::Rec r; r.cls = h->op_cls[i];
            for (hipEvent_t* e : {&r.a, &r.b}) {
                if (!h->pool.empty()) { *e = h->pool.back(); h->pool.pop_back(); }
                else if (hipEventCreate(e) != hipSuccess) return NATINF_ELAUNCH;
            }
            (void)hipEventRecord(r.a, c.stream);
            h->ops[i](c);
            (void)hipEventRecord(r.b, c.stream);
            h->recs.push_back(r);
        }
    }
    h->last_B = B; h->last_ws = c.ws;
    if (g_launch_error) { g_launch_error = 0; return NATINF_ESTATE; }
    return hipGetLastError() == hipSuccess ? NATINF_OK : NATINF_ELAUNCH;
}

int natinf_ncsnpp_describe_gemms(natinf_ncsnpp_t h, int B, char* buf, int cap) {
    if (!h || !buf || cap <= 0 || B <= 0) return NATINF_EINVAL;
    std::string out;
    g_record = &out;
    std::vector<int> scratch_bm(h->part_bm.size(), 128);
    std::vector<unsigned char> scratch_done(h->part_bm.size(), 0);
    Ctx c{B, reinterpret_cast<unsigned char*>(4096), reinterpret_cast<const unsigned char*>(4096), nullptr, nullptr, nullptr, nullptr, scratch_bm.data()};
    c.fin_done = scratch_done.data();
    for (size_t i = 0; i < h->ops.size(); ++i)
        if (h->op_cls[i] == CLS_GEMM || h->op_cls[i] == CLS_CONV_GN || h->op_cls[i] == CLS_CONV_GN8) h->ops[i](c);
    g_record = nullptr;
    if ((int)out.size() + 1 > cap) return NATINF_EINVAL;
    memcpy(buf, out.c_str(), out.size() + 1);
    return (int)out.size();
}

int natinf_debug_gemm(int variant, int M, int N, int K0, int K1, int taps, int logW, int batch,
                      const void* a0, const void* a1, const void* b, const float* bias_n, void* c, int c_f32, float scale,
                      int iters, natinf_stream_t stream) {
    if (variant < 0 || variant >= V_COUNT || !a0 || !b || !c || M <= 0 || N <= 0 || iters <= 0 || (taps != 1 && taps != 9)) return NATINF_EINVAL;
    if (!variant_shipped(variant) || variant == V_CONV_GN || variant == V_FP8_256x256) return NATINF_ESTATE;
#ifndef NATINF_DEV
    if (c_f32 >= 2) return NATINF_ESTATE;
#endif
    static bool configured = false;
    if (!configured) { if (!configure_gemm_kernels()) return NATINF_ENODEV; configured = true; }
    GemmArgs g = gemm_defaults();
    g.a0 = (const bf16*)a0; g.a0_C = K0 / taps; g.a0_ld = g.a0_C; g.taps = taps; g.logW = logW; g.logHW = 2 * logW; g.a0_padded = taps == 9;
    if (a1) { g.a1 = (const bf16*)a1; g.a1_C = K1; g.a1_ld = K1; }
    g.M = M; g.N = N; g.b = (const bf16*)b; g.b_ld = K0 + (a1 ? K1 : 0); g.batch = batch;
    if (batch > 1) { g.a_bs = (int64_t)M * g.a0_ld; g.b_bs = (int64_t)N * g.b_ld; g.c_bs = (int64_t)M * N; }
    g.bias_n = bias_n; g.scale = scale; g.c = c; g.c_ld = N; g.c_mode = c_f32 == 1 ? OUT_F32 : (c_f32 >= 2 ? 100 + c_f32 : OUT_BF16);
    g.dbg_ts = g_dbg_ts;
    g.splitk_ws = g_dbg_splitk_ws; g.splitk_max = g_dbg_splitk_max;
    const int saved = g_force_variant;
    g_force_variant = variant;
    for (int i = 0; i < iters; ++i) launch_gemm(g, (hipStream_t)stream);
    g_force_variant = saved;
    return hipGetLastError() == hipSuccess ? NATINF_OK : NATINF_ELAUNCH;
}

int natinf_debug_gemm_fused(int variant, int M, int N, int K, const void* a, const void* b, const float* bias_n, const float* bias_m,
                            const float* rowvec, const float* gate, int log_rows_per_sample, const void* resid_bf16, const float* resid_f32,
                            float scale, int act, void* c, int c_f32, float* gn_part, int* bm_out, int fp32_slab, natinf_stream_t stream) {
    if (variant < 0 || variant >= V_COUNT || !a || !b || !c || M <= 0 || N <= 0 || K <= 0 || N % 8) return NATINF_EINVAL;
    if (!variant_shipped(variant) || variant == V_CONV_GN || variant == V_FP8_256x256) return NATINF_ESTATE;
    if (!configure_gemm_kernels()) return NATINF_ENODEV;
    GemmArgs g = gemm_defaults();
    g.a0 = (const bf16*)a; g.a0_C = K; g.a0_ld = K; g.M = M; g.N = N; g.b = (const bf16*)b; g.b_ld = K;
    g.bias_n = bias_n; g.bias_m = bias_m; g.rowvec = rowvec; g.rowvec_ld = N; g.gate = gate; g.gate_ld = N; g.log_rows_per_sample = log_rows_per_sample;
    g.resid = (const bf16*)resid_bf16; g.resid_ld = N; g.resid_f32 = resid_f32; g.resid_f32_ld = N;
    g.scale = scale; g.act = act; g.c = c; g.c_ld = N; g.c_mode = c_f32 ? OUT_F32 : OUT_BF16;
    g.gn_part = gn_part; g.gn_quads = N / 4; g.epi_fp32_slab = fp32_slab != 0;
    g.splitk_ws = g_dbg_splitk_ws; g.splitk_max = g_dbg_splitk_max;
    g.dbg_ts = g_dbg_ts;
    const int saved = g_force_variant;
    g_force_variant = variant;
    const int bm = launch_gemm(g, (hipStream_t)stream);
    g_force_variant = saved;
    if (bm_out) *bm_out = bm;
    return hipGetLastError() == hipSuccess ? NATINF_OK : NATINF_ELAUNCH;
}

int g_dbg_cg_up = 0;
int natinf_debug_conv_gn_up(int flags) { if (flags & ~3) return NATINF_EINVAL; g_dbg_cg_up = flags; return NATINF_OK; }
int natinf_debug_conv_gn(int res, int B, int N, int cin, int c1, const void* x, const float* scale, const float* shift, const void* w_packed,
                         void* w_frag, const void* a1, const float* bias_n, const void* resid, float out_scale, void* out, float* gn_part, int iters,
                         natinf_stream_t stream) {
    if ((res != 32 && res != 16 && res != 8 && res != 4) || B <= 0 || N <= 0 || N % 8 || cin <= 0 || cin % 64 || c1 < 0 || c1 % 64 || (c1 > 0) != (a1 != nullptr) ||
        !x || !scale || !shift || !w_packed || !out || iters <= 0) return NATINF_EINVAL;
    static bool configured = false;
    if (!configured) { if (!configure_gemm_kernels()) return NATINF_ENODEV; configured = true; }
    GemmArgs g = gemm_defaults();
    g.a0 = (const bf16*)x; g.a0_ld = cin; g.a0_C = cin; g.taps = 9; g.logW = ilog2(res); g.logHW = 2 * g.logW;
    g.gn_scale = scale; g.gn_shift = shift; g.gn_ld = cin; g.gn_folded = 1;
    if (a1) { g.a1 = (const bf16*)a1; g.a1_ld = c1; g.a1_C = c1; }
    g.M = B * res * res; g.N = N; g.b = (const bf16*)w_packed; g.b_ld = 9 * cin + c1; g.bias_n = bias_n;
    g.resid = (const bf16*)resid; g.resid_ld = N; g.scale = out_scale; g.c = out; g.c_ld = N;
    g.gn_part = gn_part; g.gn_quads = N / 4;
    g.dbg_ts = g_dbg_ts;
    g.a0_up = g_dbg_cg_up & 1; g.a1_up = (a1 && (g_dbg_cg_up & 2)) ? 1 : 0;
    if (w_frag && N % 16 == 0) g.b_frag = (const bf16*)w_frag;
    if (!conv_gn_ok(g)) return NATINF_EINVAL;
    if (g.b_frag) {
        const int64_t n = (int64_t)(N / 16) * (9 * (cin / 32) + c1 / 32) * 64;
        hipLaunchKernelGGL(k_pack_frag, dim3(grid1d(n, 256, 1 << 30)), dim3(256), 0, (hipStream_t)stream, (const bf16*)w_packed, (bf16*)w_frag, N, g.b_ld, cin, c1);
    }
    for (int i = 0; i < iters; ++i) launch_gemm(g, (hipStream_t)stream);
    return hipGetLastError() == hipSuccess ? NATINF_OK : NATINF_ELAUNCH;
}

int natinf_debug_quant_fp8_rows(const float* w, void* q, float* row_scale, int rows, int cols, natinf_stream_t stream) {
    if (!w || !q || !row_scale || rows <= 0 || cols <= 0 || cols % 2) return NATINF_EINVAL;
    hipLaunchKernelGGL(k_pack_fp8_rows, dim3((unsigned)((rows + 3) / 4)), dim3(256), 0, (hipStream_t)stream, w, (uint8_t*)q, row_scale, rows, cols);
    return hipGetLastError() == hipSuccess ? NATINF_OK : NATINF_ELAUNCH;
}

int natinf_debug_gemm_fp8(int M, int N, int K, const void* a8, const float* a_scale, const void* a_mx, const void* b8, const float* b_scale,
                          const float* bias_n, void* c, void* c_mx, int c_mode, int iters, natinf_stream_t stream) {
    if (!a8 || !b8 || !c || M <= 0 || N <= 0 || K <= 0 || K % 128 || N % 8 || iters <= 0) return NATINF_EINVAL;
    static bool configured = false;
    if (!configured) { if (!configure_gemm_kernels()) return NATINF_ENODEV; configured = true; }
    GemmArgs g = gemm_defaults();
    g.a0 = (const bf16*)a8; g.a0_C = K; g.a0_ld = K; g.M = M; g.N = N; g.b = (const bf16*)b8; g.b_ld = K;
    const int act = c_mode >> 8; c_mode &= 0xff;
    if (act != ACT_NONE && act != ACT_GELU_TANH) return NATINF_EINVAL;
    g.deq_m = a_scale; g.deq_n = b_scale; g.bias_n = bias_n; g.c = c; g.c_ld = N; g.c_mode = c_mode; g.act = act;
    g.a_mx = (const uint8_t*)a_mx; g.a_mx_ld = M; g.c_mx = (uint8_t*)c_mx; g.c_mx_ld = M;
    if ((c_mode == OUT_FP8_MX && (!c_mx || N % 32)) || c_mode < 0 || c_mode > OUT_FP8_MX || c_mode == OUT_F32_NCHW) return NATINF_EINVAL;
    for (int i = 0; i < iters; ++i) launch_gemm_fp8(g, (hipStream_t)stream);
    return hipGetLastError() == hipSuccess ? NATINF_OK : NATINF_ELAUNCH;
}

int natinf_debug_timestamps(void* dev_buf16) {
#ifdef NATINF_DEV
    g_dbg_ts = reinterpret_cast<unsigned long long*>(dev_buf16); return NATINF_OK;
#else
    (void)dev_buf16; return NATINF_ESTATE;
#endif
}

int natinf_set_gemm_raster(int rows) { g_raster_g = rows; return NATINF_OK; }
int natinf_set_fuse_gn(int on) { g_fuse_gn = on != 0; return NATINF_OK; }
int natinf_set_fuse_gn8(int on) { g_fuse_gn8 = on != 0; return NATINF_OK; }
int natinf_set_attn256(int on) {
#ifndef NATINF_DEV
    if (!on) return NATINF_ESTATE;
#endif
    g_attn256 = on != 0; return NATINF_OK;
}
int natinf_set_conv_gn_warm(int mask) { if (mask < 0 || mask > 15) return NATINF_EINVAL; g_cg_warm = mask; return NATINF_OK; }
int natinf_set_attn_block(int on) { g_attn_blk = on < 0 ? ATTN_BLK_DEFAULT : (on > 2 ? 2 : on); return NATINF_OK; }
int natinf_set_attn_qkv(int on) { g_attn_qkv = on != 0; return NATINF_OK; }
int natinf_set_attn_waves8(int on) { g_attn_w8 = on != 0; return NATINF_OK; }
int natinf_set_attn_proj(int on) { g_attn_proj = on != 0; return NATINF_OK; }
int natinf_set_fuse_fin(int on) {
    if (on < 0 || on > 3) return NATINF_EINVAL;
    static const int mask[4] = {0, 3, 1, 2};
    g_fuse_fin = mask[on];
    return NATINF_OK;
}
int natinf_set_gemm_round_model(int on) { g_round_model = on != 0; g_round_model_w128 = on >= 10 ? on : 13; return NATINF_OK; }
int natinf_set_gemm_w128(int on) { g_w128 = on < 0 ? 0 : (on > 2 ? 2 : on); return NATINF_OK; }
int natinf_set_fuse_gn4(int on) { g_fuse_gn4 = on != 0; return NATINF_OK; }
int natinf_set_conv_gn8_tile(int one_image) {
#ifndef NATINF_DEV
    if (!one_image) return NATINF_ESTATE;
#endif
    g_cg8_tm4 = one_image != 0; return NATINF_OK;
}
int natinf_set_fuse_head(int on) { g_fuse_head = on != 0; return NATINF_OK; }
int natinf_set_conv_gn_w128(int mask) { if (mask < 0 || mask > 7) return NATINF_EINVAL; g_cg3 = mask; return NATINF_OK; }
int natinf_set_conv_gn_w128_min_k(int shape, int k) { if (shape < 0 || shape > 2 || k < 0) return NATINF_EINVAL; g_cg3_min_k[shape] = k; return NATINF_OK; }
int natinf_set_conv_gn_wide(int mask) { if (mask < 0 || mask > 3) return NATINF_EINVAL; g_cg_wide = mask; return NATINF_OK; }
int natinf_set_conv_gn_regw(int on) {
    if (!on && !HAVE_CONV_GN_V1) return NATINF_ESTATE;
    g_cg_regw = on != 0; return NATINF_OK;
}
int natinf_set_fuse_up(int on) { g_fuse_up = on != 0; return NATINF_OK; }
int natinf_set_gemm_splitk(int on) { g_splitk = on != 0; return NATINF_OK; }
int natinf_debug_set_splitk_workspace(float* ws, int max_slices) { g_dbg_splitk_ws = ws; g_dbg_splitk_max = ws ? max_slices : 0; return NATINF_OK; }
int natinf_set_gemm_half_issue(int on) {
#ifndef NATINF_DEV
    if (!on) return NATINF_ESTATE;
#endif
    g_half_issue = on != 0; return NATINF_OK;
}
int natinf_set_gemm_pref512(int on) { g_pref_512 = on != 0; return NATINF_OK; }
int natinf_set_gemm_epilogue(int fp32_slab) { g_epi_fp32_slab = fp32_slab != 0; return NATINF_OK; }

int natinf_set_gemm_variant(int variant) {
    if (variant < 0 || variant >= V_COUNT) return NATINF_EINVAL;
    if (!variant_shipped(variant) || variant == V_CONV_GN || variant == V_FP8_256x256) return NATINF_ESTATE;
    g_force_variant = variant;
    return NATINF_OK;
}

int natinf_gemm_profile(int enable) { g_gemm_prof.on = enable != 0; return NATINF_OK; }
int natinf_gemm_profile_read(char* buf, int cap) {
    if (!buf || cap <= 0) return NATINF_EINVAL;
    std::map<std::string, std::pair<double, int64_t>> by;
    std::vector<std::string> order;
    int rc = NATINF_OK;
    for (auto& e : g_gemm_prof.ev) {
        float ms = 0.f;
        if (hipEventSynchronize(e.b) != hipSuccess || hipEventElapsedTime(&ms, e.a, e.b) != hipSuccess) { (void)hipGetLastError(); rc = NATINF_ELAUNCH; }
        else {
            auto it = by.find(e.tag);
            if (it == by.end()) { order.push_back(e.tag); it = by.emplace(e.tag, std::make_pair(0.0, (int64_t)0)).first; }
            it->second.first += ms; it->second.second += 1;
        }
        g_gemm_prof.pool.emplace_back(e.a, e.b);
    }
    g_gemm_prof.ev.clear();
    if (rc != NATINF_OK) return rc;
    std::string out;
    for (auto& t : order) {
        char tail[64];
        snprintf(tail, sizeof(tail), " %lld %.6f\n", (long long)by[t].second, by[t].first);
        out += t + tail;
    }
    if ((int)out.size() + 1 > cap) return NATINF_EINVAL;
    memcpy(buf, out.c_str(), out.size() + 1);
    return (int)out.size();
}
int natinf_ncsnpp_profile(natinf_ncsnpp_t h, int enable) {
    if (!h) return NATINF_EINVAL;
    h->prof = enable != 0;
    return NATINF_OK;
}

int natinf_ncsnpp_profile_read(natinf_ncsnpp_t h, double* ms_by_class, int64_t* launches_by_class) {
    if (!h || !ms_by_class || !launches_by_class) return NATINF_EINVAL;
    for (int i = 0; i < N_CLS; ++i) { ms_by_class[i] = 0.0; launches_by_class[i] = 0; }
    for (const auto& r : h->recs) {
        float ms = 0.f;
        if (hipEventSynchronize(r.b) != hipSuccess || hipEventElapsedTime(&ms, r.a, r.b) != hipSuccess) {
            (void)hipGetLastError();
            return NATINF_ELAUNCH;
        }
        ms_by_class[r.cls] += ms; launches_by_class[r.cls] += 1;
        h->pool.push_back(r.a); h->pool.push_back(r.b);
    }
    h->recs.clear();
    return NATINF_OK;
}

int natinf_ncsnpp_debug_tap(natinf_ncsnpp_t h, int module_idx, float* out, int64_t capacity_elems, natinf_stream_t stream) {
    if (!h || !out) return NATINF_EINVAL;
    if (!(h->flags & NATINF_NCSNPP_KEEP_ACTIVATIONS) || !h->last_ws) return NATINF_ESTATE;
    auto it = h->taps.find(module_idx);
    if (it == h->taps.end()) return NATINF_EINVAL;
    const TRef& t = it->second;
    const int HW = t.res * t.res;
    const int64_t total = (int64_t)h->last_B * t.C * HW;
    if (capacity_elems < total) return NATINF_EINVAL;
    const bf16* src = reinterpret_cast<const bf16*>(h->last_ws + t.off * h->last_B) + t.coff;
    hipLaunchKernelGGL(k_nhwc_to_nchw_f32, dim3(grid1d(total, 256, 1 << 30)), dim3(256), 0, (hipStream_t)stream, src, t.ld, t.C, HW, out, total);
    return hipGetLastError() == hipSuccess ? NATINF_OK : NATINF_ELAUNCH;
}

}
#include "dit_engine.inc"
#include "mmdit_engine.inc"
#include "vae_engine.inc"
#include "inception_engine.inc"
```

Before: 3453 images/s.

## Extend conv_gn3 pipelined kernel to 8x8 resolution with two-image tiles

Adds an 8x8-resolution variant of the fully scheduled conv+GroupNorm kernel. Each 128-row tile covers two whole images, and the four waves split a 256-column block as quarters (TN=4). The variant adds dual GroupNorm tables, per-image patch placement, a weight-fragment warm-up prefetch, and a fused final epilogue. It is enabled by default for 8x8 convs with N divisible by 256. This is meant to replace the slower regw conv_gn2 path at the lowest resolution, at the cost of more complex scheduling and a risk of partial-tile handling bugs when batch rows are not a multiple of two images.

```diff
diff --git a/include/natinf_ncsnpp.h b/include/natinf_ncsnpp.h
--- a/include/natinf_ncsnpp.h
+++ b/include/natinf_ncsnpp.h
@@ -58,6 +58,7 @@
 int natinf_set_conv_gn_wide(int mask);
 int natinf_set_conv_gn_w128(int mask);
 int natinf_set_conv_gn_w128_min_k(int shape, int k);
+int natinf_set_conv_gn_w128_lowres(int mask);
 int natinf_set_conv_gn_regw(int on);
 int natinf_set_fuse_up(int on);
 int natinf_set_fuse_head(int on);
diff --git a/naturaldiffusion_amd/_lib.py b/naturaldiffusion_amd/_lib.py
--- a/naturaldiffusion_amd/_lib.py
+++ b/naturaldiffusion_amd/_lib.py
@@ -63,6 +63,7 @@
     "natinf_set_attn_block": (C.c_int, [_i32]),
     "natinf_set_conv_gn_w128": (C.c_int, [_i32]),
     "natinf_set_conv_gn_w128_min_k": (C.c_int, [_i32, _i32]),
+    "natinf_set_conv_gn_w128_lowres": (C.c_int, [_i32]),
     "natinf_set_conv_gn_regw": (C.c_int, [_i32]),
     "natinf_set_fuse_up": (C.c_int, [_i32]),
     "natinf_set_fuse_head": (C.c_int, [_i32]),
diff --git a/naturaldiffusion_amd/csrc/conv_gn3.h b/naturaldiffusion_amd/csrc/conv_gn3.h
--- a/naturaldiffusion_amd/csrc/conv_gn3.h
+++ b/naturaldiffusion_amd/csrc/conv_gn3.h
@@ -5,38 +5,43 @@
 
 template <int RES, int WM_, int WN_>
 struct ConvGn3Cfg {
-    static_assert(WM_ * WN_ == 4 && (RES == 32 || RES == 16), "four waves; 32x32 / 16x16 images");
+    static_assert(WM_ * WN_ == 4 && (RES == 32 || RES == 16 || (RES == 8 && WM_ == 1)), "four waves; 32x32 / 16x16 images, or two 8x8 images x four column quarters");
     static constexpr int W = RES, WS = RES + 2, HW = RES * RES, NW = 4, THREADS = 256, KT = 32;
-    static constexpr int WM = WM_, WN = WN_, TM = 8, TN = 8;
-    static constexpr int BM_ = WM_ * 128, BN_ = WN_ * 128;
-    static_assert(HW % BM_ == 0 && BM_ % W == 0, "a tile is whole image rows of one image");
+    static constexpr int WM = WM_, WN = WN_, TM = 8, TN = RES == 8 ? 4 : 8, SL = TM * TN;
+    static constexpr int BM_ = WM_ * 128, BN_ = WN_ * TN * 16;
+    static constexpr int NIMG = HW < BM_ ? BM_ / HW : 1, IMGP = NIMG > 1 ? 128 : 0, WPI = NW / NIMG;
+    static_assert(NIMG == 1 ? (HW % BM_ == 0 && BM_ % W == 0) : (NIMG == 2 && WS * WS <= IMGP && IMGP / 16 == WPI * 4), "a tile is whole image rows of one image, or two whole images");
     static constexpr int PR = BM_ / W + 2, PLAST = PR * WS;
-    static constexpr int NPIECE = (PLAST + 15) / 16, NROUND = (NPIECE + NW - 1) / NW;
+    static constexpr int NPIECE = NIMG > 1 ? NIMG * IMGP / 16 : (PLAST + 15) / 16, NROUND = (NPIECE + NW - 1) / NW;
+    static constexpr int RSTEP = NIMG > 1 ? WPI : NW;
+    static constexpr int piece0(int wave) { return NIMG > 1 ? (wave / WPI) * (IMGP / 16) + wave % WPI : wave; }
     static constexpr int PATCH_BYTES = NROUND * NW * 1024;
-    static constexpr int TAB_BYTES = 256;
+    static constexpr int TAB_IMG_BYTES = 256, TAB_BYTES = NIMG * TAB_IMG_BYTES;
     static constexpr int PSW = BM_ / 16 / NW, SC_BYTES = BM_ * 64;
     static constexpr int OFF_TAB = 2 * PATCH_BYTES, OFF_SC = OFF_TAB + 2 * TAB_BYTES, LOOP_BYTES = OFF_SC + 2 * SC_BYTES;
-    using Epi = EpiCfg<WM_, WN_, 8, 8, 163840>;
-    static constexpr int LDS_BYTES = LOOP_BYTES > Epi::PACK_BYTES ? LOOP_BYTES : Epi::PACK_BYTES;
+    using Epi = EpiCfg<WM_, WN_, TM, TN, 163840>;
+    static constexpr int EPI_BYTES = Epi::PACK_BYTES + (NIMG - 1) * WN * TN * 4 * 8;
+    static constexpr int LDS_BYTES = LOOP_BYTES > EPI_BYTES ? LOOP_BYTES : EPI_BYTES;
     static_assert(Epi::PACK_OK && LDS_BYTES <= 163840, "one block per CU");
-    static constexpr int swz_key(int xx) { return (xx >> 1) & 2; }
-    static constexpr int aoff(int i) { return (RES == 32 ? (i >> 1) * WS + (i & 1) * 16 : i * WS) * 64; }
-    static constexpr int BAR = 40;
+    static constexpr int swz_key(int xx) { return RES == 8 ? (xx & 2) : ((xx >> 1) & 2); }
+    static constexpr int aoff(int i) { return (RES == 32 ? (i >> 1) * WS + (i & 1) * 16 : RES == 16 ? i * WS : (i >> 2) * IMGP + (i & 3) * 2 * WS) * 64; }
+    static constexpr int BAR = SL == 64 ? 40 : 12;
     static constexpr int rd_a(int i) { return 10 + 2 * i; }
     static constexpr int rd_a_late(int i) { return BAR + 2 + 2 * i; }
     static constexpr int dma_sc(int n) { return BAR + 1 + 2 * n; }
-    static_assert(rd_a_late(7) < 64 && dma_sc(PSW - 1) < 64, "inside the step");
+    static constexpr int dma_sc_early(int n) { return 9 + 2 * n; }
+    static_assert(rd_a(7) < SL && rd_a_late(7) < SL && dma_sc(PSW - 1) < SL && dma_sc_early(PSW - 1) < BAR, "inside the step");
     static constexpr int RLEN = 34;
-    static constexpr int G_END = 6 * 64 + BAR - 2;
+    static constexpr int G_END = 6 * SL + BAR - 2;
     static constexpr int STRIDE = (G_END - 1 - RLEN - 2 - 12) / (NROUND - 1) > RLEN + 1 ? (G_END - 1 - RLEN - 2 - 12) / (NROUND - 1) : RLEN + 1;
     static constexpr int gp(int r) { return 12 + r * STRIDE; }
     static constexpr int gl(int r) { return r == 0 ? 2 : gp(r - 1) + 5; }
     static_assert(gp(NROUND - 1) + RLEN + 2 < G_END, "the rounds end in front of the barrier of tap 8");
-    static constexpr int td(int r) { return gl(r) / 64; }
-    static constexpr int nd(int t) { int n = t == 0 ? 2 : 0; for (int r = 0; r < NROUND; ++r) n += td(r) == t; return n; }
+    static constexpr int td(int r) { return gl(r) / SL; }
+    static constexpr int nd(int t) { int n = t == 0 ? 2 * NIMG : 0; for (int r = 0; r < NROUND; ++r) n += td(r) == t; return n; }
     static constexpr int DMA_TAB = 9;
     static constexpr int dma_piece(int r) { int k = td(r) == 0 ? 1 : 0; for (int q = 0; q < r; ++q) k += td(q) == td(r); return 9 + 2 * k; }
-    static_assert(td(NROUND - 1) < 8 && dma_piece(NROUND - 1) < 40, "requests behind the weight loads, in front of the barrier");
+    static_assert(td(NROUND - 1) < 8 && dma_piece(NROUND - 1) < SL, "requests behind the weight loads, inside the step");
 };
 
 __device__ __forceinline__ void cg3_mfma(f32x4& acc, const u32x4& b, const u32x4& a) {
@@ -85,8 +90,8 @@
 
 template <class Cfg>
 struct CG3Ctx {
-    u32x4 fa[2][8], fb[2][8];
-    unsigned boff[8];
+    u32x4 fa[2][8], fb[2][Cfg::TN];
+    unsigned boff[Cfg::TN];
     unsigned vo[Cfg::NROUND];
     unsigned scv[Cfg::PSW];
     unsigned a_dx[3];
@@ -100,8 +105,10 @@
     const unsigned char* wnext;
     const bf16* pnext;
     const float* tsc; const float* tsh;
+    int tio;
     const bf16* scnext;
     unsigned lds_patch, lds_tab, lds_sc, wave;
+    unsigned lds_pw;
 };
 
 template <int GG, int R, class Cfg>
@@ -169,54 +176,57 @@
     static __device__ __forceinline__ void requests(CG3Ctx<Cfg>& c) {
         if constexpr (R < Cfg::NROUND) {
             if constexpr (T == Cfg::td(R) && S == Cfg::dma_piece(R))
-                cg3_glds16(c.vo[R], c.pnext, c.lds_patch + (HP ^ 1) * Cfg::PATCH_BYTES + (R * Cfg::NW) * 1024 + c.wave * 1024);
+                cg3_glds16(c.vo[R], c.pnext, c.lds_pw + (HP ^ 1) * Cfg::PATCH_BYTES + R * Cfg::RSTEP * 1024);
             requests<R + 1>(c);
         }
     }
-    static __device__ __forceinline__ void run(f32x4 (&acc)[8][8], CG3Ctx<Cfg>& c) {
+    static __device__ __forceinline__ void run(f32x4 (&acc)[8][Cfg::TN], CG3Ctx<Cfg>& c) {
         constexpr int P = (T + HP) & 1;
         if constexpr (S == 0) {
             if constexpr (T >= 1 && NEXT) cg3_wait<Cfg::nd(T - 1), 0>(); else cg3_wait<0, 0>();
         }
-        if constexpr (S >= 1 && S <= 8) c.fb[P ^ 1][S - 1] = cg3_gload16(c.boff[S - 1], c.wnext);
+        if constexpr (S >= 1 && S <= Cfg::TN) c.fb[P ^ 1][S - 1] = cg3_gload16(c.boff[S - 1], c.wnext);
         reads<0>(c);
         if constexpr (NEXT) {
-            if constexpr (T == 0 && S == Cfg::DMA_TAB) cg3_gtab(c.tvo, c.tsc, c.tsh, c.lds_tab + (HP ^ 1) * Cfg::TAB_BYTES);
+            if constexpr (T == 0 && S == Cfg::DMA_TAB) {
+                cg3_gtab(c.tvo, c.tsc, c.tsh, c.lds_tab + (HP ^ 1) * Cfg::TAB_BYTES);
+                if constexpr (Cfg::NIMG > 1) cg3_gtab(c.tvo, c.tsc + c.tio, c.tsh + c.tio, c.lds_tab + (HP ^ 1) * Cfg::TAB_BYTES + Cfg::TAB_IMG_BYTES);
+            }
             requests<0>(c);
         } else if constexpr (T == 8 && S > Cfg::BAR && (S - Cfg::BAR - 1) % 2 == 0 && (S - Cfg::BAR - 1) / 2 < Cfg::PSW) {
             constexpr int n = (S - Cfg::BAR - 1) / 2;
             cg3_glds16(c.scv[n], c.scnext, c.lds_sc + Cfg::SC_BYTES + n * 1024 + c.wave * (Cfg::PSW * 1024));
         }
-        if constexpr (T >= 2 && NEXT) cg3_norm_slot<Cfg, HP ^ 1, (T - 2) * 64 + S>(c);
+        if constexpr (T >= 2 && NEXT) cg3_norm_slot<Cfg, HP ^ 1, (T - 2) * Cfg::SL + S>(c);
         if constexpr (T == 8) {
             if constexpr (S == Cfg::BAR - 1) cg3_wait_lgkm0();
             if constexpr (S == Cfg::BAR) cg3_barrier();
         }
-        constexpr int i = S >> 3, j = S & 7;
+        constexpr int i = S / Cfg::TN, j = S % Cfg::TN;
         cg3_mfma(acc[i][j], c.fb[P][j], c.fa[P][i]);
-        if constexpr (S + 1 < 64) CG3Tap<Cfg, T, HP, NEXT, S + 1>::run(acc, c);
+        if constexpr (S + 1 < Cfg::SL) CG3Tap<Cfg, T, HP, NEXT, S + 1>::run(acc, c);
     }
 };
 
 template <class Cfg, int P, int S>
 struct CG3Sc {
-    static __device__ __forceinline__ void run(f32x4 (&acc)[8][8], CG3Ctx<Cfg>& c) {
+    static __device__ __forceinline__ void run(f32x4 (&acc)[8][Cfg::TN], CG3Ctx<Cfg>& c) {
         if constexpr (S == 0) cg3_wait<Cfg::PSW, 0>();
         if constexpr (S == 1) cg3_barrier();
-        if constexpr (S >= 1 && S <= 8) c.fb[P ^ 1][S - 1] = cg3_gload16(c.boff[S - 1], c.wnext);
-        if constexpr (S >= 9 && (S - 9) % 2 == 0 && (S - 9) / 2 < Cfg::PSW) {
-            constexpr int n = (S - 9) / 2;
+        if constexpr (S >= 1 && S <= Cfg::TN) c.fb[P ^ 1][S - 1] = cg3_gload16(c.boff[S - 1], c.wnext);
+        if constexpr (S >= Cfg::dma_sc_early(0) && (S - Cfg::dma_sc_early(0)) % 2 == 0 && (S - Cfg::dma_sc_early(0)) / 2 < Cfg::PSW) {
+            constexpr int n = (S - Cfg::dma_sc_early(0)) / 2;
             cg3_glds16(c.scv[n], c.scnext, c.lds_sc + P * Cfg::SC_BYTES + n * 1024 + c.wave * (Cfg::PSW * 1024));
         }
-        if constexpr (S == Cfg::BAR - 1) cg3_wait<8 + Cfg::PSW, -1>();
+        if constexpr (S == Cfg::BAR - 1) cg3_wait<Cfg::TN + Cfg::PSW, -1>();
         if constexpr (S == Cfg::BAR) cg3_barrier();
         if constexpr (S > Cfg::BAR + 1 && (S - Cfg::BAR - 2) % 2 == 0 && (S - Cfg::BAR - 2) / 2 < 8) {
             constexpr int i = (S - Cfg::BAR - 2) / 2;
             c.fa[P ^ 1][i] = lds_read16<(P ^ 1) * Cfg::SC_BYTES + i * 1024>(c.a_sc);
         }
-        constexpr int i = S >> 3, j = S & 7;
+        constexpr int i = S / Cfg::TN, j = S % Cfg::TN;
         cg3_mfma(acc[i][j], c.fb[P][j], c.fa[P][i]);
-        if constexpr (S + 1 < 64) CG3Sc<Cfg, P, S + 1>::run(acc, c);
+        if constexpr (S + 1 < Cfg::SL) CG3Sc<Cfg, P, S + 1>::run(acc, c);
     }
 };
 
@@ -224,18 +234,20 @@
 __global__ __launch_bounds__(256) __attribute__((amdgpu_waves_per_eu(1, 1))) void k_conv_gn3(const GemmArgs g)
 {
     using Cfg = ConvGn3Cfg<RES, WM, WN>;
-    constexpr int W = Cfg::W, WS = Cfg::WS, HW = Cfg::HW, BM_ = Cfg::BM_, BN_ = Cfg::BN_, NROUND = Cfg::NROUND, PSW = Cfg::PSW, KT = Cfg::KT;
+    constexpr int W = Cfg::W, WS = Cfg::WS, HW = Cfg::HW, BM_ = Cfg::BM_, BN_ = Cfg::BN_, NROUND = Cfg::NROUND, PSW = Cfg::PSW, KT = Cfg::KT, TN = Cfg::TN;
+    constexpr int NIMG = Cfg::NIMG, IMGP = Cfg::IMGP;
     extern __shared__ __attribute__((aligned(16))) unsigned char smem[];
     lds_poison();
     const int tid = threadIdx.x, lane = tid & 63;
     const int wave = __builtin_amdgcn_readfirstlane(tid >> 6);
     NATINF_CG3_STAMP(0);
     const int wm = wave / WN, wn = wave % WN;
-    const int nN = g.N / BN_, nM = g.M / BM_;
+    const int nN = g.N / BN_, nM = (g.M + BM_ - 1) / BM_;
     const int tile = xcd_remap(blockIdx.x, nM * nN);
     const int mt = tile / nN, nt = tile - mt * nN;
     const int m0 = mt * BM_, n0 = nt * BN_;
     const int b = m0 / HW, y0 = (m0 % HW) / W;
+    const int nval = NIMG > 1 ? min(NIMG, (g.M - m0) / HW) : 1;
     const int ush = g.a0_up;
     const bf16* const img = g.a0 + (int64_t)b * (HW >> (2 * ush)) * g.a0_ld;
     const float* const gsc = g.gn_scale + (int64_t)b * g.gn_ld;
@@ -252,27 +264,40 @@
     c.lds_patch = (unsigned)(uintptr_t)((lds_u8*)smem);
     c.lds_tab = c.lds_patch + Cfg::OFF_TAB;
     c.lds_sc = c.lds_patch + Cfg::OFF_SC;
+    c.lds_pw = c.lds_patch + (unsigned)Cfg::piece0(wave) * 1024u;
+    c.tio = NIMG > 1 ? min(1, nval - 1) * g.gn_ld : 0;
     const int prow = lane >> 2, pslot = lane & 3;
 #pragma unroll
-    for (int j = 0; j < 8; ++j) c.boff[j] = (unsigned)(((n0 >> 4) + wn * 8 + j) * NT) * 1024u + (unsigned)lane * 16u;
+    for (int j = 0; j < TN; ++j) c.boff[j] = (unsigned)(((n0 >> 4) + wn * TN + j) * NT) * 1024u + (unsigned)lane * 16u;
 #pragma unroll
     for (int r = 0; r < NROUND; ++r) {
-        const int pp = (r * 4 + wave) * 16 + prow;
-        const int yy = pp / WS, xx = pp - yy * WS;
-        const int y = min(max(y0 - 1 + yy, 0), RES - 1), x = min(max(xx - 1, 0), RES - 1);
-        c.vo[r] = (unsigned)(((y >> ush) * (W >> ush) + (x >> ush)) * g.a0_ld + ((pslot ^ Cfg::swz_key(xx)) << 3)) * 2u;
-        const bool inside = (unsigned)(y0 - 1 + yy) < (unsigned)RES && (unsigned)(xx - 1) < (unsigned)RES;
-        c.ninf[r] = inside ? 0x3f800000u : 0x7f800000u;
-        c.nadr[r] = c.lds_patch + (unsigned)((r * 4 + wave) * 1024 + prow * 64 + ((pslot ^ Cfg::swz_key(xx)) << 4));
+        const int piece = Cfg::piece0(wave) + r * Cfg::RSTEP;
+        const int pp = piece * 16 + prow;
+        if constexpr (NIMG > 1) {
+            const int im = pp / IMGP, rem = pp - im * IMGP;
+            const int yy = rem / WS, xx = rem - yy * WS;
+            const int y = min(max(yy - 1, 0), RES - 1), x = min(max(xx - 1, 0), RES - 1);
+            c.vo[r] = (unsigned)((min(im, nval - 1) * HW + y * W + x) * g.a0_ld + ((pslot ^ Cfg::swz_key(xx)) << 3)) * 2u;
+            const bool inside = (unsigned)(yy - 1) < (unsigned)RES && (unsigned)(xx - 1) < (unsigned)RES;
+            c.ninf[r] = inside ? 0x3f800000u : 0x7f800000u;
+            c.nadr[r] = c.lds_patch + (unsigned)(piece * 1024 + prow * 64 + ((pslot ^ Cfg::swz_key(xx)) << 4));
+        } else {
+            const int yy = pp / WS, xx = pp - yy * WS;
+            const int y = min(max(y0 - 1 + yy, 0), RES - 1), x = min(max(xx - 1, 0), RES - 1);
+            c.vo[r] = (unsigned)(((y >> ush) * (W >> ush) + (x >> ush)) * g.a0_ld + ((pslot ^ Cfg::swz_key(xx)) << 3)) * 2u;
+            const bool inside = (unsigned)(y0 - 1 + yy) < (unsigned)RES && (unsigned)(xx - 1) < (unsigned)RES;
+            c.ninf[r] = inside ? 0x3f800000u : 0x7f800000u;
+            c.nadr[r] = c.lds_patch + (unsigned)(piece * 1024 + prow * 64 + ((pslot ^ Cfg::swz_key(xx)) << 4));
+        }
     }
 #pragma unroll
     for (int n = 0; n < PSW; ++n) {
         const int pp = (wave * PSW + n) * 16 + prow;
-        const int src = sup ? ((y0 + pp / W) >> 1) * (W >> 1) + ((pp % W) >> 1) : pp;
+        const int src = NIMG > 1 ? min(pp, nval * HW - 1) : (sup ? ((y0 + pp / W) >> 1) * (W >> 1) + ((pp % W) >> 1) : pp);
         c.scv[n] = (unsigned)(src * g.a1_ld + ((pslot ^ ((pp >> 1) & 2)) << 3)) * 2u;
     }
     c.tvo = (unsigned)(lane & 31) * 4u;
-    c.n_tab = c.lds_tab + ((unsigned)pslot << 5);
+    c.n_tab = c.lds_tab + ((unsigned)pslot << 5) + (unsigned)(wave / Cfg::WPI) * Cfg::TAB_IMG_BYTES;
     {
         const int frow = lane & 15, fq = lane >> 4;
         const int ml = wm * 128 + frow;
@@ -282,25 +307,39 @@
         c.a_sc = c.lds_sc + (unsigned)(ml * 64 + ((fq ^ ((ml >> 1) & 2)) << 4));
     }
 
+    unsigned warm_junk = 0;
+    if (RES <= 8 && g.w_warm) {
+        const int jx = (int)blockIdx.x >> 3;
+        const int nbx = min(((int)gridDim.x + 7 - ((int)blockIdx.x & 7)) >> 3, 16);
+        if (jx < nbx) {
+            const int NB16 = g.N >> 4, total = NB16 * NT;
+            int i = jx * Cfg::NW + wave;
+            for (int it = 0; it < 8 && i * 8 < total; ++it, i += nbx * Cfg::NW) {
+                const int pz = min(i * 8 + (lane >> 3), total - 1), kt = pz / NB16, nt_ = pz - kt * NB16;
+                asm volatile("global_load_dword %0, %1, %2" : "+v"(warm_junk) : "v"((unsigned)((nt_ * NT + kt) * 1024 + (lane & 7) * 128)), "s"(wfrag) : "memory");
+            }
+        }
+    }
     if (n_sc > 0) {
 #pragma unroll
         for (int n = 0; n < PSW; ++n) cg3_glds16(c.scv[n], a1base, c.lds_sc + n * 1024 + c.wave * (PSW * 1024));
     }
     cg3_gtab(c.tvo, gsc, gsh, c.lds_tab);
-#pragma unroll
-    for (int r = 0; r < NROUND; ++r) cg3_glds16(c.vo[r], img, c.lds_patch + (r * 4) * 1024 + c.wave * 1024);
-#pragma unroll
-    for (int j = 0; j < 8; ++j) c.fb[0][j] = cg3_gload16(c.boff[j], wfrag);
+    if constexpr (NIMG > 1) cg3_gtab(c.tvo, gsc + c.tio, gsh + c.tio, c.lds_tab + Cfg::TAB_IMG_BYTES);
+#pragma unroll
+    for (int r = 0; r < NROUND; ++r) cg3_glds16(c.vo[r], img, c.lds_pw + r * Cfg::RSTEP * 1024);
+#pragma unroll
+    for (int j = 0; j < TN; ++j) c.fb[0][j] = cg3_gload16(c.boff[j], wfrag);
     c.scnext = n_sc > 0 ? a1base + KT : reinterpret_cast<const bf16*>(wfrag);
-    f32x4 acc[8][8];
+    f32x4 acc[8][TN];
 #pragma unroll
     for (int i = 0; i < 8; ++i)
 #pragma unroll
-        for (int j = 0; j < 8; ++j) acc[i][j] = f32x4{0.f, 0.f, 0.f, 0.f};
+        for (int j = 0; j < TN; ++j) acc[i][j] = f32x4{0.f, 0.f, 0.f, 0.f};
     NATINF_CG3_STAMP(1);
     auto norm0 = [&](auto r_tag, const f32x4& s0, const f32x4& s1, const f32x4& h0, const f32x4& h1) __attribute__((always_inline)) {
         constexpr int R = decltype(r_tag)::value;
-        cg3_wait<NROUND - 1 - R + 8, -1>();
+        cg3_wait<NROUND - 1 - R + TN, -1>();
         unsigned char* const pa = smem + (c.nadr[R] - c.lds_patch);
         const u32x4 nv = *reinterpret_cast<const u32x4*>(pa);
         const float ni = __uint_as_float(c.ninf[R]);
@@ -320,17 +359,19 @@
         *reinterpret_cast<u32x4*>(pa) = ou;
     };
     {
-        cg3_wait<NROUND + 8, -1>();
+        cg3_wait<NROUND + TN, -1>();
+        asm volatile("" :: "v"(warm_junk));
         NATINF_CG3_STAMP(2);
         const unsigned char* const tp = smem + (c.n_tab - c.lds_patch);
         const f32x4 s0 = *reinterpret_cast<const f32x4*>(tp), s1 = *reinterpret_cast<const f32x4*>(tp + 16);
         const f32x4 h0 = *reinterpret_cast<const f32x4*>(tp + 128), h1 = *reinterpret_cast<const f32x4*>(tp + 144);
         using std::integral_constant;
         norm0(integral_constant<int, 0>{}, s0, s1, h0, h1); norm0(integral_constant<int, 1>{}, s0, s1, h0, h1); norm0(integral_constant<int, 2>{}, s0, s1, h0, h1);
-        norm0(integral_constant<int, 3>{}, s0, s1, h0, h1); norm0(integral_constant<int, 4>{}, s0, s1, h0, h1); norm0(integral_constant<int, 5>{}, s0, s1, h0, h1);
+        norm0(integral_constant<int, 3>{}, s0, s1, h0, h1);
+        if constexpr (NROUND > 4) { norm0(integral_constant<int, 4>{}, s0, s1, h0, h1); norm0(integral_constant<int, 5>{}, s0, s1, h0, h1); }
         if constexpr (NROUND > 6) { norm0(integral_constant<int, 6>{}, s0, s1, h0, h1); norm0(integral_constant<int, 7>{}, s0, s1, h0, h1); }
         if constexpr (NROUND > 8) { norm0(integral_constant<int, 8>{}, s0, s1, h0, h1); norm0(integral_constant<int, 9>{}, s0, s1, h0, h1); }
-        static_assert(NROUND == 6 || NROUND == 8 || NROUND == 10, "rounds of the prologue");
+        static_assert(NROUND == 4 || NROUND == 6 || NROUND == 8 || NROUND == 10, "rounds of the prologue");
     }
     cg3_wait<0, -1>();
     __syncthreads();
@@ -369,8 +410,11 @@
     }
     cg3_wait<0, 0>();
 #define NATINF_CG3_PIN8(a) asm volatile("" :: "v"(a[0]), "v"(a[1]), "v"(a[2]), "v"(a[3]), "v"(a[4]), "v"(a[5]), "v"(a[6]), "v"(a[7]));
-    NATINF_CG3_PIN8(c.fb[0]) NATINF_CG3_PIN8(c.fb[1]) NATINF_CG3_PIN8(c.fa[0]) NATINF_CG3_PIN8(c.fa[1])
+#define NATINF_CG3_PIN4(a) asm volatile("" :: "v"(a[0]), "v"(a[1]), "v"(a[2]), "v"(a[3]));
+    if constexpr (TN == 8) { NATINF_CG3_PIN8(c.fb[0]) NATINF_CG3_PIN8(c.fb[1]) } else { NATINF_CG3_PIN4(c.fb[0]) NATINF_CG3_PIN4(c.fb[1]) }
+    NATINF_CG3_PIN8(c.fa[0]) NATINF_CG3_PIN8(c.fa[1])
 #undef NATINF_CG3_PIN8
+#undef NATINF_CG3_PIN4
     NATINF_CG3_STAMP(41);
 #if defined(__HIP_DEVICE_COMPILE__)
     typedef const unsigned __attribute__((address_space(4))) *kernarg_u32_t;
@@ -394,8 +438,8 @@
     const int tid_e = wave * 64 + lane_e;
     NATINF_CG3_STAMP(42);
     static_assert(EPI == 1 || EPI == 2 || EPI == 5 || EPI == 6, "packed epilogues: plain / + GroupNorm partials / + bf16 residual / both");
-    constexpr bool FIN16 = RES == 16 && WM == 2 && WN == 2 && (EPI == 2 || EPI == 6);
-    packed_tile_epilogue<WM, WN, 8, 8, typename Cfg::Epi, ACT_NONE, EPI == 2 || EPI == 6, EPI == 5 || EPI == 6, false, false, 1, FIN16, true, true>(ge, smem, acc, m0, n0, 0, tid_e, lane_e, wm, wn);
+    constexpr bool FIN = ((RES == 16 && WM == 2 && WN == 2) || RES == 8) && (EPI == 2 || EPI == 6);
+    packed_tile_epilogue<WM, WN, 8, TN, typename Cfg::Epi, ACT_NONE, EPI == 2 || EPI == 6, EPI == 5 || EPI == 6, false, false, NIMG, FIN, true, true>(ge, smem, acc, m0, n0, 0, tid_e, lane_e, wm, wn);
     NATINF_CG3_STAMP(43);
 }
 
diff --git a/naturaldiffusion_amd/csrc/conv_gn3_lowres.hip b/naturaldiffusion_amd/csrc/conv_gn3_lowres.hip
--- /dev/null
+++ b/naturaldiffusion_amd/csrc/conv_gn3_lowres.hip
@@ -0,0 +1,33 @@
+#include <hip/hip_runtime.h>
+#include <stdint.h>
+#include <string.h>
+#include <type_traits>
+#include <utility>
+
+namespace {
+#include "conv_gn3.h"
+}
+using namespace ncsn;
+
+namespace {
+using Cfg8 = ConvGn3Cfg<8, 1, 4>;
+template <int EPI>
+bool cfg1() {
+    return hipFuncSetAttribute(reinterpret_cast<const void*>(&k_conv_gn3<8, 1, 4, EPI>), hipFuncAttributeMaxDynamicSharedMemorySize, Cfg8::LDS_BYTES) == hipSuccess;
+}
+}
+
+namespace ncsn_cg3l {
+__attribute__((visibility("hidden"))) bool configure() { return cfg1<2>() && cfg1<6>(); }
+__attribute__((visibility("hidden"))) bool has_epi(int epi) { return epi == 2 || epi == 6; }
+__attribute__((visibility("hidden"))) int tile_rows() { return Cfg8::BM_; }
+__attribute__((visibility("hidden"))) int tile_cols() { return Cfg8::BN_; }
+__attribute__((visibility("hidden"))) void launch(const void* gemm_args, int epi, void* stream) {
+    GemmArgs g;
+    memcpy(&g, gemm_args, sizeof(g));
+    hipStream_t s = reinterpret_cast<hipStream_t>(stream);
+    const dim3 grid((unsigned)(((g.M + Cfg8::BM_ - 1) / Cfg8::BM_) * (g.N / Cfg8::BN_)));
+    if (epi == 2) hipLaunchKernelGGL((k_conv_gn3<8, 1, 4, 2>), grid, dim3(256), Cfg8::LDS_BYTES, s, g);
+    else hipLaunchKernelGGL((k_conv_gn3<8, 1, 4, 6>), grid, dim3(256), Cfg8::LDS_BYTES, s, g);
+}
+}
diff --git a/naturaldiffusion_amd/csrc/ncsnpp.hip b/naturaldiffusion_amd/csrc/ncsnpp.hip
--- a/naturaldiffusion_amd/csrc/ncsnpp.hip
+++ b/naturaldiffusion_amd/csrc/ncsnpp.hip
@@ -121,6 +121,7 @@
 bool configure_conv_ring();
 namespace { bool configure_dit_attention(); }
 namespace ncsn_cg3 { bool configure(); int tile_rows(int shape); int tile_cols(int shape); void launch(const void* gemm_args, int shape, int epi, void* stream); }
+namespace ncsn_cg3l { bool configure(); bool has_epi(int epi); int tile_rows(); int tile_cols(); void launch(const void* gemm_args, int epi, void* stream); }
 
 namespace {
 
@@ -263,7 +264,7 @@
                                   GEMM_LDS_BYTES) == hipSuccess;
     ok = ok && hipFuncSetAttribute(reinterpret_cast<const void*>(&k_head_conv), hipFuncAttributeMaxDynamicSharedMemorySize, HeadConvCfg::LDS_BYTES) == hipSuccess &&
          set_lds<CfgR128x128>(&k_gemm_ring<2, 2, 4, 4, 4, 9>) &&
-         set_lds_epi_all() && ncsn_cg3::configure() && ::configure_conv_ring() && configure_dit_attention() && set_lds_conv_gn<1>() && set_lds_conv_gn<2>() && set_lds_conv_gn<5>() && set_lds_conv_gn<6>() &&
+         set_lds_epi_all() && ncsn_cg3::configure() && ncsn_cg3l::configure() && ::configure_conv_ring() && configure_dit_attention() && set_lds_conv_gn<1>() && set_lds_conv_gn<2>() && set_lds_conv_gn<5>() && set_lds_conv_gn<6>() &&
 #ifdef NATINF_DEV
          set_lds<CfgD256x256>(&k_gemm_dma<2, 4, 8, 4>) && set_lds<CfgD256x128>(&k_gemm_dma<4, 2, 4, 4>) &&
          set_lds<CfgD128x128>(&k_gemm_dma<2, 2, 4, 4>) && set_lds<CfgR256x256>(&k_gemm_ring<2, 4, 8, 4, 4>) &&
@@ -311,9 +312,13 @@
 int g_fuse_up = 1;
 int g_cg_regw = 1;
 int g_cg3_min_k[3] = {2304, 0, 2304};
+int g_cg3_lowres = 1;
+int packed_epi_of_conv(const GemmArgs& g, int part_rows) { GemmArgs t = g; t.epi_fp32_slab = 0; return packed_epi(t, part_rows); }
 inline int conv_gn3_shape(const GemmArgs& g) {
     const int res = 1 << g.logW;
     if (!g_cg3 || !g_cg_regw || !g.b_frag || g.N % 128) return -1;
+    if (res == 8)
+        return (g_cg3_lowres & 1) && g.N % 256 == 0 && !g.a0_up && !g.a1_up && ncsn_cg3l::has_epi(packed_epi_of_conv(g, 64)) ? 3 : -1;
     int sh = -1;
     if (res == 32) sh = g.N % 256 ? ((g_cg3 & 1) ? 0 : -1) : ((g_cg3 & 2) ? 1 : -1);
     else if (res == 16) sh = (g.N % 256 == 0 && (g_cg3 & 4)) ? 2 : -1;
@@ -322,7 +327,7 @@
 }
 inline int conv_gn_bm(const GemmArgs& g) {
     const int res = 1 << g.logW;
-    if (const int sh3 = conv_gn3_shape(g); sh3 >= 0) return ncsn_cg3::tile_rows(sh3);
+    if (const int sh3 = conv_gn3_shape(g); sh3 >= 0) return sh3 == 3 ? ncsn_cg3l::tile_rows() : ncsn_cg3::tile_rows(sh3);
     if (res == 8) return g_cg8_tm4 ? 64 : 128;
     if (res == 4) return 64;
     if (res == 32) return ((g_cg_wide & 2) && g.N % 256 == 0 && g_cg_regw && g.b_frag) ? 128 : 256;
@@ -335,7 +340,7 @@
 #else
 constexpr bool HAVE_CONV_GN_V1 = false;
 #endif
-inline int conv_gn_epi(const GemmArgs& g) { GemmArgs t = g; t.epi_fp32_slab = 0; return packed_epi(t, conv_gn_part_rows(g)); }
+inline int conv_gn_epi(const GemmArgs& g) { return packed_epi_of_conv(g, conv_gn_part_rows(g)); }
 inline bool conv_gn_ok(const GemmArgs& g) {
     if (!g.gn_scale || !g.gn_shift || !g.gn_folded || g.taps != 9 || g.batch != 1 || g.a0_C % BK || (g.a1 && g.a1_C % BK)) return false;
     const int res = 1 << g.logW;
@@ -593,7 +598,8 @@
     if (g_record) {
         char line[160];
         snprintf(line, sizeof(line), "%d %d %d %d %d %d %s/e%d\n", g.M, g.N, g.taps * g.a0_C, g.a1 ? g.a1_C : 0, g.taps, g.batch,
-                 v == V_CONV_GN && conv_gn3_shape(g) >= 0 ? "conv_gn3" : variant_name(v), v == V_CONV_GN ? conv_gn_epi(g) : effective_epi(v, g));
+                 v == V_CONV_GN && conv_gn3_shape(g) >= 0 && conv_gn3_shape(g) < 3 ? "conv_gn3" : variant_name(v),
+                 v == V_CONV_GN ? conv_gn_epi(g) : effective_epi(v, g));
         *g_record += line;
         return v == V_CONV_GN ? conv_gn_part_rows(g) : variant_bm(v);
     }
@@ -660,6 +666,7 @@
                 default: launch_tiles<CFG>(&k_conv_gn2<RES, WIDE, 6>, g, s); break;                             \
             }
             if (const int sh3 = conv_gn3_shape(g); sh3 >= 0) {
+                if (sh3 == 3) { ncsn_cg3l::launch(&g, e, (void*)s); return conv_gn_part_rows(g); }
                 ncsn_cg3::launch(&g, sh3, e, (void*)s);
                 g_fin_written = sh3 == 2 && g.fin_scale && (e == 2 || e == 6) && g.N == 256;
                 return conv_gn_part_rows(g);
@@ -1721,6 +1728,7 @@
 }
 int natinf_set_fuse_head(int on) { g_fuse_head = on != 0; return NATINF_OK; }
 int natinf_set_conv_gn_w128(int mask) { if (mask < 0 || mask > 7) return NATINF_EINVAL; g_cg3 = mask; return NATINF_OK; }
+int natinf_set_conv_gn_w128_lowres(int mask) { if (mask < 0 || mask > 1) return NATINF_EINVAL; g_cg3_lowres = mask; return NATINF_OK; }
 int natinf_set_conv_gn_w128_min_k(int shape, int k) { if (shape < 0 || shape > 2 || k < 0) return NATINF_EINVAL; g_cg3_min_k[shape] = k; return NATINF_OK; }
 int natinf_set_conv_gn_wide(int mask) { if (mask < 0 || mask > 3) return NATINF_EINVAL; g_cg_wide = mask; return NATINF_OK; }
 int natinf_set_conv_gn_regw(int on) {
```

Result: no change. 3473 images/s, median of 6 (+0.6%).
